# HKUST-Aerial-Robotics/MIND

Measured on AMD Instinct MI355X. Metric: sim steps/sec (whole node) + scenario-tree nodes expanded/sec, AV2 demo scenes, higher is better.
Workload: dtype f32-class (bf16 hi+mid+lo split operands = 24 significand bits, six products, fp32 accumulate) pair kernel + ActorNet, f32 elsewhere in the predictor, f64 iLQR

## Files before the change

include/mind_hip.h:

```cpp
#ifndef MIND_HIP_H
#define MIND_HIP_H

#include <stddef.h>
#include <stdint.h>

#ifdef __cplusplus
extern "C" {
#endif

#define MIND_OK 0
#define MIND_EINVAL (-1)
#define MIND_ENOMEM (-2)
#define MIND_EHIP (-3)
#define MIND_ESTATE (-4)
#define MIND_ENOTFOUND (-5)

typedef struct mind_ctx mind_ctx;

int mind_ctx_create(int device, void *stream, mind_ctx **out);
int mind_ctx_destroy(mind_ctx *ctx);
const char *mind_last_error_string(mind_ctx *ctx);
int mind_ctx_synchronize(mind_ctx *ctx);

typedef struct {
// ... 12 lines not shown
  const float *lanes;
  const float *lane_feat;
  const float *actor_ctrs;
  const float *actor_vecs;
  const float *lane_ctrs;
  const float *lane_vecs;
  const float *const *rpe;
  const float *tgt_nodes;
  const float *tgt_rpe;
} mind_scene_batch;

typedef struct {
  float *cls;
  float *reg;
  float *vel;
  float *lane_feat;
  float *actor_emb;
  float *cls_emb;
} mind_pred_out;

int mind_predict_batch(mind_ctx *ctx, const mind_scene_batch *in, mind_pred_out *out);

int mind_last_fusion_stats(mind_ctx *ctx, int *n_launches, float *total_ms, double *pairs_processed);
int mind_last_actor_stats(mind_ctx *ctx, int *layerwise, int *n_launches, int *n_chunks, float *total_ms);
int mind_last_token_stats(mind_ctx *ctx, int *layerwise, int *n_launches, int *n_chunks, float *total_ms);
int mind_last_token_stage_ms(mind_ctx *ctx, float *out_ms, int cap);
int mind_last_ilqr_stats(mind_ctx *ctx, float *kernel_ms, int *n_trees, int *workgroups_per_tree);
int mind_last_ilqr_profile(mind_ctx *ctx, double *out9);
int mind_last_ilqr_trace(mind_ctx *ctx, int tree, int phase, double *out, int cap_rows, int *n_rows);
int mind_set_profiling(mind_ctx *ctx, int enable);

#define MIND_PAIR_F32 0
#define MIND_PAIR_BF16X3 1
#define MIND_PAIR_BF16 2
#define MIND_PAIR_BF16X6 3
int mind_set_pair_precision(mind_ctx *ctx, int mode);

int mind_set_tuning(mind_ctx *ctx, const char *name, int value);
int mind_get_pair_precision(mind_ctx *ctx);
int mind_debug_pack_bfrag(const float *w, int row_stride, uint32_t *out);

int mind_debug_pair_schedule(const int *scene_tokens, const int *scene_actors, int n_scenes, int n_cu, int last_layer, int *out_jobs, int cap,
                             int *out_info);

int mind_debug_predict_choice(const char *const *knob_names, const int *knob_values, int n_knobs, int pair_prec, int n_cu, int have_side,
                              const int *scene_actors, const int *scene_lanes, int n_scenes, long long *out, int cap);

int mind_debug_ilqr_plan(const char *const *knob_names, const int *knob_values, int n_knobs, int n_cu, int mode, int n_trees, const int *n_nodes,
                         const int32_t *parents, long long *out, int cap, int *bad);

int mind_debug_aime_book(int pred_len, int max_depth, int max_rounds, int n_agents, int world, int rank, int force, int n_rounds, const int *dec_len,
                         const float *dec, int n_tokens, int bytes_per_pair, int plan_chunk_mb, int per_scene, long long *out, int cap, char *msg,
                         int msg_cap);

int mind_debug_actor_lw_plan(int n_actors, int np, int chunk, long long *out_launches, int cap, long long *out_info);

int mind_debug_token_lw_plan(int n_tokens, int mode, int chunk, long long *out_launches, int cap, long long *out_info);

int mind_debug_pack_conv_frag(const float *w, int co, int ci, int ksz, uint32_t *out, size_t cap);

int mind_debug_pack(const char *what, const float *w, int a, int b, int c, float *out, size_t cap);
int mind_debug_weight_image(const mind_tensor_desc *tensors, int n_tensors, float *blob, size_t blob_cap, char *names, size_t names_cap,
                            long long *entries, int entries_cap, long long *out_info, char *msg, int msg_cap);
int mind_debug_weight_bind(const mind_tensor_desc *tensors, int n_tensors, const char *drop, char *msg, int msg_cap);

int mind_debug_trig(mind_ctx *ctx, const double *x, int n, double *out);

int mind_debug_set_layers(mind_ctx *ctx, int n);
int64_t mind_debug_read(mind_ctx *ctx, const char *name, float *host, int64_t max_floats);

typedef struct {
  int n_nodes;
  const int32_t *parent;
  const float *prob;
  int n_agents;
  const float *agent_mean;
  const float *agent_cov;
  const double *field;
  const double *node_w;
} mind_cost_tree;

typedef struct {
  double dt, wheelbase;
  double w_des_state[6];
  double w_state_con[6];
  double state_lower[6], state_upper[6];
  double w_ctrl[2];
  double w_tgt, w_ego, w_ego_cov_offset, w_exo, w_exo_cov_offset, w_exo_cost_offset;
  double grid_res; int grid_w, grid_h;
  int max_iter;
} mind_ilqr_cfg;

typedef struct { int iterations; int converged; double J; double mu; } mind_ilqr_stats;

int mind_ilqr_solve_trees(mind_ctx *ctx, const mind_ilqr_cfg *cfg, const mind_cost_tree *trees,
                          int n_trees, const double *x0, const double *target_lane, int n_lane_pts,
                          double target_vel, int use_exo, const double *us_init, double *xs,
                          double *us, mind_ilqr_stats *stats);

int mind_ilqr_contingency(mind_ctx *ctx, const mind_ilqr_cfg *cfg_warm, const mind_ilqr_cfg *cfg_full,
                          const mind_cost_tree *trees, int n_trees, const double *x0,
                          const double *target_lane, int n_lane_pts, double target_vel, double *xs,
                          double *us, mind_ilqr_stats *stats_warm, mind_ilqr_stats *stats_full);
int mind_ilqr_contingency_begin(mind_ctx *ctx, const mind_ilqr_cfg *cfg_warm, const mind_ilqr_cfg *cfg_full,
                                const mind_cost_tree *trees, int n_trees, const double *x0,
                                const double *target_lane, int n_lane_pts, double target_vel, double *xs,
// ... 282 lines not shown
```

mind_amd/_lib.py:

```python
import ctypes as C
import os

_HERE = os.path.dirname(os.path.abspath(__file__))
LIB_PATH = os.environ.get("MIND_HIP_LIB", os.path.join(_HERE, "libmind_hip.so"))

MIND_OK = 0
MIND_EINVAL, MIND_ENOMEM, MIND_EHIP, MIND_ESTATE, MIND_ENOTFOUND = -1, -2, -3, -4, -5


class TensorDesc(C.Structure):
    _fields_ = [("name", C.c_char_p), ("data", C.POINTER(C.c_float)), ("numel", C.c_int64)]


class SceneBatch(C.Structure):
    _fields_ = [("n_scenes", C.c_int), ("actor_off", C.POINTER(C.c_int32)), ("lane_off", C.POINTER(C.c_int32)),
                ("actors", C.c_void_p), ("lanes", C.c_void_p), ("lane_feat", C.c_void_p),
                ("actor_ctrs", C.c_void_p), ("actor_vecs", C.c_void_p), ("lane_ctrs", C.c_void_p),
                ("lane_vecs", C.c_void_p), ("rpe", C.POINTER(C.c_void_p)), ("tgt_nodes", C.c_void_p),
                ("tgt_rpe", C.c_void_p)]


class PredOut(C.Structure):
    _fields_ = [("cls", C.c_void_p), ("reg", C.c_void_p), ("vel", C.c_void_p), ("lane_feat", C.c_void_p),
                ("actor_emb", C.c_void_p), ("cls_emb", C.c_void_p)]


class CostTree(C.Structure):
    _fields_ = [("n_nodes", C.c_int), ("parent", C.POINTER(C.c_int32)), ("prob", C.POINTER(C.c_float)),
                ("n_agents", C.c_int), ("agent_mean", C.POINTER(C.c_float)), ("agent_cov", C.POINTER(C.c_float)),
                ("field", C.POINTER(C.c_double)), ("node_w", C.POINTER(C.c_double))]


class FieldGrid(C.Structure):
    _fields_ = [("W", C.c_int), ("H", C.c_int), ("res", C.c_double), ("off_x", C.c_double), ("off_y", C.c_double),
                ("gx", C.POINTER(C.c_double)), ("gy", C.POINTER(C.c_double))]


class IlqrGainsOut(C.Structure):
    _fields_ = [(n, C.POINTER(C.c_double)) for n in ("k", "K", "dV", "V_x", "V_xx", "xs", "L", "J")] + [("bad_node", C.POINTER(C.c_int32))]


class WorldIn(C.Structure):
    _fields_ = [("n_scenes", C.c_int), ("actor_off", C.POINTER(C.c_int32)), ("reg", C.c_void_p), ("vel", C.c_void_p),
                ("actor_ctrs", C.c_void_p), ("actor_vecs", C.c_void_p), ("rot", C.POINTER(C.c_float)),
                ("orig", C.POINTER(C.c_float)), ("cov_last", C.POINTER(C.c_float)), ("last", C.POINTER(C.c_int32)),
                ("target_lane", C.POINTER(C.c_float)), ("n_lane_pts", C.c_int), ("cls", C.c_void_p),
                ("scen_prob", C.POINTER(C.c_float)), ("lane_check", C.c_int), ("dist_thres", C.c_float)]


class WorldOut(C.Structure):
    _fields_ = [("world", C.c_void_p), ("topo", C.c_void_p), ("ego_end", C.c_void_p), ("sel", C.c_void_p), ("sel_prob", C.c_void_p)]


class RebaseIn(C.Structure):
    _fields_ = [("n_scenes", C.c_int), ("n_agents", C.c_int), ("n_lanes", C.c_int), ("pos", C.POINTER(C.c_float)),
                ("ang", C.POINTER(C.c_float)), ("vel", C.POINTER(C.c_float)), ("types", C.POINTER(C.c_float)),
                ("pad", C.POINTER(C.c_float)), ("lane_ctrs", C.POINTER(C.c_float)), ("lane_vecs", C.POINTER(C.c_float)),
                ("target_lane", C.POINTER(C.c_float)), ("target_lane_info", C.POINTER(C.c_float)), ("n_lane_pts", C.c_int),
# ... 52 lines not shown

class LoopDesc(C.Structure):
    _fields_ = [("n_tracks", C.c_int), ("n_steps", C.c_int), ("clamp_last", C.c_int), ("ego_state", C.c_void_p), ("ego_state_is_f32", C.c_int), ("ego_obs", C.c_void_p), ("ego_trig32", C.c_void_p),
                ("tan_fn", C.c_void_p), ("sincos_fn", C.c_void_p), ("exo_obs", C.c_void_p),
                ("exo_valid", C.c_void_p), ("timestep", C.c_void_p), ("type_slot", C.c_void_p),
                ("sim_step", C.c_double), ("plan_step", C.c_double), ("enable_time", C.c_double),
                ("wheelbase", C.c_double), ("max_speed", C.c_double), ("max_steer", C.c_double), ("max_acc", C.c_double), ("max_dec", C.c_double),
                ("n_lanes", C.c_int), ("lane_pts", C.c_void_p), ("lane_flags", C.c_void_p),
                ("n_lane_pts", C.c_int), ("target_lane", C.c_void_p), ("target_lane_info", C.c_void_p),
                ("time_ahead", C.c_double), ("min_vel", C.c_float), ("dist_thres", C.c_float), ("max_depth", C.c_int), ("max_rounds", C.c_int),
                ("pred_len", C.c_int), ("prob_floor", C.c_float),
                ("cfg_warm", C.c_void_p), ("cfg_full", C.c_void_p), ("solve_n_lane_pts", C.c_int), ("solve_lane", C.c_void_p), ("target_vel", C.c_double),
                ("eval_n_lane_pts", C.c_int), ("eval_lane_is_f32", C.c_int), ("eval_lane", C.c_void_p), ("speculative", C.c_int)]


class LoopTotals(C.Structure):
    _fields_ = [("plans", C.c_longlong), ("expansions", C.c_longlong), ("scen_trees", C.c_longlong), ("rounds", C.c_longlong),
                ("aime_s", C.c_double), ("ilqr_s", C.c_double), ("total_s", C.c_double),
                ("iterations", C.c_longlong), ("node_iterations", C.c_longlong), ("node_iterations_exo", C.c_longlong),
                ("warm_speculated", C.c_longlong), ("warm_hits", C.c_longlong),
                ("pair_ms", C.c_double), ("pair_launches", C.c_longlong), ("scene_n2", C.c_double), ("scene_n_a1", C.c_double),
                ("ilqr_ms", C.c_double), ("ilqr_launches", C.c_longlong), ("ilqr_trees", C.c_longlong), ("ilqr_workgroups_per_tree", C.c_int),
                ("ilqr_prof", C.c_double * 9), ("ilqr_node_steps", C.c_double)]


class LoopOut(C.Structure):
    _fields_ = [("planned", C.c_int), ("enabled", C.c_int), ("n_steps", C.c_longlong), ("n_plans", C.c_longlong), ("episode_steps", C.c_longlong),
                ("sim_time", C.c_double), ("last_trigger", C.c_double), ("state", C.c_double * 4), ("ctrl", C.c_double * 2),
                ("n_agents", C.c_int), ("n_trees", C.c_int), ("best", C.c_int), ("n_expanded", C.c_int), ("n_rounds", C.c_int), ("n_traj_nodes", C.c_int),
                ("costs", C.POINTER(C.c_double)), ("aime_s", C.c_double), ("ilqr_s", C.c_double), ("total_s", C.c_double),
                ("tot", LoopTotals)]


PLANNER_EGO_KEY = -(1 << 63)


class PlannerDesc(C.Structure):
    _fields_ = [("time_ahead", C.c_double), ("min_vel", C.c_float), ("dist_thres", C.c_float), ("max_depth", C.c_int), ("max_rounds", C.c_int),
                ("pred_len", C.c_int), ("prob_floor", C.c_float), ("cfg_warm", C.c_void_p), ("cfg_full", C.c_void_p), ("speculative", C.c_int),
                ("ego_type_slot", C.c_int)]


class PlannerOut(C.Structure):
    _fields_ = [("n_plans", C.c_longlong),
                ("n_agents", C.c_int), ("n_trees", C.c_int), ("best", C.c_int), ("n_expanded", C.c_int), ("n_rounds", C.c_int), ("n_traj_nodes", C.c_int),
                ("costs", C.POINTER(C.c_double)), ("ctrl", C.c_double * 2), ("aime_s", C.c_double), ("ilqr_s", C.c_double), ("total_s", C.c_double),
                ("tot", LoopTotals)]


EXPORTS = ["mind_ctx_create", "mind_ctx_destroy", "mind_last_error_string", "mind_ctx_synchronize",
           "mind_weights_load", "mind_predict_batch", "mind_last_fusion_stats", "mind_last_actor_stats", "mind_debug_actor_lw_plan", "mind_last_token_stats", "mind_last_token_stage_ms", "mind_debug_token_lw_plan", "mind_set_profiling",
           "mind_ilqr_solve_trees", "mind_ilqr_contingency", "mind_ilqr_solve_fields", "mind_cost_eval", "mind_ilqr_score_trees", "mind_ilqr_gains", "mind_ilqr_policy_rollouts", "mind_lane_dist_field", "mind_aime_world", "mind_aime_rebase", "mind_debug_aime_decide", "mind_debug_set_layers",
           "mind_debug_read", "mind_set_pair_precision", "mind_get_pair_precision", "mind_debug_pack_bfrag", "mind_debug_pack_conv_frag", "mind_debug_pack", "mind_debug_weight_image", "mind_debug_weight_bind", "mind_debug_pair_schedule", "mind_debug_predict_choice", "mind_debug_ilqr_plan", "mind_debug_aime_book", "mind_set_tuning", "mind_last_ilqr_stats", "mind_aime_plan", "mind_last_ilqr_profile", "mind_eval_traj_trees", "mind_last_ilqr_trace", "mind_ilqr_contingency_begin", "mind_ilqr_finish", "mind_fill_tracks", "mind_ilqr_contingency_begin_plan", "mind_debug_trig", "mind_aime_plan_begin", "mind_aime_plan_poll", "mind_aime_plan_finish", "mind_ctx_busy", "mind_ilqr_finish_plan",
           "mind_set_exchange", "mind_last_exchange_stats",
           "mind_loop_create", "mind_loop_destroy", "mind_loop_reset", "mind_loop_advance", "mind_loop_state", "mind_loop_last_plan", "mind_loop_export",
           "mind_planner_create", "mind_planner_destroy", "mind_planner_reset", "mind_planner_observe", "mind_planner_set_lanes", "mind_planner_set_target_lane",
           "mind_planner_set_solve_lane", "mind_planner_set_eval_lane", "mind_planner_plan", "mind_planner_last_plan", "mind_planner_export"]

EXCHANGE_FN = C.CFUNCTYPE(C.c_int, C.c_void_p, C.c_int, C.c_void_p, C.c_void_p, C.c_int64)
XCHG_ALLGATHER, XCHG_ALLREDUCE, XCHG_ALLTOALLV = 0, 1, 2

_lib = None


def load():
    global _lib
    if _lib is not None:
        return _lib
    if not os.path.exists(LIB_PATH):
        raise ImportError(f"{LIB_PATH} is missing: the HIP extension must be built (hipcc --offload-arch=gfx950); "
                          "there is no CPU fallback for the product path")
    lib = C.CDLL(LIB_PATH)
    lib.mind_ctx_create.argtypes = [C.c_int, C.c_void_p, C.POINTER(C.c_void_p)]
    lib.mind_ctx_destroy.argtypes = [C.c_void_p]
    lib.mind_last_error_string.argtypes = [C.c_void_p]
    lib.mind_last_error_string.restype = C.c_char_p
    lib.mind_ctx_synchronize.argtypes = [C.c_void_p]
    lib.mind_weights_load.argtypes = [C.c_void_p, C.POINTER(TensorDesc), C.c_int]
    lib.mind_predict_batch.argtypes = [C.c_void_p, C.POINTER(SceneBatch), C.POINTER(PredOut)]
    lib.mind_last_fusion_stats.argtypes = [C.c_void_p, C.POINTER(C.c_int), C.POINTER(C.c_float), C.POINTER(C.c_double)]
    lib.mind_last_actor_stats.argtypes = [C.c_void_p, C.POINTER(C.c_int), C.POINTER(C.c_int), C.POINTER(C.c_int), C.POINTER(C.c_float)]
    lib.mind_debug_actor_lw_plan.argtypes = [C.c_int, C.c_int, C.c_int, C.POINTER(C.c_longlong), C.c_int, C.POINTER(C.c_longlong)]
    lib.mind_last_token_stats.argtypes = [C.c_void_p, C.POINTER(C.c_int), C.POINTER(C.c_int), C.POINTER(C.c_int), C.POINTER(C.c_float)]
    lib.mind_last_token_stage_ms.argtypes = [C.c_void_p, C.POINTER(C.c_float), C.c_int]
    lib.mind_debug_token_lw_plan.argtypes = [C.c_int, C.c_int, C.c_int, C.POINTER(C.c_longlong), C.c_int, C.POINTER(C.c_longlong)]
    lib.mind_set_profiling.argtypes = [C.c_void_p, C.c_int]
    lib.mind_ilqr_solve_trees.argtypes = [C.c_void_p, C.POINTER(IlqrCfg), C.POINTER(CostTree), C.c_int,
                                          C.POINTER(C.c_double), C.POINTER(C.c_double), C.c_int, C.c_double, C.c_int,
                                          C.POINTER(C.c_double), C.POINTER(C.c_double), C.POINTER(C.c_double),
                                          C.POINTER(IlqrStats)]
    lib.mind_ilqr_contingency.argtypes = [C.c_void_p, C.POINTER(IlqrCfg), C.POINTER(IlqrCfg), C.POINTER(CostTree), C.c_int,
                                          C.POINTER(C.c_double), C.POINTER(C.c_double), C.c_int, C.c_double,
                                          C.POINTER(C.c_double), C.POINTER(C.c_double), C.POINTER(IlqrStats), C.POINTER(IlqrStats)]
    lib.mind_ilqr_contingency_begin.argtypes = [C.c_void_p, C.POINTER(IlqrCfg), C.POINTER(IlqrCfg), C.POINTER(CostTree), C.c_int,
                                          C.POINTER(C.c_double), C.POINTER(C.c_double), C.c_int, C.c_double,
                                          C.POINTER(C.c_double), C.POINTER(C.c_double), C.POINTER(IlqrStats), C.POINTER(IlqrStats)]
    lib.mind_ilqr_finish.argtypes = [C.c_void_p]
    lib.mind_ilqr_contingency_begin_plan.argtypes = [C.c_void_p, C.POINTER(IlqrCfg), C.POINTER(IlqrCfg), C.c_void_p, C.c_void_p, C.c_int, C.c_double,
                                                     C.c_void_p, C.c_void_p, C.c_void_p, C.c_void_p]
    lib.mind_fill_tracks.argtypes = [C.c_void_p, C.c_int, C.c_int, C.c_void_p, C.c_void_p, C.c_void_p, C.c_void_p, C.c_void_p, C.c_void_p]
    lib.mind_ilqr_solve_fields.argtypes = [C.c_void_p, C.POINTER(IlqrCfg), C.POINTER(FieldGrid), C.POINTER(CostTree), C.c_int,
                                           C.POINTER(C.c_double), C.POINTER(C.c_double), C.POINTER(C.c_double),
                                           C.POINTER(C.c_double), C.POINTER(IlqrStats)]
    lib.mind_cost_eval.argtypes = [C.c_void_p, C.POINTER(IlqrCfg), C.POINTER(FieldGrid), C.POINTER(CostTree),
                                   C.POINTER(C.c_double), C.POINTER(C.c_double), C.c_int, C.c_double, C.c_int, C.c_int,
                                   C.POINTER(C.c_int32), C.POINTER(C.c_double), C.POINTER(C.c_double), C.POINTER(C.c_double)]
    lib.mind_ilqr_score_trees.argtypes = [C.c_void_p, C.POINTER(IlqrCfg), C.POINTER(FieldGrid), C.POINTER(CostTree), C.c_int,
                                          C.POINTER(C.c_double), C.POINTER(C.c_double), C.c_int, C.c_double, C.c_int, C.c_int,
                                          C.POINTER(C.c_double), C.POINTER(C.c_double), C.POINTER(C.c_double), C.POINTER(C.c_double)]
    lib.mind_ilqr_gains.argtypes = [C.c_void_p, C.POINTER(IlqrCfg), C.POINTER(FieldGrid), C.POINTER(CostTree), C.c_int,
                                    C.POINTER(C.c_double), C.POINTER(C.c_double), C.c_int, C.c_double, C.c_int,
                                    C.POINTER(C.c_double), C.POINTER(C.c_double), C.POINTER(IlqrGainsOut)]
    lib.mind_ilqr_policy_rollouts.argtypes = [C.c_void_p, C.POINTER(IlqrCfg), C.POINTER(FieldGrid), C.POINTER(CostTree), C.c_int,
                                              C.POINTER(C.c_double), C.POINTER(C.c_double), C.c_int, C.c_double, C.c_int,
                                              C.POINTER(C.c_double), C.POINTER(C.c_double), C.POINTER(C.c_double), C.c_int,
                                              C.POINTER(C.c_double), C.POINTER(C.c_double), C.POINTER(C.c_double), C.POINTER(C.c_double),
                                              C.POINTER(C.c_double), C.POINTER(C.c_double)]
    lib.mind_lane_dist_field.argtypes = [C.c_void_p, C.POINTER(C.c_double), C.POINTER(C.c_double), C.c_int, C.c_int, C.c_int,
                                         C.c_double] + [C.POINTER(C.c_double)] * 4
    lib.mind_aime_world.argtypes = [C.c_void_p, C.POINTER(WorldIn), C.POINTER(WorldOut)]
    lib.mind_aime_rebase.argtypes = [C.c_void_p, C.POINTER(RebaseIn), C.POINTER(RebaseOut)]
    lib.mind_debug_aime_decide.argtypes = [C.c_void_p, C.c_int, C.POINTER(C.c_int32), C.POINTER(C.c_int32), C.c_void_p, C.POINTER(C.c_float), C.c_void_p,
                                           C.c_void_p, C.c_void_p, C.c_int, C.c_float, C.c_float, C.c_int, C.c_int, C.c_void_p, C.c_void_p, C.c_void_p]
    lib.mind_aime_plan.argtypes = [C.c_void_p, C.POINTER(AimePlanIn), C.POINTER(AimePlanOut)]
    lib.mind_aime_plan_begin.argtypes = [C.c_void_p, C.POINTER(AimePlanIn)]
    lib.mind_aime_plan_poll.argtypes = [C.c_void_p]
    lib.mind_aime_plan_finish.argtypes = [C.c_void_p, C.POINTER(AimePlanOut)]
    lib.mind_ctx_busy.argtypes = [C.c_void_p]
    lib.mind_ilqr_finish_plan.argtypes = [C.c_void_p, C.c_int, C.c_int, C.c_void_p, C.c_void_p, C.c_void_p, C.c_void_p]
    lib.mind_set_pair_precision.argtypes = [C.c_void_p, C.c_int]
    lib.mind_set_tuning.argtypes = [C.c_void_p, C.c_char_p, C.c_int]
    lib.mind_last_ilqr_stats.argtypes = [C.c_void_p, C.POINTER(C.c_float), C.POINTER(C.c_int), C.POINTER(C.c_int)]
    lib.mind_last_ilqr_profile.argtypes = [C.c_void_p, C.POINTER(C.c_double)]
    lib.mind_last_ilqr_trace.argtypes = [C.c_void_p, C.c_int, C.c_int, C.POINTER(C.c_double), C.c_int, C.POINTER(C.c_int)]
    lib.mind_eval_traj_trees.argtypes = [C.POINTER(C.c_double), C.POINTER(C.c_double), C.POINTER(C.c_int32), C.c_int, C.c_void_p, C.c_int, C.c_int,
                                         C.c_double, C.POINTER(C.c_double)]
    lib.mind_get_pair_precision.argtypes = [C.c_void_p]
    lib.mind_debug_pack_bfrag.argtypes = [C.POINTER(C.c_float), C.c_int, C.POINTER(C.c_uint32)]
    lib.mind_debug_pair_schedule.argtypes = [C.POINTER(C.c_int), C.POINTER(C.c_int), C.c_int, C.c_int, C.c_int, C.POINTER(C.c_int), C.c_int, C.POINTER(C.c_int)]
    lib.mind_debug_predict_choice.argtypes = [C.POINTER(C.c_char_p), C.POINTER(C.c_int), C.c_int, C.c_int, C.c_int, C.c_int, C.POINTER(C.c_int), C.POINTER(C.c_int),
                                              C.c_int, C.POINTER(C.c_longlong), C.c_int]
    lib.mind_debug_ilqr_plan.argtypes = [C.POINTER(C.c_char_p), C.POINTER(C.c_int), C.c_int, C.c_int, C.c_int, C.c_int, C.POINTER(C.c_int), C.POINTER(C.c_int32),
                                         C.POINTER(C.c_longlong), C.c_int, C.POINTER(C.c_int)]
    lib.mind_debug_aime_book.argtypes = [C.c_int] * 8 + [C.POINTER(C.c_int), C.POINTER(C.c_float)] + [C.c_int] * 4 + [C.POINTER(C.c_longlong), C.c_int, C.c_char_p, C.c_int]
    lib.mind_debug_trig.argtypes = [C.c_void_p, C.POINTER(C.c_double), C.c_int, C.POINTER(C.c_double)]
    lib.mind_debug_pack_conv_frag.argtypes = [C.POINTER(C.c_float), C.c_int, C.c_int, C.c_int, C.POINTER(C.c_uint32), C.c_size_t]
    lib.mind_debug_pack.argtypes = [C.c_char_p, C.POINTER(C.c_float), C.c_int, C.c_int, C.c_int, C.POINTER(C.c_float), C.c_size_t]
    lib.mind_debug_weight_image.argtypes = [C.POINTER(TensorDesc), C.c_int, C.POINTER(C.c_float), C.c_size_t, C.c_char_p, C.c_size_t,
                                            C.POINTER(C.c_longlong), C.c_int, C.POINTER(C.c_longlong), C.c_char_p, C.c_int]
    lib.mind_debug_weight_bind.argtypes = [C.POINTER(TensorDesc), C.c_int, C.c_char_p, C.c_char_p, C.c_int]
    lib.mind_debug_set_layers.argtypes = [C.c_void_p, C.c_int]
    lib.mind_debug_read.argtypes = [C.c_void_p, C.c_char_p, C.POINTER(C.c_float), C.c_int64]
    lib.mind_set_exchange.argtypes = [C.c_void_p, C.c_int, C.c_int, EXCHANGE_FN, C.c_void_p, C.c_int]
    lib.mind_last_exchange_stats.argtypes = [C.c_void_p, C.POINTER(C.c_longlong), C.POINTER(C.c_longlong)]
    lib.mind_loop_create.argtypes = [C.c_void_p, C.POINTER(LoopDesc), C.POINTER(C.c_void_p)]
    lib.mind_loop_destroy.argtypes = [C.c_void_p]
    lib.mind_loop_reset.argtypes = [C.c_void_p]
    lib.mind_loop_advance.argtypes = [C.c_void_p, C.c_int, C.c_double, C.c_longlong, C.POINTER(LoopOut)]
    lib.mind_loop_state.argtypes = [C.c_void_p, C.POINTER(LoopOut)]
    lib.mind_loop_last_plan.argtypes = [C.c_void_p, C.POINTER(AimePlanOut)] + [C.POINTER(C.c_void_p)] * 6 + [C.c_void_p]
    lib.mind_loop_export.argtypes = [C.c_void_p, C.c_int, C.POINTER(C.c_int), C.c_void_p, C.c_void_p, C.c_void_p]
    lib.mind_planner_create.argtypes = [C.c_void_p, C.POINTER(PlannerDesc), C.POINTER(C.c_void_p)]
    lib.mind_planner_destroy.argtypes = [C.c_void_p]
    lib.mind_planner_reset.argtypes = [C.c_void_p]
    lib.mind_planner_observe.argtypes = [C.c_void_p, C.c_int, C.c_void_p, C.c_int, C.c_void_p, C.c_void_p, C.c_void_p]
    lib.mind_planner_set_lanes.argtypes = [C.c_void_p, C.c_int, C.c_void_p, C.c_void_p]
    lib.mind_planner_set_target_lane.argtypes = [C.c_void_p, C.c_int, C.c_void_p, C.c_void_p]
    lib.mind_planner_set_solve_lane.argtypes = [C.c_void_p, C.c_int, C.c_void_p, C.c_double]
    lib.mind_planner_set_eval_lane.argtypes = [C.c_void_p, C.c_int, C.c_void_p, C.c_int]
    lib.mind_planner_plan.argtypes = [C.c_void_p, C.c_void_p, C.c_void_p, C.POINTER(PlannerOut)]
    lib.mind_planner_last_plan.argtypes = [C.c_void_p, C.POINTER(AimePlanOut)] + [C.POINTER(C.c_void_p)] * 6 + [C.c_void_p]
    lib.mind_planner_export.argtypes = [C.c_void_p, C.c_int, C.POINTER(C.c_int), C.c_void_p, C.c_void_p, C.c_void_p]
    for n in EXPORTS:
        getattr(lib, n)
        if n not in ("mind_last_error_string", "mind_debug_read"):
            getattr(lib, n).restype = C.c_int
    lib.mind_debug_read.restype = C.c_int64
    _lib = lib
    return lib


PRED_CHOICE_FIELDS = ("header", "n_runs", "np", "actor_form", "actor_arg", "actor_grid", "actor_chunk", "actor_chunks", "actor_launches", "qsplit", "qk_stride",
                      "tiled", "edge_bf16", "edge_pair_bytes", "tok_chunk", "tok_lw", "tok_chunks", "pair_family", "pair_np", "l5_jobs5", "xcd_lanes",
                      "xcd_lanes5", "dec_actor", "dec_np", "fp32_dec", "split_dec", "want_mw", "mw_blocks", "cls_on_side", "tgt_wait_first")
PAIR_PREC = ("f32", "bf16x3", "bf16", "bf16x6")


def predict_choice(knobs, prec, scenes, n_cu=256, have_side=True):
    lib = load()
    names = (C.c_char_p * max(1, len(knobs)))(*[k.encode() for k in knobs])
    vals = (C.c_int * max(1, len(knobs)))(*[int(v) for v in knobs.values()])
    sa = (C.c_int * len(scenes))(*[a for a, _ in scenes])
    sl = (C.c_int * len(scenes))(*[l for _, l in scenes])
    cap = 32 + 6 * len(scenes)
    out = (C.c_longlong * cap)()
    n = lib.mind_debug_predict_choice(names, vals, len(knobs), PAIR_PREC.index(prec) if isinstance(prec, str) else prec, n_cu, int(have_side),
                                      sa, sl, len(scenes), out, cap)
    if n == MIND_EINVAL:
        return None
    assert 0 < n <= cap and out[0] == 32 and n == 32 + 6 * out[1], n
    d = dict(zip(PRED_CHOICE_FIELDS, out[:30]))
    d["runs"] = [tuple(out[32 + 6 * i:38 + 6 * i]) for i in range(out[1])]
    return d


ILQR_PLAN_FIELDS = ("header", "n_trees", "form", "G", "GS", "spec", "nslot", "grid", "workgroups_per_tree", "host_out", "early", "starve_followers")
ILQR_TREE_FIELDS = ("M", "nl", "nseg", "nsl", "maxls", "nfs")
ILQR_TREE_TABLES = ("level_start", "level_nodes", "child_start", "child_list", "seg_start", "seg_nodes", "slevel_start", "slevel_segs", "seg_rec",
                    "fstep_start", "fstep_items", "fstep_q1", "fstep_nstart", "fstep_nodes")


def ilqr_plan(knobs, parents, n_cu=256, generic=False, evaluate=False, two_fits=False):
    lib = load()
    names = (C.c_char_p * max(1, len(knobs)))(*[k.encode() for k in knobs])
    vals = (C.c_int * max(1, len(knobs)))(*[int(v) for v in knobs.values()])
    nn = (C.c_int * len(parents))(*[len(p) for p in parents])
    flat = [int(v) for p in parents for v in p]
    par = (C.c_int32 * max(1, len(flat)))(*flat)
    bad = (C.c_int * 2)()
    mode = int(generic) | int(evaluate) << 1 | int(two_fits) << 2
    n = lib.mind_debug_ilqr_plan(names, vals, len(knobs), n_cu, mode, len(parents), nn, par, None, 0, bad)
    if n == MIND_EINVAL:
        return {"bad": (bad[0], bad[1])} if bad[0] >= 0 else None
    out = (C.c_longlong * n)()
    assert lib.mind_debug_ilqr_plan(names, vals, len(knobs), n_cu, mode, len(parents), nn, par, out, n, bad) == n and out[0] == 16
    d = dict(zip(ILQR_PLAN_FIELDS, out[:12]))
    d["trees"], o = [], 16
    for _ in parents:
        tr = dict(zip(ILQR_TREE_FIELDS, out[o:o + 6]))
        lens, o = out[o + 6:o + 20], o + 20
        for name, ln in zip(ILQR_TREE_TABLES, lens):
            tr[name], o = list(out[o:o + ln]), o + ln
        d["trees"].append(tr)
    assert o == n
    return d


AIME_ROUND_FIELDS = ("B", "lo", "hi", "Bmax", "chunk", "S", "s0", "Sm", "any")
AIME_NODE_FIELDS = ("round", "scene", "mode", "parent", "prob", "cur_t", "end_t", "flags", "dur", "row_off", "owner", "lscene")


def aime_book(pred_len, max_depth, n_agents, rounds, world=1, rank=0, force=False, max_rounds=32, n_tokens=0, bytes_per_pair=512, plan_chunk_mb=96 * 1024,
              per_scene=1):
    import numpy as np
    lib = load()
    arrs = [np.ascontiguousarray(r, np.float32).ravel() for r in rounds]
    lens = (C.c_int * max(1, len(arrs)))(*[a.size for a in arrs])
    dec = np.concatenate(arrs + [np.zeros(1, np.float32)])
    msg = C.create_string_buffer(256)
    args = [pred_len, max_depth, max_rounds, n_agents, world, rank, int(force), len(arrs), lens, dec.ctypes.data_as(C.POINTER(C.c_float)), n_tokens,
            bytes_per_pair, plan_chunk_mb, per_scene]
    n = lib.mind_debug_aime_book(*args, None, 0, msg, 256)
    if n == MIND_EINVAL:
        return None
# ... 78 lines not shown
```

mind_amd/csrc/aime_book.h:

```cpp
#pragma once
#include <algorithm>
#include <cstddef>
#include <cstdint>
#include <cstring>
#include <vector>

#include "../../include/mind_hip.h"

constexpr int PL_K = 6;
constexpr int PL_OBS = 50;

struct PlScene {
  int node;
  float prob;
  int cur_t, end_t;
  float rot[4], orig[2], tgt[22];
};

struct PlNode {
  int round, scene, mode, parent, depth;
  int owner, lscene;
  float prob;
  int cur_t, end_t;
  bool branch, end, term, rebased;
  unsigned long long hit;
  float tgt[22];
};

inline void pl_block(int n, int r, int w, int &lo, int &hi) {
  const int base = n / w, rem = n % w;
  lo = r * base + (r < rem ? r : rem);
  hi = lo + base + (r < rem ? 1 : 0);
}
inline int pl_owner(int n, int w, int b) {
  for (int r = 0; r < w; ++r) { int lo, hi; pl_block(n, r, w, lo, hi); if (b >= lo && b < hi) return r; }
  return w - 1;
}

inline bool pl_exchanges(bool have_transport, int world, bool force) { return have_transport && (world > 1 || force); }

inline int pl_chunk(int n_tokens, int bytes_per_pair, int plan_chunk_mb, int Bk) {
  const double edge_mb = (double)n_tokens * (((n_tokens + 15) / 16) * 16) * bytes_per_pair / (1024.0 * 1024.0);
  return std::max(1, (int)std::min<double>((double)(Bk > 0 ? Bk : 1), (double)plan_chunk_mb / edge_mb));
}

enum { PL_OK = 0, PL_E_ROUNDS, PL_E_ROOT, PL_E_TRIMMED, PL_E_AGAIN, PL_E_ORDER, PL_E_NO_END };
struct PlErr { int code = PL_OK, a0 = 0, a1 = 0; explicit operator bool() const { return code != PL_OK; } };
inline const char *pl_err_format(int code) {
  switch (code) {
    case PL_E_ROUNDS: return "unsupported: more than %d AIME rounds";
    case PL_E_ROOT: return "unsupported: the root is a branching candidate";
    case PL_E_TRIMMED: return "unsupported: branch time of a trimmed node with CUR_T > 0";
    case PL_E_AGAIN: return "unsupported: a node of round %d is expanded again in round %d";
    case PL_E_ORDER: return "unsupported: branch set out of scene order";
    case PL_E_NO_END: return "unsupported: no end node found in the scenario tree";
  }
  return "";
}

struct PlTake { size_t o = 0; size_t operator()(size_t n) { const size_t r = o; o += (n + 3) & ~(size_t)3; return r; } };
struct RootLayout {
  size_t actors, ctrs, vecs, lanes, lc, lv, tn, tr, cov, types, tl, ti, wpos, wang, wvel, fr, rpos, rang, rvel, rpad, lpts, lfl, total;
  RootLayout(size_t a, size_t l, size_t P, bool raw) {
    PlTake take;
    actors = take(a * 14 * 48); ctrs = take(a * 2); vecs = take(a * 2); lanes = take(l * 160);
    lc = take(l * 2); lv = take(l * 2); tn = take(160); tr = take(20); cov = take(a);
    types = take(a * PL_OBS * 7); tl = take(P * 2); ti = take(P * 12);
    wpos = take(a * PL_OBS * 2); wang = take(a * PL_OBS); wvel = take(a * PL_OBS * 2);
    fr = take(28); rpos = take(raw ? a * PL_OBS * 2 : 0); rang = take(raw ? a * PL_OBS : 0);
    rvel = take(raw ? a * PL_OBS * 2 : 0); rpad = take(raw ? a * PL_OBS : 0);
    lpts = take(raw ? l * 11 * 2 * 2 : 0); lfl = take(raw ? l * 6 : 0);
    total = take.o;
  }
};
struct InLayout {
  size_t actors, ctrs, vecs, lc, lv, tn, tr, fr, cov, total;
  InLayout(size_t S, size_t a, size_t l) {
    PlTake take;
    actors = take(S * a * 14 * 48); ctrs = take(S * a * 2); vecs = take(S * a * 2); lc = take(S * l * 2); lv = take(S * l * 2);
    tn = take(S * 160); tr = take(S * 20); fr = take(S * 28); cov = take(S * a); total = take.o;
  }
};

struct PlRoute {
  std::vector<int64_t> tab;
  std::vector<int> snd, rcv;
  long long any = 0;
};
inline void pl_route(int S, int world, int rank, const std::vector<int> &cnt_r, const std::vector<int> &s0_r, size_t per_scene, bool self_too, PlRoute &q) {
  q.tab.assign(2 * (size_t)world, 0); q.snd.assign(2 * (size_t)world, 0); q.rcv.assign(2 * (size_t)world, 0);
  q.any = 0;
  for (int j = 0; j < world; ++j)
    for (int k = 0; k < world; ++k) {
      if (j == k && !self_too) continue;
      int klo, khi;
      pl_block(S, k, world, klo, khi);
// ... 240 lines not shown
```

mind_amd/csrc/aime_kernels.hip:

```cpp
#include <hip/hip_runtime.h>
#include <stdint.h>

struct AimeScene {
  int a0, a1;
  int last, cmp;
  float r00, r01, r10, r11;
  float ox, oy, theta_g, pad2;
};

#define AIME_SMALL 8
struct AimeSmall {
  AimeScene s[AIME_SMALL];
  float prob[AIME_SMALL];
  int n, a, pad0, pad1;
};

#define AIME_T 60
#define AIME_K 6
#define AIME_PK 6

__device__ __forceinline__ void aime_to_world(float lx, float ly, float c, float s, float cx, float cy, const AimeScene &S,
                                              bool translate, float &wx, float &wy) {
  float ax = lx * c + ly * (-s), ay = lx * s + ly * c;
  if (translate) { ax += cx; ay += cy; }
// ... 151 lines not shown
  float so[AIME_K], po[AIME_K];
  aime_select_scene(S, sp, b, t, cls, topo, ego_end, lane_check, dist_thres, prob_floor, so, po);
  if (t != 0) return;
#pragma unroll
  for (int k = 0; k < AIME_K; ++k) { sel[(size_t)b * AIME_K + k] = so[k]; sel_prob[(size_t)b * AIME_K + k] = po[k]; }
}

#define RB_THREADS 256
#define RB_FEAT_BLOCKS(a) ((int)(((size_t)(a) * 48 + RB_THREADS - 1) / RB_THREADS))
#define RB_T 50
#define RB_LANE_LDS 1024

struct RebaseArgs {
  int a, l, n_lane, pad_ones;
  const float *pos, *ang, *vel;
  const float *types;
  const float *pad;
  const float *lane_ctrs0, *lane_vecs0;
  const float *tlane, *tinfo;
  float time_ahead, min_vel;
  float *actors, *actor_ctrs, *actor_vecs, *lane_ctrs, *lane_vecs, *tgt_nodes, *tgt_rpe, *frames;
  float travel0;
};

__device__ __forceinline__ void rb_cs(float ax, float ay, float bx, float by, float &c, float &s) {
  const float den = sqrtf(ax * ax + ay * ay) * sqrtf(bx * bx + by * by) + 1e-10f;
  c = (ax * bx + ay * by) / den;
  s = (ax * by - ay * bx) / den;
}

__global__ __launch_bounds__(64) void k_aime_windows(const float *__restrict__ prev_pos, const float *__restrict__ prev_ang,
                                                     const float *__restrict__ prev_vel, const float *__restrict__ rows,
                                                     const int *__restrict__ parent_slot, const int *__restrict__ row0,
                                                     const int *__restrict__ dur, int a, float *__restrict__ pos,
                                                     float *__restrict__ ang, float *__restrict__ vel, int row_stride,
                                                     float *__restrict__ cov_last) {
  const int s = blockIdx.x / a, i = blockIdx.x - s * a, t = threadIdx.x;
  if (t >= RB_T) return;
  const int d = dur[s];
  const int src = t + d;
  float x, y, vx, vy, h;
  if (src < RB_T) {
    const size_t p = ((size_t)parent_slot[s] * a + i) * RB_T + src;
    x = prev_pos[2 * p]; y = prev_pos[2 * p + 1]; vx = prev_vel[2 * p]; vy = prev_vel[2 * p + 1]; h = prev_ang[p];
  } else {
    const float *r = rows + (((size_t)row0[s] + (size_t)i * row_stride) * AIME_T + (src - RB_T)) * AIME_PK;
    x = r[0]; y = r[1]; vx = r[2]; vy = r[3]; h = r[4];
    if (cov_last && t == RB_T - 1) cov_last[(size_t)s * a + i] = r[5];
  }
  const size_t o = ((size_t)s * a + i) * RB_T + t;
  pos[2 * o] = x; pos[2 * o + 1] = y; vel[2 * o] = vx; vel[2 * o + 1] = vy; ang[o] = h;
}

__global__ __launch_bounds__(64) void k_aime_branch(const AimeScene *__restrict__ scenes, const float *__restrict__ sel,
                                                    const float *__restrict__ world, unsigned *__restrict__ hit,
                                                    const float *__restrict__ sel_prob, float *__restrict__ h_sel, float *__restrict__ h_selp,
                                                    unsigned *__restrict__ h_hit, const AimeSmall sm) {
  const int b = blockIdx.x / AIME_K, j = blockIdx.x % AIME_K, t = threadIdx.x;
  const AimeScene S = sm.n ? sm.s[b] : scenes[b];
  const int k = (int)sel[(size_t)b * AIME_K + j];
  bool h = false;
  if (k >= 0 && t < AIME_T) {
    for (int i = S.a0; i < S.a1; ++i) {
      const float *r = world + ((size_t)i * AIME_K + k) * AIME_T * AIME_PK;
      h |= (r[t * AIME_PK + 5] / r[S.cmp * AIME_PK + 5]) > 9.0f;
    }
  }
  const unsigned long long m = __ballot(h);
  if (t == 0) { hit[2 * (size_t)blockIdx.x] = (unsigned)m; hit[2 * (size_t)blockIdx.x + 1] = (unsigned)(m >> 32); }
  if (h_sel && t == 0) {
    h_hit[2 * (size_t)blockIdx.x] = (unsigned)m; h_hit[2 * (size_t)blockIdx.x + 1] = (unsigned)(m >> 32);
    h_sel[blockIdx.x] = sel[blockIdx.x]; h_selp[blockIdx.x] = sel_prob[blockIdx.x];
  }
}

__global__ __launch_bounds__(64) void k_aime_select_branch(const AimeScene *__restrict__ scenes, const float *__restrict__ cls,
                                                           const float *__restrict__ scen_prob, const float *__restrict__ topo,
                                                           const float *__restrict__ ego_end, int lane_check, float dist_thres, float prob_floor,
                                                           const float *__restrict__ world, float *__restrict__ sel, float *__restrict__ sel_prob,
                                                           unsigned *__restrict__ hit, float *__restrict__ h_sel, float *__restrict__ h_selp,
                                                           unsigned *__restrict__ h_hit, const AimeSmall sm) {
  const int b = blockIdx.x / AIME_K, j = blockIdx.x % AIME_K, t = threadIdx.x;
  const AimeScene S = sm.n ? sm.s[b] : scenes[b];
  const float sp = sm.n ? sm.prob[b] : scen_prob[b];
  float so[AIME_K], po[AIME_K];
  aime_select_scene(S, sp, b, t, cls, topo, ego_end, lane_check, dist_thres, prob_floor, so, po);
  float kf = -1.f, pj = 0.f;
#pragma unroll
  for (int q = 0; q < AIME_K; ++q) if (q == j) { kf = so[q]; pj = po[q]; }
  const int k = (int)kf;
  bool h = false;
  if (k >= 0 && t < AIME_T) {
    for (int i0 = S.a0; i0 < S.a1; i0 += 8) {
      float num[8], den[8];
#pragma unroll
      for (int q = 0; q < 8; ++q) {
        const int i = i0 + q < S.a1 ? i0 + q : S.a1 - 1;
        const float *r = world + ((size_t)i * AIME_K + k) * AIME_T * AIME_PK;
        num[q] = r[t * AIME_PK + 5]; den[q] = r[S.cmp * AIME_PK + 5];
      }
#pragma unroll
      for (int q = 0; q < 8; ++q) if (i0 + q < S.a1) h |= (num[q] / den[q]) > 9.0f;
    }
  }
  const unsigned long long m = __ballot(h);
  if (t == 0) {
    hit[2 * (size_t)blockIdx.x] = (unsigned)m; hit[2 * (size_t)blockIdx.x + 1] = (unsigned)(m >> 32);
    sel[blockIdx.x] = kf; sel_prob[blockIdx.x] = pj;
    if (h_sel) {
      h_hit[2 * (size_t)blockIdx.x] = (unsigned)m; h_hit[2 * (size_t)blockIdx.x + 1] = (unsigned)(m >> 32);
      h_sel[blockIdx.x] = kf; h_selp[blockIdx.x] = pj;
    }
  }
}

struct AimeGather { int row0, dur, dst, a; };
__global__ __launch_bounds__(64) void k_aime_gather(const AimeGather *__restrict__ jobs, const int *__restrict__ job_of_block,
                                                    const int *__restrict__ agent_of_block, const float *const *__restrict__ world_of_job,
                                                    float *__restrict__ out) {
  const AimeGather J = jobs[job_of_block[blockIdx.x]];
  const int i = agent_of_block[blockIdx.x], t = threadIdx.x;
  if (t >= J.dur) return;
  const float *r = world_of_job[job_of_block[blockIdx.x]] + (((size_t)J.row0 + (size_t)i * AIME_K) * AIME_T + t) * AIME_PK;
  float *o = out + (size_t)J.dst + ((size_t)i * J.dur + t) * 3;
  o[0] = r[0]; o[1] = r[1]; o[2] = r[5];
}

struct AimeFlat { int row0, n, dst, a; };
__global__ __launch_bounds__(64) void k_aime_flat(const AimeFlat *__restrict__ jobs, const int *__restrict__ job_of_block,
                                                  const int *__restrict__ agent_of_block, const float *const *__restrict__ world_of_job,
                                                  float *__restrict__ mean, float *__restrict__ cov) {
  const AimeFlat J = jobs[job_of_block[blockIdx.x]];
  const int i = agent_of_block[blockIdx.x], m = threadIdx.x;
  if (m >= J.n) return;
  const float *r = world_of_job[job_of_block[blockIdx.x]] + (((size_t)J.row0 + (size_t)i * AIME_K) * AIME_T + 2 * m) * AIME_PK;
  const size_t o = (size_t)(J.dst + m) * J.a + i;
  mean[2 * o] = r[0]; mean[2 * o + 1] = r[1];
  cov[o] = r[5];
}

__global__ void k_repeat_rows(const float *__restrict__ src, size_t n, int times, float *__restrict__ dst) {
  const size_t i = (size_t)blockIdx.x * blockDim.x + threadIdx.x;
  if (i >= n * (size_t)times) return;
  dst[i] = src[i % n];
}

__global__ __launch_bounds__(RB_THREADS) void k_aime_rebase(RebaseArgs A) {
  const int sc = blockIdx.x, tid = threadIdx.x;
  const int a = A.a;
  extern __shared__ float rb_sm[];
  __shared__ float fr[8];
  __shared__ float rdv[RB_THREADS];
  __shared__ int rdi[RB_THREADS];
  __shared__ int s_idx;
  __shared__ float ctr[11][2];
  const float *pos = A.pos + (size_t)sc * a * RB_T * 2;
  const float *ang = A.ang + (size_t)sc * a * RB_T;
  const float *vel = A.vel + (size_t)sc * a * RB_T * 2;
  if (tid == 0) {
    const float th = ang[RB_T - 1];
    fr[0] = pos[(RB_T - 1) * 2]; fr[1] = pos[(RB_T - 1) * 2 + 1]; fr[2] = th; fr[3] = cosf(th); fr[4] = sinf(th);
  }
  __syncthreads();
  const float ox = fr[0], oy = fr[1], th0 = fr[2], c0 = fr[3], s0 = fr[4];
// ... 222 lines not shown
```

mind_amd/csrc/aime_plan.hip:

```cpp
#include <chrono>
namespace {

int pl_pin(mind_ctx *c, int which, size_t bytes) {
  if (bytes <= c->pl_pin_cap[which]) return MIND_OK;
  if (c->pl_pin[which]) (void)hipHostFree(c->pl_pin[which]);
  c->pl_pin[which] = nullptr; c->pl_pin_cap[which] = 0;
  const size_t want = bytes < ((size_t)64 << 20) ? std::max<size_t>(2 * bytes, (size_t)1 << 20) : bytes + bytes / 2 + 4096;
  if (hipHostMalloc(&c->pl_pin[which], want, hipHostMallocDefault) != hipSuccess)
    return fail(c, MIND_ENOMEM, "hipHostMalloc(%zu) failed", want);
  c->pl_pin_cap[which] = want;
  return MIND_OK;
}

struct CopySeg { const float *src; float *dst; long long n; };
__global__ __launch_bounds__(256) void k_copy_segs(const CopySeg *__restrict__ segs) {
  const CopySeg S = segs[blockIdx.y];
  const long long i0 = (long long)blockIdx.x * 2048 + threadIdx.x;
#pragma unroll
  for (int k = 0; k < 8; ++k) {
    const long long i = i0 + k * 256;
    if (i < S.n) S.dst[i] = S.src[i];
  }
}

int pl_exchange(mind_ctx *c, int op, void *send, void *recv, size_t bytes) {
  HIPCHK(c, hipStreamSynchronize(c->stream));
  const int rc = c->xfn(c->xuser, op, send, recv, (int64_t)bytes);
  if (rc) return fail(c, MIND_EHIP, "mind_aime_plan: the exchange callback failed (%d)", rc);
  c->x_collectives += 1;
  c->x_bytes += op == MIND_XCHG_ALLGATHER ? (long long)bytes * c->xw : (long long)bytes;
  return MIND_OK;
}

int pl_exchange_v(mind_ctx *c, void *send, void *recv, const int64_t *table) {
  HIPCHK(c, hipStreamSynchronize(c->stream));
  const int rc = c->xfn(c->xuser, MIND_XCHG_ALLTOALLV, send, recv, (int64_t)(intptr_t)table);
  if (rc) return fail(c, MIND_EHIP, "mind_aime_plan: the exchange callback failed (%d)", rc);
  c->x_collectives += 1;
  for (int r = 0; r < c->xw; ++r) c->x_bytes += (long long)table[(size_t)c->xw + r];
  return MIND_OK;
}

int pl_copy_segs(mind_ctx *c, const std::vector<CopySeg> &segs) {
  if (segs.empty()) return MIND_OK;
  long long mx = 0;
  for (const CopySeg &s : segs) mx = std::max(mx, s.n);
  if (mx == 0) return MIND_OK;
  int rc;
  if ((rc = ensure(c, c->x_seg, segs.size() * sizeof(CopySeg)))) return rc;
  if ((rc = pl_pin(c, 6, segs.size() * sizeof(CopySeg)))) return rc;
  memcpy(c->pl_pin[6], segs.data(), segs.size() * sizeof(CopySeg));
  HIPCHK(c, hipMemcpyAsync(c->x_seg.p, c->pl_pin[6], segs.size() * sizeof(CopySeg), hipMemcpyHostToDevice, c->stream));
  hipLaunchKernelGGL(k_copy_segs, dim3((unsigned)((mx + 2047) / 2048), (unsigned)segs.size()), dim3(256), 0, c->stream, (const CopySeg *)c->x_seg.p);
  HIPCHK(c, hipGetLastError());
  return MIND_OK;
}

static_assert(PL_K == AIME_K && PL_OBS == RB_T, "aime_book.h restates the kernels' constants");
static_assert(sizeof(PlJob) == sizeof(AimeGather) && sizeof(PlJob) == sizeof(AimeFlat) && offsetof(PlJob, row0) == offsetof(AimeGather, row0) &&
                  offsetof(PlJob, row0) == offsetof(AimeFlat, row0) && offsetof(PlJob, n) == offsetof(AimeGather, dur) && offsetof(PlJob, n) == offsetof(AimeFlat, n) &&
                  offsetof(PlJob, dst) == offsetof(AimeGather, dst) && offsetof(PlJob, dst) == offsetof(AimeFlat, dst) && offsetof(PlJob, a) == offsetof(AimeGather, a) &&
                  offsetof(PlJob, a) == offsetof(AimeFlat, a), "JobTable holds the packing kernels' job records");

struct PlTrace {
  std::chrono::steady_clock::time_point t0 = std::chrono::steady_clock::now();
  void operator()(const char *what) const {
    static const bool on = getenv("MIND_PLAN_TRACE") != nullptr;
    if (on) fprintf(stderr, "[plan] %8.1f us  %s\n", std::chrono::duration<double, std::micro>(std::chrono::steady_clock::now() - t0).count(), what);
  }
};

struct PlanRun {
  mind_ctx *c;
  const mind_aime_plan_in *in;
  mind_aime_plan_out *out;
  hipStream_t st;
  AimeBook &book;
  const int a, l, P, HZ;
  const bool raw;
  const int XW, XR;
  const bool dist;
  const RootLayout ro;
  const float *droot = nullptr;
  int cur_in = -1;
  const float *prev_pos = nullptr, *prev_ang = nullptr, *prev_vel = nullptr, *cov_last_dev = nullptr;
  bool frames_pending = false;
  int n_expanded = 0, pair_launches = 0;
  PlGeom g = {0, 0, 0, 0, 0};
  int chunk = 1;
  bool all_small = false, tables_done = false;
  size_t bS = 0, bI = 0, bP = 0, tab_bytes = 0, n_back = 0;
  DevBuf *tabb = nullptr;
  float *d_topo = nullptr, *d_ego = nullptr, *d_sel = nullptr, *d_selp = nullptr, *h_mirror = nullptr, *d_world = nullptr;
  unsigned *d_hit = nullptr;
  int nxt = 0;
  InLayout q{0, 0, 0};
  float *d_in = nullptr, *w_pos = nullptr, *w_ang = nullptr, *w_vel = nullptr;
  bool want_solves = false, solves_tried = false;
  int solves_rc = MIND_OK;
  PlTrace TR;

  PlanRun(mind_ctx *c_, const mind_aime_plan_in *in_, mind_aime_plan_out *out_)
      : c(c_), in(in_), out(out_), st(c_->stream), book(c_->plan.book), a(in_->n_agents), l(in_->n_lanes), P(in_->n_lane_pts), HZ(in_->pred_len),
        raw(in_->raw_pos != nullptr), XW(c_->xfn ? c_->xw : 1), XR(c_->xfn ? c_->xr : 0), dist(pl_exchanges(c_->xfn != nullptr, c_->xw, c_->xforce)),
        ro(in_->n_agents, in_->n_lanes, in_->n_lane_pts, in_->raw_pos != nullptr) {}
  bool solves_asked() const { return in->solve_cfg_full && in->solve_x0 && in->solve_lane && in->solve_n_lane_pts >= 2 && !dist; }
  int fail_book(const PlErr &e) const { return fail(c, MIND_ESTATE, pl_err_format(e.code), e.a0, e.a1); }
  int pl_root(), pl_root_raw(), pl_root_host();
  int pl_round_buffers(int round), pl_round_launch(), pl_round_tables(), pl_round_decisions(const float *&h_dec);
  int pl_predict_chunk(int g0, int cb, float *d_cls, float *d_reg, float *d_vel, const float *&d_ctrs, const float *&d_vecs);
  int pl_rebase_next(), pl_exchange_next(int round), pl_next_inputs(), pl_pack_results(), pl_hand_out();
  void pl_begin_solves();
  int pl_side_hop(hipStream_t &rs), pl_frames_back(const float *d_fr, size_t S, hipStream_t rs);
  template <class Layout> RebaseArgs pl_rebase_args(float *base, const Layout &q, size_t s0, int l) const;
};

int PlanRun::pl_side_hop(hipStream_t &rs) {
  rs = st;
  if (c->side && !dist) {
    if (!c->ev_root) HIPCHK(c, hipEventCreateWithFlags(&c->ev_root, hipEventDisableTiming));
    HIPCHK(c, hipEventRecord(c->ev_root, st));
    HIPCHK(c, hipStreamWaitEvent(c->side, c->ev_root, 0));
    rs = c->side;
  }
  return MIND_OK;
}

int PlanRun::pl_frames_back(const float *d_fr, size_t S, hipStream_t rs) {
  int rc;
  if ((rc = pl_pin(c, 3, S * 28 * sizeof(float)))) return rc;
  HIPCHK(c, hipMemcpyAsync(c->pl_pin[3], d_fr, S * 28 * sizeof(float), hipMemcpyDeviceToHost, rs));
  HIPCHK(c, hipEventRecord(c->ev_pl, rs));
  frames_pending = true;
  return MIND_OK;
}

template <class Layout>
RebaseArgs PlanRun::pl_rebase_args(float *base, const Layout &q, size_t s0, int l) const {
  RebaseArgs R;
  R.a = a; R.l = l; R.n_lane = P;
  R.types = droot + ro.types; R.tlane = droot + ro.tl; R.tinfo = droot + ro.ti;
  R.time_ahead = in->time_ahead; R.min_vel = in->min_vel;
  R.actors = base + q.actors + s0 * a * 14 * 48; R.actor_ctrs = base + q.ctrs + s0 * a * 2; R.actor_vecs = base + q.vecs + s0 * a * 2;
  R.lane_ctrs = l ? base + q.lc + s0 * l * 2 : nullptr; R.lane_vecs = l ? base + q.lv + s0 * l * 2 : nullptr;
  R.tgt_nodes = base + q.tn + s0 * 160; R.tgt_rpe = base + q.tr + s0 * 20; R.frames = base + q.fr + s0 * 28;
  return R;
}

int pl_check(mind_ctx *c, const mind_aime_plan_in *in) {
  if (!c->have_weights) return fail(c, MIND_ESTATE, "weights not loaded");
  if (c->il_finish) {
    if (!c->il_finish_owned)
      return fail(c, MIND_ESTATE, "mind_aime_plan: a tree-iLQR call begun with mind_ilqr_contingency_begin is pending on this context (mind_ilqr_finish first)");
    (void)mind_ilqr_finish(c);
    c->pl_sol_xs.clear(); c->pl_sol_us.clear(); c->pl_sol_stw.clear(); c->pl_sol_stf.clear();
  }
  const bool raw = in->raw_pos != nullptr;
  if (in->n_agents <= 0 || in->n_lanes <= 0 || in->n_lane_pts < 12 || !in->types || !in->target_lane || !in->target_lane_info ||
      (raw ? (!in->raw_ang || !in->raw_vel || !in->raw_pad || !in->lane_pts || !in->lane_flags || !(in->travel0 >= 0.f))
           : (!in->actors || !in->actor_ctrs || !in->actor_vecs || !in->lanes || !in->lane_ctrs || !in->lane_vecs || !in->tgt_nodes ||
              !in->tgt_rpe || !in->rot || !in->orig || !in->tgt_pts || !in->hist)) || in->max_depth < 0 || in->max_rounds <= 0 || in->max_rounds > 32 || in->pred_len < 2 || in->pred_len > AIME_T)
    return fail(c, MIND_EINVAL, "mind_aime_plan: bad argument");
  if (in->script_cls && (!in->script_reg || !in->script_vel)) return fail(c, MIND_EINVAL, "mind_aime_plan: scripted modes need cls, reg and vel");
  return MIND_OK;
}

int PlanRun::pl_root_raw() {
  const RootLayout &o = ro;
  const size_t OBS = RB_T;
  int rc;
  float *h = (float *)c->pl_pin[0];
  memcpy(h + o.types, in->types, a * OBS * 7 * sizeof(float));
  memcpy(h + o.tl, in->target_lane, P * 2 * sizeof(float));
  memcpy(h + o.ti, in->target_lane_info, P * 12 * sizeof(float));
  memcpy(h + o.rpos, in->raw_pos, a * OBS * 2 * sizeof(float));
  memcpy(h + o.rang, in->raw_ang, a * OBS * sizeof(float));
  memcpy(h + o.rvel, in->raw_vel, a * OBS * 2 * sizeof(float));
  memcpy(h + o.rpad, in->raw_pad, a * OBS * sizeof(float));
  memcpy(h + o.lpts, in->lane_pts, l * 22 * sizeof(double));
  memcpy(h + o.lfl, in->lane_flags, l * 6 * sizeof(int));
  if ((rc = pl_upload(c, (float *)c->pl_root.p + o.types, h + o.types, (o.total - o.types) * sizeof(float), st))) return rc;
  float *d = (float *)c->pl_root.p;
  RebaseArgs R = pl_rebase_args(d, o, 0, 0);
  R.pad_ones = 0;
  R.pos = d + o.rpos; R.ang = d + o.rang; R.vel = d + o.rvel; R.pad = d + o.rpad;
  R.lane_ctrs0 = nullptr; R.lane_vecs0 = nullptr; R.travel0 = in->travel0;
  hipLaunchKernelGGL(k_aime_rebase, dim3(1, 1 + RB_FEAT_BLOCKS(a)), dim3(RB_THREADS), 5 * a * sizeof(float), st, R);
  hipStream_t rs;
  if ((rc = pl_side_hop(rs))) return rc;
  hipLaunchKernelGGL(k_aime_root_lanes, dim3(l), dim3(64), 0, rs, (const double *)(d + o.lpts), (const int *)(d + o.lfl), (const float *)(d + o.fr),
                     d + o.lc, d + o.lv, d + o.lanes);
  hipLaunchKernelGGL(k_aime_root_hist, dim3(a), dim3(64), 0, rs, (const float *)(d + o.rpos), (const float *)(d + o.rang), (const float *)(d + o.rvel),
                     (const float *)(d + o.fr), (const float *)(d + o.ctrs), (const float *)(d + o.vecs), d + o.wpos, d + o.wang, d + o.wvel, d + o.cov);
  HIPCHK(c, hipGetLastError());
  return pl_frames_back(d + o.fr, 1, rs);
}

int PlanRun::pl_root_host() {
  const RootLayout &o = ro;
  const size_t OBS = RB_T;
  float *h = (float *)c->pl_pin[0];
  memcpy(h + o.actors, in->actors, a * 14 * 48 * sizeof(float));
  memcpy(h + o.ctrs, in->actor_ctrs, a * 2 * sizeof(float));
  memcpy(h + o.vecs, in->actor_vecs, a * 2 * sizeof(float));
  memcpy(h + o.lanes, in->lanes, l * 160 * sizeof(float));
  memcpy(h + o.lc, in->lane_ctrs, l * 2 * sizeof(float));
  memcpy(h + o.lv, in->lane_vecs, l * 2 * sizeof(float));
  memcpy(h + o.tn, in->tgt_nodes, 160 * sizeof(float));
  memcpy(h + o.tr, in->tgt_rpe, 20 * sizeof(float));
  memcpy(h + o.types, in->types, a * OBS * 7 * sizeof(float));
  memcpy(h + o.tl, in->target_lane, P * 2 * sizeof(float));
  memcpy(h + o.ti, in->target_lane_info, P * 12 * sizeof(float));
  for (size_t i = 0; i < a; ++i) {
    h[o.cov + i] = in->hist[(i * OBS + OBS - 1) * 6 + 5];
    for (size_t t = 0; t < OBS; ++t) {
      const float *r = in->hist + (i * OBS + t) * 6;
      h[o.wpos + (i * OBS + t) * 2] = r[0]; h[o.wpos + (i * OBS + t) * 2 + 1] = r[1];
      h[o.wvel + (i * OBS + t) * 2] = r[2]; h[o.wvel + (i * OBS + t) * 2 + 1] = r[3];
      h[o.wang + i * OBS + t] = r[4];
    }
  }
  HIPCHK(c, hipMemcpyAsync(c->pl_root.p, h, o.total * sizeof(float), hipMemcpyHostToDevice, st));
  PlScene &s = book.batch[0];
  memcpy(s.rot, in->rot, 4 * sizeof(float)); memcpy(s.orig, in->orig, 2 * sizeof(float)); memcpy(s.tgt, in->tgt_pts, 22 * sizeof(float));
  return MIND_OK;
}

int PlanRun::pl_root() {
  int rc;
  if ((rc = ensure(c, c->pl_root, ro.total * sizeof(float)))) return rc;
  if ((rc = pl_pin(c, 0, ro.total * sizeof(float)))) return rc;
  droot = (const float *)c->pl_root.p;
  if ((rc = raw ? pl_root_raw() : pl_root_host())) return rc;
  if ((rc = ensure(c, c->pl_lf, (size_t)l * 128 * sizeof(float)))) return rc;
  if (solves_asked() && (rc = il_field_prepare(c, in->solve_cfg_full, in->solve_x0, in->solve_lane, in->solve_n_lane_pts, c->pl_copy))) return rc;
  prev_pos = droot + ro.wpos; prev_ang = droot + ro.wang; prev_vel = droot + ro.wvel;
  cov_last_dev = droot + ro.cov;
  return MIND_OK;
}

int PlanRun::pl_round_buffers(int round) {
  const int Bk = g.Bk, Bmax = g.Bmax, A = Bk * a;
  int rc;
  const size_t n_topo = ((size_t)A * 6 + 3) & ~(size_t)3, n_ego = (size_t)Bk * 24;
  n_back = (size_t)Bmax * 6 * 4;
  if ((rc = ensure(c, c->pl_small, (n_topo + n_ego + n_back) * sizeof(float)))) return rc;
  d_topo = (float *)c->pl_small.p; d_ego = d_topo + n_topo; d_sel = d_ego + n_ego; d_selp = d_sel + (size_t)Bmax * 6;
  d_hit = (unsigned *)(d_selp + (size_t)Bmax * 6);
  h_mirror = nullptr;
  if (!dist && c->dec_mirror) {
    if ((rc = pl_pin(c, 2, n_back * sizeof(float)))) return rc;
    h_mirror = (float *)c->pl_pin[2];
  }
  tabb = &c->pl_tab[round & 1];
  bS = ((size_t)Bk * sizeof(AimeScene) + 15) & ~(size_t)15; bI = ((size_t)A * sizeof(int) + 15) & ~(size_t)15;
  bP = ((size_t)Bk * sizeof(float) + 15) & ~(size_t)15;
  tab_bytes = bS + bI + bP;
  if ((rc = ensure(c, *tabb, tab_bytes + 3 * (size_t)6 * Bmax * sizeof(int) + 64))) return rc;
  if ((rc = pl_pin(c, 1, tab_bytes + 3 * (size_t)6 * Bmax * sizeof(int) + 64))) return rc;
  if ((int)c->pl_world.size() <= round) c->pl_world.resize(round + 1);
  d_world = nullptr;
  chunk = pl_chunk(a + l + 1, pred_edge_pair_bytes(c->pt, c->pair_prec), c->plan_chunk_mb, Bk);
  if (Bk > 0) {
    if ((rc = ensure(c, c->pl_world[round], (size_t)A * 6 * AIME_T * 6 * sizeof(float)))) return rc;
    d_world = (float *)c->pl_world[round].p;
    const int cbm = std::min(chunk, Bk);
    const size_t n_cls = ((size_t)cbm * 6 + 3) & ~(size_t)3;
    if ((rc = ensure(c, c->pl_pred, (n_cls + (size_t)cbm * a * 6 * AIME_T * 7) * sizeof(float)))) return rc;
  }
  tables_done = false;
  all_small = c->tab_small && std::min(chunk, std::max(Bk, 1)) <= AIME_SMALL;
  return MIND_OK;
}

int PlanRun::pl_round_tables() {
  std::vector<PlScene> &batch = book.batch;
  const int Bk = g.Bk;
  tables_done = true;
  if (frames_pending) {
    HIPCHK(c, hipEventSynchronize(c->ev_pl));
    const float *fr = (const float *)c->pl_pin[3];
    for (int b = 0; b < g.B; ++b) {
      memcpy(batch[b].rot, fr + (size_t)b * 28, 4 * sizeof(float));
      memcpy(batch[b].orig, fr + (size_t)b * 28 + 4, 2 * sizeof(float));
      memcpy(batch[b].tgt, fr + (size_t)b * 28 + 6, 22 * sizeof(float));
    }
    frames_pending = false;
  }
  if (Bk <= 0) return MIND_OK;
  char *h = (char *)c->pl_pin[1];
  AimeScene *hs = (AimeScene *)h;
  int *as = (int *)(h + bS);
  float *sp = (float *)(h + bS + bI);
  for (int b = 0; b < Bk; ++b) {
    AimeScene &S = hs[b];
    const PlScene &q = batch[g.lo + b];
    const int bc = b % chunk;
    S.a0 = a * bc; S.a1 = a * (bc + 1); S.last = HZ - 1;      S.cmp = q.cur_t == 0 ? 1 : q.cur_t; S.pad2 = 0.f;
    S.r00 = q.rot[0]; S.r01 = q.rot[1]; S.r10 = q.rot[2]; S.r11 = q.rot[3];
    S.ox = q.orig[0]; S.oy = q.orig[1];
    S.theta_g = atan2f(S.r10, S.r00);
    for (int i = 0; i < a; ++i) as[(size_t)b * a + i] = bc;
    sp[b] = q.prob;
  }
  if (all_small) {
  } else if (c->pl_tab_side) {
    HIPCHK(c, hipMemcpyAsync(tabb->p, h, tab_bytes, hipMemcpyHostToDevice, c->pl_copy));
    HIPCHK(c, hipEventRecord(c->ev_tab, c->pl_copy));
    HIPCHK(c, hipStreamWaitEvent(st, c->ev_tab, 0));
  } else {
    HIPCHK(c, hipMemcpyAsync(tabb->p, h, tab_bytes, hipMemcpyHostToDevice, st));
  }
  return MIND_OK;
}

int PlanRun::pl_predict_chunk(int g0, int cb, float *d_cls, float *d_reg, float *d_vel, const float *&d_ctrs, const float *&d_vecs) {
  std::vector<int32_t> ao(cb + 1), lof(cb + 1);
  for (int b = 0; b <= cb; ++b) { ao[b] = a * b; lof[b] = l * b; }
  mind_scene_batch sb;
  memset(&sb, 0, sizeof(sb));
  mind_pred_out po;
  memset(&po, 0, sizeof(po));
  sb.n_scenes = cb; sb.actor_off = ao.data(); sb.lane_off = lof.data();
  if (cur_in < 0) {
// ... 4 lines not shown
  } else {
    const InLayout q(g.B, a, l);
    const float *d = (const float *)c->pl_in[cur_in].p;
    sb.actors = d + q.actors + (size_t)g0 * a * 14 * 48; sb.actor_ctrs = d_ctrs = d + q.ctrs + (size_t)g0 * a * 2; sb.actor_vecs = d_vecs = d + q.vecs + (size_t)g0 * a * 2;
    sb.lane_ctrs = d + q.lc + (size_t)g0 * l * 2; sb.lane_vecs = d + q.lv + (size_t)g0 * l * 2;
    sb.tgt_nodes = d + q.tn + (size_t)g0 * 160; sb.tgt_rpe = d + q.tr + (size_t)g0 * 20;
    sb.lane_feat = cb == 1 ? (const float *)c->pl_lf.p : (const float *)c->pl_lrep.p;
  }
  po.cls = d_cls; po.reg = d_reg; po.vel = d_vel;
  TR("round: predictor launch begins");
  const int rc = mind_predict_batch(c, &sb, &po);
  if (!rc) TR("round: predictor launched");
  return rc;
}

int PlanRun::pl_round_launch() {
  const int T = AIME_T, Bk = g.Bk, Bmax = g.Bmax;
  const char *dtab = (const char *)tabb->p;
  int rc;
  for (int c0 = 0; c0 < Bk; c0 += chunk) {
    const int cb = std::min(chunk, Bk - c0), g0 = g.lo + c0, Ac = cb * a;
    const size_t n_cls = ((size_t)cb * 6 + 3) & ~(size_t)3;
    float *d_cls = (float *)c->pl_pred.p, *d_reg = d_cls + n_cls, *d_vel = d_reg + (size_t)Ac * 6 * T * 5;
    const float *d_ctrs, *d_vecs;
    if ((rc = pl_predict_chunk(g0, cb, d_cls, d_reg, d_vel, d_ctrs, d_vecs))) return rc;
    if (!tables_done && (rc = pl_round_tables())) return rc;
    TR("round: tables prepared");
    n_expanded += cb;
    if (c->profiling) pair_launches += c->n_pair_launch;
    if (in->script_cls) {
      const size_t nr = (size_t)a * 6 * T * 5, nv = (size_t)a * 6 * T * 2;
      hipLaunchKernelGGL(k_repeat_rows, dim3((unsigned)((6 * (size_t)cb + 255) / 256)), dim3(256), 0, st, in->script_cls, (size_t)6, cb, d_cls);
      hipLaunchKernelGGL(k_repeat_rows, dim3((unsigned)((nr * cb + 255) / 256)), dim3(256), 0, st, in->script_reg, nr, cb, d_reg);
      hipLaunchKernelGGL(k_repeat_rows, dim3((unsigned)((nv * cb + 255) / 256)), dim3(256), 0, st, in->script_vel, nv, cb, d_vel);
    }
    const AimeScene *t_sc = (const AimeScene *)dtab + c0;
    const float *t_prob = (const float *)(dtab + bS + bI) + c0;
    float *w_c = d_world + (size_t)c0 * a * 6 * T * 6, *topo_c = d_topo + (size_t)c0 * a * 6, *ego_c = d_ego + (size_t)c0 * 24;
    float *sel_c = d_sel + (size_t)c0 * 6, *selp_c = d_selp + (size_t)c0 * 6;
    unsigned *hit_c = d_hit + (size_t)c0 * 12;
    AimeSmall sm;
    memset(&sm, 0, sizeof(sm));
    if (all_small) {
      const char *h = (const char *)c->pl_pin[1];
      memcpy(sm.s, (const AimeScene *)h + c0, (size_t)cb * sizeof(AimeScene));
      memcpy(sm.prob, (const float *)(h + bS + bI) + c0, (size_t)cb * sizeof(float));
      sm.n = cb; sm.a = a;
    }
    hipLaunchKernelGGL(k_aime_world, dim3(Ac * AIME_K), dim3(64), 0, st, t_sc, (const int *)(dtab + bS) + (size_t)c0 * a, d_reg, d_vel, d_ctrs, d_vecs,
                       cov_last_dev + (size_t)g0 * a, w_c, topo_c, ego_c, droot + ro.tl, P, sm);
    float *hs_ = h_mirror ? h_mirror + (size_t)c0 * 6 : nullptr, *hp_ = h_mirror ? h_mirror + (size_t)Bmax * 6 + (size_t)c0 * 6 : nullptr;
    unsigned *hh_ = h_mirror ? (unsigned *)(h_mirror + (size_t)Bmax * 12) + (size_t)c0 * 12 : nullptr;
    const float pf_ = in->prob_floor > 0.f ? in->prob_floor : 0.001f;
    if (c->glue_fused) {
      hipLaunchKernelGGL(k_aime_select_branch, dim3(cb * AIME_K), dim3(64), 0, st, t_sc, d_cls, t_prob, topo_c, ego_c, 1, in->dist_thres, pf_, w_c, sel_c, selp_c,
                         hit_c, hs_, hp_, hh_, sm);
    } else {
      hipLaunchKernelGGL(k_aime_select, dim3(cb), dim3(64), 0, st, t_sc, d_cls, t_prob, topo_c, ego_c, 1, in->dist_thres, sel_c, selp_c, pf_, sm);
      hipLaunchKernelGGL(k_aime_branch, dim3(cb * AIME_K), dim3(64), 0, st, t_sc, sel_c, w_c, hit_c, (const float *)selp_c, hs_, hp_, hh_, sm);
    }
    HIPCHK(c, hipGetLastError());
  }
  if (!tables_done && (rc = pl_round_tables())) return rc;
  return MIND_OK;
}

int PlanRun::pl_round_decisions(const float *&h_dec) {
  int rc;
  if (dist) {
    if ((rc = ensure(c, c->x_recv, (size_t)XW * n_back * sizeof(float)))) return rc;
    if ((rc = pl_exchange(c, MIND_XCHG_ALLGATHER, d_sel, c->x_recv.p, n_back * sizeof(float)))) return rc;
    if ((rc = pl_pin(c, 2, (size_t)XW * n_back * sizeof(float)))) return rc;
    HIPCHK(c, hipMemcpyAsync(c->pl_pin[2], c->x_recv.p, (size_t)XW * n_back * sizeof(float), hipMemcpyDeviceToHost, st));
  } else if (!h_mirror) {
    if ((rc = pl_pin(c, 2, n_back * sizeof(float)))) return rc;
    HIPCHK(c, hipMemcpyAsync(c->pl_pin[2], d_sel, n_back * sizeof(float), hipMemcpyDeviceToHost, st));
  }
  TR("round: glue launched, waiting for the decisions");
  HIPCHK(c, hipStreamSynchronize(st));
  TR("round: decisions on the host");
  h_dec = (const float *)c->pl_pin[2];
  return MIND_OK;
}

int PlanRun::pl_rebase_next() {
  const PlRound &r = book.rec;
  const size_t OBS = RB_T, S = r.S, s0 = r.s0;
  const int Sm = r.Sm;
  int rc;
  nxt = cur_in < 0 ? 0 : cur_in ^ 1;
  q = InLayout(S, a, l);
  if ((rc = ensure(c, c->pl_in[nxt], q.total * sizeof(float)))) return rc;
  const size_t n_wpos = S * a * OBS * 2, n_wang = S * a * OBS;
  if ((rc = ensure(c, c->pl_win[nxt], (2 * n_wpos + n_wang) * sizeof(float)))) return rc;
  w_pos = (float *)c->pl_win[nxt].p; w_ang = w_pos + n_wpos; w_vel = w_ang + n_wang;
  d_in = (float *)c->pl_in[nxt].p;
  if (Sm <= 0) return MIND_OK;
  int *hi_ = (int *)((char *)c->pl_pin[1] + tab_bytes);
  memcpy(hi_, r.win.data(), 3 * (size_t)Sm * sizeof(int));
  const bool tab_host = c->tab_host_max > 0 && (size_t)Sm * a <= (size_t)c->tab_host_max;
  if (!tab_host) HIPCHK(c, hipMemcpyAsync((char *)tabb->p + tab_bytes, hi_, 3 * (size_t)Sm * sizeof(int), hipMemcpyHostToDevice, st));
  const int *d_idx = tab_host ? (const int *)hi_ : (const int *)((const char *)tabb->p + tab_bytes);
  float *pos0 = w_pos + s0 * a * OBS * 2, *ang0 = w_ang + s0 * a * OBS, *vel0 = w_vel + s0 * a * OBS * 2;
  hipLaunchKernelGGL(k_aime_windows, dim3((unsigned)(Sm * a)), dim3(64), 0, st, prev_pos, prev_ang, prev_vel, (const float *)d_world, d_idx, d_idx + Sm,
                     d_idx + 2 * Sm, a, pos0, ang0, vel0, AIME_K, d_in + q.cov + s0 * a);
  RebaseArgs R = pl_rebase_args(d_in, q, s0, l);
  R.pad_ones = 1;
  R.pos = pos0; R.ang = ang0; R.vel = vel0; R.pad = nullptr;
  R.lane_ctrs0 = droot + ro.lc; R.lane_vecs0 = droot + ro.lv; R.travel0 = -1.f;
  hipLaunchKernelGGL(k_aime_rebase, dim3((unsigned)Sm, 1 + RB_FEAT_BLOCKS(a)), dim3(RB_THREADS), 5 * a * sizeof(float), st, R);
  HIPCHK(c, hipGetLastError());
  return MIND_OK;
}

int PlanRun::pl_exchange_next(int round) {
  const PlRound &r = book.rec;
  const size_t OBS = RB_T;
  float *fr_base = d_in + q.fr;
  int rc;
  struct Arr { float *base; size_t per; };
  const size_t na = a, nl = l;
  const Arr arrs[11] = {{d_in + q.actors, na * 14 * 48}, {d_in + q.ctrs, na * 2}, {d_in + q.vecs, na * 2}, {d_in + q.lc, nl * 2}, {d_in + q.lv, nl * 2}, {d_in + q.tn, 160},
                        {d_in + q.tr, 20}, {d_in + q.cov, na}, {w_pos, na * OBS * 2}, {w_ang, na * OBS}, {w_vel, na * OBS * 2}};
  std::vector<CopySeg> segs;
  {
    int cmax = 0;
    for (int k = 0; k < XW; ++k) cmax = std::max(cmax, r.cnt_r[k]);
    const size_t n_hdr = round == 0 ? nl * 128 : 0;
    const size_t n_pay = (n_hdr + (size_t)cmax * 28 + 3) & ~(size_t)3;
    if ((rc = ensure(c, c->x_send, n_pay * sizeof(float)))) return rc;
    if ((rc = ensure(c, c->x_recv, (size_t)XW * n_pay * sizeof(float)))) return rc;
    float *snd = (float *)c->x_send.p, *rcv = (float *)c->x_recv.p;
    if (n_hdr && XR == 0) segs.push_back({(const float *)c->pl_lf.p, snd, (long long)n_hdr});
    if (r.Sm > 0) segs.push_back({fr_base + (size_t)r.s0 * 28, snd + n_hdr, (long long)r.Sm * 28});
    if ((rc = pl_copy_segs(c, segs))) return rc;
    if ((rc = pl_exchange(c, MIND_XCHG_ALLGATHER, snd, rcv, n_pay * sizeof(float)))) return rc;
    segs.clear();
    if (n_hdr && XR != 0) segs.push_back({rcv, (float *)c->pl_lf.p, (long long)n_hdr});
    for (int k = 0; k < XW; ++k) {
      if (k == XR || r.cnt_r[k] == 0) continue;
      segs.push_back({rcv + (size_t)k * n_pay + n_hdr, fr_base + (size_t)r.s0_r[k] * 28, (long long)r.cnt_r[k] * 28});
    }
    if ((rc = pl_copy_segs(c, segs))) return rc;
  }
  size_t per_scene = 0;
  for (int k = 0; k < 11; ++k) per_scene += arrs[k].per;
  PlRoute rt;
  pl_route(r.S, XW, XR, r.cnt_r, r.s0_r, per_scene, c->xforce != 0, rt);
  if (rt.any <= 0) return MIND_OK;
  size_t n_snd = 0, n_rcv = 0;
  for (int k = 0; k < XW; ++k) { n_snd += (size_t)rt.tab[k] / sizeof(float); n_rcv += (size_t)rt.tab[(size_t)XW + k] / sizeof(float); }
  if ((rc = ensure(c, c->x_send, (n_snd + 4) * sizeof(float)))) return rc;
  if ((rc = ensure(c, c->x_recv, (n_rcv + 4) * sizeof(float)))) return rc;
  float *snd = (float *)c->x_send.p, *rcv = (float *)c->x_recv.p;
  const auto pair_segs = [&](const std::vector<int> &range, float *packed, bool unpack) {
    segs.clear();
    size_t o = 0;
    for (int k = 0; k < XW; ++k) {
      const size_t i0 = range[2 * k], n = range[2 * k + 1] - range[2 * k];
      for (int e = 0; e < 11 && n > 0; ++e) {
        float *arr = arrs[e].base + arrs[e].per * i0;
        segs.push_back(unpack ? CopySeg{packed + o, arr, (long long)(arrs[e].per * n)} : CopySeg{arr, packed + o, (long long)(arrs[e].per * n)});
        o += arrs[e].per * n;
      }
    }
  };
  pair_segs(rt.snd, snd, false);
  if ((rc = pl_copy_segs(c, segs))) return rc;
  if ((rc = pl_exchange_v(c, snd, rcv, rt.tab.data()))) return rc;
  pair_segs(rt.rcv, rcv, true);
  return pl_copy_segs(c, segs);
}

int PlanRun::pl_next_inputs() {
  const int S = book.rec.S;
  int nlo, nhi, rc;
  pl_block(S, XR, XW, nlo, nhi);
  hipStream_t rs;
  if ((rc = pl_side_hop(rs))) return rc;
  if (nhi - nlo > 1) {
    if ((rc = ensure(c, c->pl_lrep, (size_t)(nhi - nlo) * l * 128 * sizeof(float)))) return rc;
    const size_t n = (size_t)l * 128;
    hipLaunchKernelGGL(k_repeat_rows, dim3((unsigned)((n * (nhi - nlo) + 255) / 256)), dim3(256), 0, rs, (const float *)c->pl_lf.p, n, nhi - nlo, (float *)c->pl_lrep.p);
    HIPCHK(c, hipGetLastError());
  }
  if ((rc = pl_frames_back(d_in + q.fr, (size_t)S, rs))) return rc;
  prev_pos = w_pos; prev_ang = w_ang; prev_vel = w_vel;
  cov_last_dev = d_in + q.cov;
  cur_in = nxt;
  return MIND_OK;
}

void PlanRun::pl_begin_solves() {
  const size_t Mtot = (size_t)book.tree_off.back(), nt = book.tree_top.size();
  c->pl_sol_xs.resize(Mtot * 6); c->pl_sol_us.resize(Mtot * 2);
  c->pl_sol_stw.resize(nt); c->pl_sol_stf.resize(nt);
  solves_tried = true;
  solves_rc = mind_ilqr_contingency_begin_plan(c, in->solve_cfg_warm, in->solve_cfg_full, in->solve_x0, in->solve_lane, in->solve_n_lane_pts,
                                               in->solve_target_vel, c->pl_sol_xs.data(), c->pl_sol_us.data(), c->pl_sol_stw.data(), c->pl_sol_stf.data());
  c->il_finish_owned = solves_rc == MIND_OK;
}

int PlanRun::pl_pack_results() {
  const size_t Mtot = (size_t)book.tree_off.back(), n_rows = (size_t)book.n_rows, n_flat = Mtot * a * 3, n_res = n_rows + n_flat;
  want_solves = solves_asked() && !book.tree_top.empty();
  int rc;
  c->plan.agents = a;
  c->plan.rows_p = c->plan.fmean_p = c->plan.fcov_p = nullptr;
  c->plan.dev_fmean = c->plan.dev_fcov = nullptr;
  if (n_res > 0) {
    const JobTable &F = book.flat, &G = book.gather;
    const size_t o_g = F.bytes(), n_tab = o_g + G.bytes();
    const size_t o_rows = (n_tab + 255) & ~(size_t)255;
    if ((rc = ensure(c, c->pl_flat, o_rows + n_res * sizeof(float)))) return rc;
    if ((rc = pl_pin(c, 0, n_tab))) return rc;
    char *h = (char *)c->pl_pin[0];
    const float *world_of_round[32];
    for (size_t i = 0; i < c->pl_world.size() && i < 32; ++i) world_of_round[i] = (const float *)c->pl_world[i].p;
    F.pack(h, world_of_round);
    G.pack(h + o_g, world_of_round);
    TR("end: trees flattened on the host");
    const bool tab_host = !dist && c->tab_host_max > 0 && F.job_of_block.size() + G.job_of_block.size() <= (size_t)c->tab_host_max;
    if (n_tab && !tab_host) HIPCHK(c, hipMemcpyAsync(c->pl_flat.p, h, n_tab, hipMemcpyHostToDevice, st));
    char *d = tab_host ? h : (char *)c->pl_flat.p;
    float *d_rows = (float *)((char *)c->pl_flat.p + o_rows), *d_fmean = d_rows + n_rows, *d_fcov = d_fmean + Mtot * a * 2;
    if (dist) HIPCHK(c, hipMemsetAsync(d_rows, 0, n_res * sizeof(float), st));
    if (!F.jobs.empty())
      hipLaunchKernelGGL(k_aime_flat, dim3((unsigned)F.job_of_block.size()), dim3(64), 0, st, (const AimeFlat *)d, (const int *)(d + F.off_job()),
                         (const int *)(d + F.off_agent()), (const float *const *)(d + F.off_world()), d_fmean, d_fcov);
    const auto gather = [&](hipStream_t gs) {
      if (!G.jobs.empty())
        hipLaunchKernelGGL(k_aime_gather, dim3((unsigned)G.job_of_block.size()), dim3(64), 0, gs, (const AimeGather *)(d + o_g), (const int *)(d + o_g + G.off_job()),
                           (const int *)(d + o_g + G.off_agent()), (const float *const *)(d + o_g + G.off_world()), d_rows);
    };
    if (!want_solves) gather(st);
    HIPCHK(c, hipGetLastError());
    if (dist && (rc = pl_exchange(c, MIND_XCHG_ALLREDUCE, d_rows, d_rows, n_res * sizeof(float)))) return rc;
    c->plan.dev_fmean = d_fmean; c->plan.dev_fcov = d_fcov;
    if ((rc = pl_pin(c, 2, n_res * sizeof(float)))) return rc;
// ... 6 lines not shown
      TR("end: solves begun");
      HIPCHK(c, hipStreamWaitEvent(c->pl_copy, c->ev_tab, 0));
      gather(c->pl_copy);
      HIPCHK(c, hipGetLastError());
      HIPCHK(c, hipMemcpyAsync(hp, d_rows, n_res * sizeof(float), hipMemcpyDeviceToHost, c->pl_copy));
      HIPCHK(c, hipEventRecord(c->ev_rows, c->pl_copy));
      HIPCHK(c, hipEventSynchronize(c->ev_rows));
      TR("end: read-back on the host");
    } else {
      HIPCHK(c, hipMemcpyAsync(hp, d_rows, n_res * sizeof(float), hipMemcpyDeviceToHost, st));
      HIPCHK(c, hipStreamSynchronize(st));
    }
    c->plan.rows_p = hp; c->plan.fmean_p = hp + n_rows; c->plan.fcov_p = hp + n_rows + Mtot * a * 2;
  } else {
    HIPCHK(c, hipStreamSynchronize(st));
  }
  return MIND_OK;
}

int PlanRun::pl_hand_out() {
  float pair_ms = 0.f;
  int rc;
  out->nodes = book.table.data(); out->n_nodes = (int)book.table.size();
  out->rows = c->plan.rows_p; out->n_row_floats = book.n_rows;
  out->n_expanded = n_expanded; out->n_rounds = book.n_rounds;
  out->root_flags = book.root_flags();
  if (c->profiling && (rc = mind_pair_events_resolve(c, &pair_ms))) return rc;
  out->pair_ms = pair_ms; out->pair_launches = pair_launches;
  out->n_trees = (int)book.tree_top.size(); out->tree_top = book.tree_top.data(); out->tree_off = book.tree_off.data();
  out->flat_parent = book.flat_parent.data(); out->flat_prob = book.flat_prob.data();
  out->flat_mean = c->plan.fmean_p; out->flat_cov = c->plan.fcov_p;
  if (want_solves) {
    if (!solves_tried) pl_begin_solves();
    out->solves_begun = solves_rc == MIND_OK ? 1 : 0;
  }
  TR("end: result handed out");
  return MIND_OK;
}

}

extern "C" int mind_aime_plan(mind_ctx *c, const mind_aime_plan_in *in, mind_aime_plan_out *out) {
  if (!c || !in || !out) return MIND_EINVAL;
  int rc;
  if ((rc = pl_check(c, in))) return rc;
  HIPCHK(c, hipSetDevice(c->device));
  PlanRun p(c, in, out);
  c->plan.agents = 0;
  c->plan.gen += 1;
  p.book.reset(in->pred_len, in->max_depth, p.a, p.XW, p.XR, p.dist);
  if (!c->ev_pl) HIPCHK(c, hipEventCreateWithFlags(&c->ev_pl, hipEventDisableTiming));
  if (!c->ev_tab) HIPCHK(c, hipEventCreateWithFlags(&c->ev_tab, hipEventDisableTiming));
  if (!c->pl_copy) HIPCHK(c, hipStreamCreateWithFlags(&c->pl_copy, hipStreamNonBlocking));
  if ((rc = p.pl_root())) return rc;
  memset(out, 0, sizeof(*out));
  p.TR.t0 = std::chrono::steady_clock::now();
  struct DeferGuard { mind_ctx *c; ~DeferGuard() { c->ev_defer = false; c->ev_pending.clear(); c->ev_pool_used = 0; } } defer_guard{c};
  c->ev_defer = c->profiling;
  c->ev_pending.clear(); c->ev_pool_used = 0;
  for (int round = 0;; ++round) {
    PlErr e = p.book.begin_round(in->max_rounds, p.g);
    if (e) return p.fail_book(e);
    out->round_scenes[round] = p.g.Bk;
    const float *h_dec;
    if ((rc = p.pl_round_buffers(round)) || (rc = p.pl_round_launch()) || (rc = p.pl_round_decisions(h_dec))) return rc;
    if ((e = p.book.round(h_dec, p.g.Bmax))) return p.fail_book(e);
    if (p.book.rec.todo.empty()) break;
    if ((rc = p.pl_rebase_next())) return rc;
    if (p.dist && (rc = p.pl_exchange_next(round))) return rc;
    if ((rc = p.pl_next_inputs())) return rc;
  }
  p.TR("rounds done");
  const PlErr e = p.book.finish();
  if (e) return p.fail_book(e);
  if ((rc = p.pl_pack_results())) return rc;
  return p.pl_hand_out();
}

extern "C" int mind_ilqr_finish_plan(mind_ctx *c, int n_nodes, int n_trees, double *xs, double *us, mind_ilqr_stats *stats_warm, mind_ilqr_stats *stats_full) {
  if (!c || !xs || !us || !stats_full) return MIND_EINVAL;
  if (!c->il_finish || !c->il_finish_owned) return fail(c, MIND_ESTATE, "mind_ilqr_finish_plan: no plan-begun tree-iLQR call is pending on this context");
  const int rc = mind_ilqr_finish(c);
  if (rc) return rc;
  if ((size_t)n_nodes * 6 != c->pl_sol_xs.size() || (size_t)n_trees != c->pl_sol_stf.size() || (size_t)n_trees + 1 != c->plan.book.tree_off.size() ||
      c->plan.book.tree_off[(size_t)n_trees] != n_nodes)
    return fail(c, MIND_EINVAL, "mind_ilqr_finish_plan: the caller expects %d nodes in %d trees, the pending solves hold %zu in %zu", n_nodes, n_trees,
                c->pl_sol_xs.size() / 6, c->pl_sol_stf.size());
  memcpy(xs, c->pl_sol_xs.data(), c->pl_sol_xs.size() * sizeof(double));
  memcpy(us, c->pl_sol_us.data(), c->pl_sol_us.size() * sizeof(double));
  if (stats_warm) memcpy(stats_warm, c->pl_sol_stw.data(), c->pl_sol_stw.size() * sizeof(mind_ilqr_stats));
  memcpy(stats_full, c->pl_sol_stf.data(), c->pl_sol_stf.size() * sizeof(mind_ilqr_stats));
  return MIND_OK;
}


extern "C" int mind_aime_plan_begin(mind_ctx *c, const mind_aime_plan_in *in) {
  if (!c || !in) return MIND_EINVAL;
  if (c->pa_state.load(std::memory_order_acquire) == 1) return fail(c, MIND_ESTATE, "mind_aime_plan_begin: a plan is running on this context");
  if (c->pa_thread.joinable()) c->pa_thread.join();
  c->pa_in = *in;
  memset(&c->pa_out, 0, sizeof(c->pa_out));
  c->pa_state.store(1, std::memory_order_release);
  try {
    c->pa_thread = std::thread([c] {
      c->pa_rc = mind_aime_plan(c, &c->pa_in, &c->pa_out);
      c->pa_state.store(2, std::memory_order_release);
    });
  } catch (...) {
    c->pa_state.store(0, std::memory_order_release);
    return fail(c, MIND_ESTATE, "mind_aime_plan_begin: no thread");
  }
  return MIND_OK;
}

extern "C" int mind_aime_plan_poll(mind_ctx *c) {
  if (!c) return MIND_EINVAL;
  return c->pa_state.load(std::memory_order_acquire) == 1 ? 1 : 0;
}

extern "C" int mind_aime_plan_finish(mind_ctx *c, mind_aime_plan_out *out) {
  if (!c || !out) return MIND_EINVAL;
  if (c->pa_state.load(std::memory_order_acquire) == 0) return fail(c, MIND_ESTATE, "mind_aime_plan_finish: no plan was begun");
  if (c->pa_thread.joinable()) c->pa_thread.join();
  *out = c->pa_out;
  c->pa_state.store(0, std::memory_order_release);
  return c->pa_rc;
}

extern "C" int mind_ctx_busy(mind_ctx *c) {
  if (!c) return MIND_EINVAL;
  if (c->pa_state.load(std::memory_order_acquire) == 1) return 1;
  (void)hipSetDevice(c->device);
  const hipError_t e = hipStreamQuery(c->stream);
  if (e == hipErrorNotReady) return 1;
  if (e != hipSuccess) return fail(c, MIND_EHIP, "mind_ctx_busy: %s", hipGetErrorString(e));
  return 0;
}

constexpr int PL_BOOK_HEADER = 16;
extern "C" int mind_debug_aime_book(int pred_len, int max_depth, int max_rounds, int n_agents, int world, int rank, int force, int n_rounds, const int *dec_len,
                                    const float *dec, int n_tokens, int bytes_per_pair, int plan_chunk_mb, int per_scene, long long *out, int cap, char *msg,
                                    int msg_cap) {
  if (pred_len < 2 || pred_len > AIME_T || max_depth < 0 || max_rounds <= 0 || max_rounds > 32 || n_agents <= 0 || world < 1 || rank < 0 || rank >= world ||
      n_rounds < 0 || (n_rounds > 0 && (!dec_len || !dec)) || n_tokens < 0 || (n_tokens > 0 && (bytes_per_pair <= 0 || plan_chunk_mb <= 0)) || per_scene < 0 ||
      cap < 0 || (cap > 0 && !out) || msg_cap < 0 || (msg_cap > 0 && !msg))
    return MIND_EINVAL;
  const bool dist = pl_exchanges(true, world, force != 0);
  const auto bits = [](float f) { uint32_t u; memcpy(&u, &f, 4); return (long long)u; };
  AimeBook book(pred_len, max_depth, n_agents, world, rank, dist);
  std::vector<long long> rec(PL_BOOK_HEADER, 0);
  const auto put = [&rec](const auto &v) { rec.insert(rec.end(), v.begin(), v.end()); };
  PlErr e;
  PlGeom g;
  PlRoute rt;
  int rounds = 0;
  for (const float *d = dec; rounds < n_rounds; d += dec_len[rounds++]) {
    if ((e = book.begin_round(max_rounds, g))) break;
    if (dec_len[rounds] != (dist ? world : 1) * g.Bmax * 24) return MIND_EINVAL;
    if ((e = book.round(d, g.Bmax))) break;
    const PlRound &q = book.rec;
    pl_route(q.S, world, rank, q.cnt_r, q.s0_r, (size_t)per_scene, force != 0, rt);
    rec.insert(rec.end(), {g.B, g.lo, g.hi, g.Bmax, n_tokens ? pl_chunk(n_tokens, bytes_per_pair, plan_chunk_mb, g.Bk) : 0, q.S, q.s0, q.Sm, rt.any});
    put(q.todo); put(q.cnt_r); put(q.s0_r); put(q.win); put(rt.tab); put(rt.snd); put(rt.rcv);
  }
  if (!e) e = book.finish();
  if (msg_cap > 0) snprintf(msg, (size_t)msg_cap, pl_err_format(e.code), e.a0, e.a1);
  if (!e) {
    for (size_t i = 0; i < book.table.size(); ++i) {
      const mind_aime_node &n = book.table[i];
      const PlNode &m = book.nodes[i + 1];
      rec.insert(rec.end(), {n.round, n.scene, n.mode, n.parent, bits(n.prob), n.cur_t, n.end_t, n.flags, n.dur, n.row_off, m.owner, m.lscene});
    }
    for (const JobTable *t : {&book.gather, &book.flat}) {
      rec.insert(rec.end(), {(long long)t->jobs.size(), (long long)t->job_of_block.size(), (long long)t->bytes()});
      for (size_t i = 0; i < t->jobs.size(); ++i) rec.insert(rec.end(), {t->jobs[i].row0, t->jobs[i].n, t->jobs[i].dst, t->jobs[i].a, t->world[i]});
      put(t->job_of_block); put(t->agent_of_block);
    }
    put(book.tree_top); put(book.tree_off); put(book.flat_parent);
    for (float f : book.flat_prob) rec.push_back(bits(f));
  }
  const long long hdr[12] = {PL_BOOK_HEADER, e.code, e.a0, e.a1, rounds, e ? 0 : (long long)book.table.size(), e ? 0 : (long long)book.tree_top.size(),
                             e ? 0 : (long long)book.flat_parent.size(), e ? 0 : book.n_rows, book.root_flags(), dist, world};
  std::copy(hdr, hdr + 12, rec.begin());
  for (size_t i = 0; i < rec.size() && (int)i < cap; ++i) out[i] = rec[i];
  return (int)rec.size();
}
```

mind_amd/csrc/encdec_kernels.hip:

```cpp
#include <hip/hip_runtime.h>
#include <stdint.h>

#include "weight_tables.h"

typedef float f32x4 __attribute__((ext_vector_type(4)));

#define NT 256

__device__ __forceinline__ float wave_sum(float v) {
  v += __shfl_xor(v, 32, 64);
  v += __shfl_xor(v, 16, 64);
  v += __shfl_xor(v, 8, 64);
  v += __shfl_xor(v, 4, 64);
  v += __shfl_xor(v, 2, 64);
  v += __shfl_xor(v, 1, 64);
  return v;
}

__device__ __forceinline__ float block_sum(float v, float *red) {
  v = wave_sum(v);
  __syncthreads();
  if ((threadIdx.x & 63) == 0) red[threadIdx.x >> 6] = v;
  __syncthreads();
  return red[0] + red[1] + red[2] + red[3];
// ... 226 lines not shown
            acc[r] = fmaf(w[4 * q4 + 3], x[3], acc[r]);
          }
        DENSE_ROW_FENCE();
        }
      }
      for (; k < K; k += 4) {
#pragma unroll
        for (int r = 0; r < R; ++r) {
          const f32x4 x = *(const f32x4 *)(in + r * ldi + k);
#pragma unroll
          for (int q = 0; q < 4; ++q) acc[r] = fmaf(WT[(size_t)(k + q) * NOUT + o], x[q], acc[r]);
        }
      }
#pragma unroll
      for (int r = 0; r < R; ++r) out[r * ldo + o] = acc[r];
    }
    return;
  }
  const int kp = threadIdx.x / NOUT, o = threadIdx.x % NOUT;
  const int Kc = ((K / 4 + KP - 1) / KP) * 4;
  if (kp < KP) {
    float acc[R];
#pragma unroll
    for (int r = 0; r < R; ++r) acc[r] = 0.f;
    const int k0 = kp * Kc, k1 = min(K, k0 + Kc);
    int k = k0;
    for (; k + DB <= k1; k += DB) {
      float w[DB];
#pragma unroll
      for (int q = 0; q < DB; ++q) w[q] = WT[(size_t)(k + q) * NOUT + o];
#pragma unroll
      for (int r = 0; r < R; ++r) {
#pragma unroll
        for (int q4 = 0; q4 < DB / 4; ++q4) {
          const f32x4 x = *(const f32x4 *)(in + r * ldi + k + 4 * q4);
          acc[r] = fmaf(w[4 * q4 + 0], x[0], acc[r]);
          acc[r] = fmaf(w[4 * q4 + 1], x[1], acc[r]);
          acc[r] = fmaf(w[4 * q4 + 2], x[2], acc[r]);
          acc[r] = fmaf(w[4 * q4 + 3], x[3], acc[r]);
        }
        DENSE_ROW_FENCE();
      }
    }
    for (; k < k1; k += 4) {
#pragma unroll
      for (int r = 0; r < R; ++r) {
        const f32x4 x = *(const f32x4 *)(in + r * ldi + k);
#pragma unroll
        for (int q = 0; q < 4; ++q) acc[r] = fmaf(WT[(size_t)(k + q) * NOUT + o], x[q], acc[r]);
      }
    }
#pragma unroll
    for (int r = 0; r < R; ++r) part[(kp * R + r) * NOUT + o] = acc[r];
  }
  __syncthreads();
  for (int i = threadIdx.x; i < R * NOUT; i += nthr) {
    const int r = i / NOUT, oo = i % NOUT;
    float v = b ? b[oo] : 0.f;
    for (int q = 0; q < KP; ++q) v += part[(q * R + r) * NOUT + oo];
    out[r * ldo + oo] = v;
  }
}

#define LN_REGS 12
__device__ __forceinline__ void ln_rows(float *buf, int ld, int R, int n, const float *__restrict__ g,
                                        const float *__restrict__ be, bool relu) {
  const int lane = threadIdx.x & 63, wave = threadIdx.x >> 6, nw = blockDim.x >> 6;
  for (int r = wave; r < R; r += nw) {
    if (n <= 64 * LN_REGS) {
      float xv[LN_REGS], gv[LN_REGS], bv[LN_REGS];
#pragma unroll
      for (int i = 0; i < LN_REGS; ++i) {
        const int k = lane + 64 * i;
        const bool in = k < n;
        xv[i] = in ? buf[r * ld + k] : 0.f;
        gv[i] = in ? g[k] : 0.f;
        bv[i] = in ? be[k] : 0.f;
      }
      float s = 0.f;
#pragma unroll
      for (int i = 0; i < LN_REGS; ++i) if (lane + 64 * i < n) s += xv[i];
      const float mean = wave_sum(s) / (float)n;
      float v = 0.f;
#pragma unroll
      for (int i = 0; i < LN_REGS; ++i) if (lane + 64 * i < n) { const float d = xv[i] - mean; v = fmaf(d, d, v); }
      const float rstd = 1.0f / sqrtf(wave_sum(v) / (float)n + 1e-5f);
#pragma unroll
      for (int i = 0; i < LN_REGS; ++i) {
        const int k = lane + 64 * i;
        if (k < n) {
          float y = (xv[i] - mean) * rstd * gv[i] + bv[i];
          if (relu) y = fmaxf(y, 0.f);
          buf[r * ld + k] = y;
        }
      }
      continue;
    }
    float s = 0.f;
    for (int k = lane; k < n; k += 64) s += buf[r * ld + k];
    const float mean = wave_sum(s) / (float)n;
    float v = 0.f;
    for (int k = lane; k < n; k += 64) { const float d = buf[r * ld + k] - mean; v = fmaf(d, d, v); }
    const float rstd = 1.0f / sqrtf(wave_sum(v) / (float)n + 1e-5f);
    for (int k = lane; k < n; k += 64) {
      float y = (buf[r * ld + k] - mean) * rstd * g[k] + be[k];
      if (relu) y = fmaxf(y, 0.f);
// ... 444 lines not shown
  __syncthreads();
  dense<6>(&att[0][0], 128, 128, W.k3W, W.k3b, 128, &t2[0][0], 128, part, PF);
  DEC_MARK();
  __syncthreads();
  ln_rows(&t2[0][0], 128, 6, 128, W.k3g, W.k3be, true);
  DEC_MARK();
  __syncthreads();
  for (int k = tid >> 6; k < 6; k += (int)(blockDim.x >> 6)) {
    const int lane = tid & 63;
    float s = t2[k][lane] * W.k6W[lane] + t2[k][lane + 64] * W.k6W[lane + 64];
    s = wave_sum(s);
    if (lane == 0) sc[0][0][k] = s + W.k6b[0];
  }
  __syncthreads();
  if (tid == 0 && (!MW || wg == 0)) {
    float m = -INFINITY;
    for (int k = 0; k < 6; ++k) m = fmaxf(m, sc[0][0][k]);
    float e[6], sum = 0.f;
    for (int k = 0; k < 6; ++k) { e[k] = expf(sc[0][0][k] - m); sum += e[k]; }
    for (int k = 0; k < 6; ++k) cls_out[(size_t)b * 6 + k] = e[k] / sum;
  }
  DEC_MARK();
#ifdef MIND_DEC_TRACE
  if (blockIdx.x == 0 && tid == 0) {
    printf("[k_dec_scene] cycles between marks (dense / LayerNorm stages in program order):");
    for (int q = 1; q < dec_trn_ && q < 64; ++q) printf(" %lld", dec_tr_[q] - dec_tr_[q - 1]);
    printf("\n");
  }
#endif
}

__global__ __launch_bounds__(DT) void k_dec_scene(const float *__restrict__ x, const int *__restrict__ cls_row, float *__restrict__ Cout,
                                                  float *__restrict__ cls_out, DecW W) {
  k_dec_scene_body<false>(x, cls_row, Cout, cls_out, W, (int)blockIdx.x, 0, 1, nullptr, nullptr, nullptr);
}
__global__ __launch_bounds__(DT) void k_dec_scene_c(const float *__restrict__ x, const int *__restrict__ cls_row, float *__restrict__ Cout, DecW W) {
  k_dec_scene_body<false, 1>(x, cls_row, Cout, nullptr, W, (int)blockIdx.x, 0, 1, nullptr, nullptr, nullptr);
}
__global__ __launch_bounds__(DT) void k_dec_cls(float *__restrict__ Cout, float *__restrict__ cls_out, DecW W) {
  k_dec_scene_body<false, 2>(nullptr, nullptr, Cout, cls_out, W, (int)blockIdx.x, 0, 1, nullptr, nullptr, nullptr);
}
#define DEC_MW_G 8
__global__ __launch_bounds__(DT) void k_dec_scene_mw(const float *__restrict__ x, const int *__restrict__ cls_row, float *__restrict__ Cout,
                                                     float *__restrict__ cls_out, DecW W, int n_scenes, float *__restrict__ xbuf,
                                                     unsigned *__restrict__ bars, unsigned *abort_word) {
  const int r = (int)blockIdx.x % (8 * DEC_MW_G);
  const int b = 8 * ((int)blockIdx.x / (8 * DEC_MW_G)) + (r & 7), wg = r >> 3;
  if (b >= n_scenes) return;
  k_dec_scene_body<true>(x, cls_row, Cout, cls_out, W, b, wg, DEC_MW_G, xbuf + (size_t)b * 2 * 6 * 1536, bars + 4 * (size_t)b, abort_word);
}

#define RA 4
#define DEC_ACTOR_LDS_FLOATS (512 + 1536 + 3072 + 3072 + 3072 + 960 + 6144)
template <int PART>
__global__ __launch_bounds__(DT) void k_dec_actor(const float *__restrict__ x ,
                                                  const int *__restrict__ actor_row ,
                                                  const int *__restrict__ actor_scene , int n_actors,
                                                  const float *__restrict__ Cmode ,
                                                  const float *__restrict__ tgt ,
                                                  float *__restrict__ reg, float *__restrict__ vel, DecW W, float *__restrict__ h2g) {
  extern __shared__ __attribute__((aligned(16))) float dsm[];
  float (*xin)[128] = (float (*)[128])(dsm);
  float (*h1)[384] = (float (*)[384])(dsm + 512);
  float (*h2)[768] = (float (*)[768])(dsm + 2048);
  float (*E)[128] = (float (*)[128])(dsm + 5120);
  float (*t1)[128] = (float (*)[128])(dsm + 8192);
  float (*prm)[40] = (float (*)[40])(dsm + 11264);
  float *part = dsm + 12224;
  const int PF = 6144;
  const int tid = threadIdx.x;
  const int a0 = blockIdx.x * RA;
  if (PART != 2) {
    for (int i = tid; i < RA * 128; i += blockDim.x) {
      const int r = i / 128, a = a0 + r;
      xin[r][i % 128] = a < n_actors ? x[(size_t)actor_row[a] * 128 + i % 128] : 0.f;
    }
    __syncthreads();
    dense<RA>(&xin[0][0], 128, 128, W.a0W, W.a0b, 384, &h1[0][0], 384, part, PF);
    __syncthreads();
    ln_rows(&h1[0][0], 384, RA, 384, W.a0g, W.a0be, true);
    __syncthreads();
    dense<RA>(&h1[0][0], 384, 384, W.a3W, W.a3b, 768, &h2[0][0], 768, part, PF);
    __syncthreads();
    ln_rows(&h2[0][0], 768, RA, 768, W.a3g, W.a3be, true);
    __syncthreads();
    if (PART == 1) {
      for (int i = tid; i < RA * 768; i += blockDim.x) {
        const int r = i / 768, a = a0 + r;
        if (a < n_actors) h2g[(size_t)a * 768 + i % 768] = h2[r][i % 768];
      }
      return;
    }
  } else {
    for (int i = tid; i < RA * 768; i += blockDim.x) {
      const int r = i / 768, a = a0 + r;
      h2[r][i % 768] = a < n_actors ? h2g[(size_t)a * 768 + i % 768] : 0.f;
    }
    __syncthreads();
  }
  for (int i = tid; i < RA * 768; i += blockDim.x) {
    const int r = i / 768, k = (i % 768) / 128, c = i % 128;
    const int a = a0 + r;
    float v = 0.f;
    if (a < n_actors) {
      const int sc = actor_scene[a];
      v = h2[r][k * 128 + c] + Cmode[((size_t)sc * 6 + k) * 128 + c];
      if (k == 0) v += tgt[(size_t)sc * 128 + c];
    }
    E[r * 6 + k][c] = v;
  }
  __syncthreads();
  dense<RA * 6>(&E[0][0], 128, 128, W.r0W, W.r0b, 128, &t1[0][0], 128, part, PF);
  __syncthreads();
  ln_rows(&t1[0][0], 128, RA * 6, 128, W.r0g, W.r0be, true);
  __syncthreads();
  dense<RA * 6>(&t1[0][0], 128, 128, W.r3W, W.r3b, 128, &E[0][0], 128, part, PF);
  __syncthreads();
  ln_rows(&E[0][0], 128, RA * 6, 128, W.r3g, W.r3be, true);
  __syncthreads();
  for (int i = tid; i < RA * 6 * 40; i += blockDim.x) {
    const int r = i / 40, o = i % 40;
    float acc = W.r6b[o];
    for (int k = 0; k < 128; ++k) acc = fmaf(W.r6W[k * 40 + o], E[r][k], acc);
    prm[r][o] = acc;
  }
  __syncthreads();
  for (int i = tid; i < RA * 6 * 60; i += blockDim.x) {
    const int r = i / 60, t = i % 60;
    const int a = a0 + r / 6, k = r % 6;
    if (a >= n_actors) continue;
    float o5[5] = {0.f, 0.f, 0.f, 0.f, 0.f};
    for (int c = 0; c < 8; ++c) {
      const float tv = W.T[t * 8 + c];
#pragma unroll
      for (int d = 0; d < 5; ++d) o5[d] = fmaf(tv, prm[r][c * 5 + d], o5[d]);
    }
    float v2[2] = {0.f, 0.f};
    for (int c = 0; c < 7; ++c) {
      const float tv = W.Tp[t * 7 + c];
      v2[0] = fmaf(tv, prm[r][(c + 1) * 5 + 0] - prm[r][c * 5 + 0], v2[0]);
      v2[1] = fmaf(tv, prm[r][(c + 1) * 5 + 1] - prm[r][c * 5 + 1], v2[1]);
    }
    float *ro = reg + (((size_t)a * 6 + k) * 60 + t) * 5;
    ro[0] = o5[0]; ro[1] = o5[1]; ro[2] = expf(o5[2]); ro[3] = expf(o5[3]); ro[4] = expf(o5[4]);
    float *vo = vel + (((size_t)a * 6 + k) * 60 + t) * 2;
    vo[0] = v2[0] / 6.0f; vo[1] = v2[1] / 6.0f;
  }
}

extern "C" size_t mind_dec_scene_lds_bytes() { return (size_t)DEC_SCENE_LDS_FLOATS * sizeof(float); }
extern "C" size_t mind_dec_actor_lds_bytes() { return (size_t)DEC_ACTOR_LDS_FLOATS * sizeof(float); }
```

mind_amd/csrc/mind_hip.hip:

```cpp
#include <hip/hip_runtime.h>

#include <cmath>
#include <cstdarg>
#include <cstdio>
#include <cstdlib>
#include <algorithm>
#include <cstring>
#include <map>
#include <string>
#include <thread>
#include <atomic>
#include <functional>
#include <vector>

#include "../../include/mind_hip.h"
#include "encdec_kernels.hip"
#include "fusion_kernels.hip"
#include "pair_bf16_kernels.hip"
#include "pair_tile_kernels.hip"
#include "pair_tile6_kernels.hip"
#include "token_mfma_kernels.hip"
#include "actor_mfma_kernels.hip"
#include "actor_lw_kernels.hip"
#include "token_lw_kernels.hip"
// ... 4 lines not shown
#include "ilqr_policy_kernels.hip"
#include "pair_jobs.h"
#include "pred_choice.h"
#include "ilqr_choice.h"
#include "aime_book.h"
#include "weight_pack.h"
#include "aime_kernels.hip"

namespace {

struct DevBuf {
  void *p = nullptr;
  size_t cap = 0;
};

}

struct TableSet {
  std::vector<int> key;
  DevBuf meta, jobs, jobs5, rows;
  std::vector<int> actor_row, cls_row, scene_n;
  long long edge_pairs = 0, edge_pairs_t = 0, stamp = 0;
  int ntok = 0, slot = 0, njobs = 0, njobs5 = 0;
  double pairs_full = 0, pairs_l5 = 0;
};
#define MIND_TABLE_SETS 8

struct mind_ctx {
  int device = 0;
  hipStream_t stream = nullptr;
  bool own_stream = false;
  hipStream_t side = nullptr;
  hipEvent_t ev_side = nullptr, ev_main = nullptr, ev_stage = nullptr, ev_tgt = nullptr, ev_cls = nullptr;
  std::vector<char> aime_stage;
  bool aime_stage_busy = false;
  std::string err;
  float *wdev = nullptr;
  bool have_weights = false;
  WeightTables W = {};
  PredTuning pt;
  DevBuf tok_lw_arena;
  std::vector<TlLaunch> tok_lw_plan;
  int last_tok_lw = 0, last_tok_launches = 0, last_tok_chunks = 0;
  float tok_ms = 0.f, tok_stage_ms[TL_NSTAGE + 1] = {};
  std::vector<hipEvent_t> ev_tok;
  std::vector<int> ev_tok_tag;
  TableSet tabs[MIND_TABLE_SETS];
  long long tab_clock = 0;
  long long n_table_hits = 0;
  IlqrTuning it;
  int upload_kernel_max = 1 << 20;
  bool dec_mirror = true;
  bool glue_fused = true;
  bool early_eval = true;
  int tab_host_max = 4096;
  bool tab_small = true;
  std::vector<IlTables> il_tab;
  struct IlImage { std::vector<double> hD; std::vector<float> hF; std::vector<int> hI; } il_img;
  struct IlEarly { const double *xs = nullptr, *us = nullptr; volatile unsigned *done = nullptr; unsigned gen = 0; int n_trees = 0; long nodes = 0; } il_early;
  unsigned il_gen = 0;
  long long il_spec_req = 0, il_spec_hit = 0;
  DevBuf actor_lw_arena;
  std::vector<LwLaunch> actor_lw_plan;
  int last_actor_lw = 0, last_actor_launches = 0, last_actor_chunks = 0;
  float actor_ms = 0.f;
  hipEvent_t ev_act0 = nullptr, ev_act1 = nullptr;
  int pair_prec = 3;
  int plan_chunk_mb = 96 * 1024;
  std::vector<int> last_scene_n;
  bool last_edge_tiled = false, last_edge_bf16 = false;
  DevBuf edge, x, ST, QK, part, tokpos, meta, jobs, actor_feat, lane_feat, tgt_feat, cmode, tgt_emb,
      rows, rpe_ptrs;
  DevBuf ilqr_dev, aime_dev, rebase_dev2[2], dec_h2;
  DevBuf pl_root, pl_in[2], pl_lf, pl_lrep, pl_pred, pl_small, pl_tab[2], pl_win[2];
  std::vector<DevBuf> pl_world;
  void *pl_pin[8] = {nullptr, nullptr, nullptr, nullptr, nullptr, nullptr, nullptr, nullptr};
  size_t pl_pin_cap[8] = {0, 0, 0, 0, 0, 0, 0, 0};
  hipEvent_t ev_pl = nullptr, ev_tab = nullptr, ev_root = nullptr;
  DevBuf il_field;
  void *il_field_pin = nullptr;
  size_t il_field_pin_cap = 0;
  hipEvent_t ev_field = nullptr;
  bool il_field_valid = false;
  double il_field_key[5] = {0, 0, 0, 0, 0};
  std::vector<double> il_field_lane;
  int xr = 0, xw = 1;
  mind_exchange_fn xfn = nullptr;
  void *xuser = nullptr;
  bool xforce = false;
  DevBuf x_send, x_recv, x_seg;
  long long x_collectives = 0, x_bytes = 0;
  hipStream_t pl_copy = nullptr;
  bool pl_tab_side = false;
  std::vector<double> pl_sol_xs, pl_sol_us;
  std::vector<mind_ilqr_stats> pl_sol_stw, pl_sol_stf;
  std::thread pa_thread;
  std::atomic<int> pa_state{0};
  mind_aime_plan_in pa_in;
  mind_aime_plan_out pa_out;
  int pa_rc = 0;
  struct Plan {
    AimeBook book;
    int agents = 0;
    long long gen = 0;
    const float *rows_p = nullptr, *fmean_p = nullptr, *fcov_p = nullptr;
    const float *dev_fmean = nullptr, *dev_fcov = nullptr;
// ... 103 lines not shown
  (void)hipFuncSetAttribute((const void *)k_pair_t<0, 1>, hipFuncAttributeMaxDynamicSharedMemorySize, (int)mind_pair_bf_lds_bytes());
  (void)hipFuncSetAttribute((const void *)k_pair_t<1, 1>, hipFuncAttributeMaxDynamicSharedMemorySize, (int)mind_pair_bf_lds_bytes());
  (void)hipFuncSetAttribute((const void *)k_pair_t6<0>, hipFuncAttributeMaxDynamicSharedMemorySize, (int)mind_pair_bf_lds_bytes());
  (void)hipFuncSetAttribute((const void *)k_pair_t6<1>, hipFuncAttributeMaxDynamicSharedMemorySize, (int)mind_pair_bf_lds_bytes());
  if (const char *te = getenv("MIND_PAIR_TILE")) c->pt.pair_tile = !(te[0] == '0');
  if (const char *xe = getenv("MIND_XCD_ORDER")) c->pt.xcd_order = !(xe[0] == '0');

  if (const char *pe = getenv("MIND_PAIR_PREC")) {
    const std::string v = pe;
    if (v == "f32" || v == "0") c->pair_prec = 0;
    else if (v == "bf16x3" || v == "1") c->pair_prec = 1;
    else if (v == "bf16" || v == "2") c->pair_prec = 2;
    else if (v == "bf16x6" || v == "3") c->pair_prec = 3;
  }
  (void)hipFuncSetAttribute((const void *)k_actor_net, hipFuncAttributeMaxDynamicSharedMemorySize, (int)mind_actor_lds_bytes());
  (void)hipFuncSetAttribute((const void *)k_actor_mfma<3>, hipFuncAttributeMaxDynamicSharedMemorySize, (int)mind_actor_mfma_lds_bytes());
  (void)hipFuncSetAttribute((const void *)k_actor_mfma<6>, hipFuncAttributeMaxDynamicSharedMemorySize, (int)mind_actor_mfma_lds_bytes());
  (void)hipFuncSetAttribute((const void *)k_dec_actor_mfma<1>, hipFuncAttributeMaxDynamicSharedMemorySize, (int)mind_dec_actor_mfma_lds_bytes());
  (void)hipFuncSetAttribute((const void *)k_dec_actor_mfma<3>, hipFuncAttributeMaxDynamicSharedMemorySize, (int)mind_dec_actor_mfma_lds_bytes());
  (void)hipFuncSetAttribute((const void *)k_dec_actor_mfma<6>, hipFuncAttributeMaxDynamicSharedMemorySize, (int)mind_dec_actor_mfma_lds_bytes());
  if (const char *se = getenv("MIND_ACTOR_SPLIT")) c->pt.actor_np = atoi(se) == 3 ? 3 : 6;
  (void)hipFuncSetAttribute((const void *)k_actor_mfma<1>, hipFuncAttributeMaxDynamicSharedMemorySize, (int)mind_actor_mfma_lds_bytes());
  if (const char *me = getenv("MIND_ENC_MFMA")) c->pt.enc_mfma = !(me[0] == '0');
  if (const char *me = getenv("MIND_ACTOR_F32")) c->pt.actor_f32 = !(me[0] == '0');
  if (const char *me = getenv("MIND_ACTOR_F32_MIN")) c->pt.actor_f32_min = atoi(me);
  if (const char *me = getenv("MIND_ACTOR_LW_MIN")) c->pt.actor_lw_min = atoi(me);
  lw_set_attributes();
  (void)hipFuncSetAttribute((const void *)k_actor_f32<1>, hipFuncAttributeMaxDynamicSharedMemorySize, (int)mind_actor_f32_lds_bytes(1));
  (void)hipFuncSetAttribute((const void *)k_actor_f32<2>, hipFuncAttributeMaxDynamicSharedMemorySize, (int)mind_actor_f32_lds_bytes(2));
  if (const char *de = getenv("MIND_DEC_MFMA_MIN")) c->pt.dec_mfma_min = atoi(de);
  if (const char *oe = getenv("MIND_DEC_OVERLAP")) c->pt.dec_overlap = !(oe[0] == '0');
  (void)hipFuncSetAttribute((const void *)k_ilqr<true, 0>, hipFuncAttributeMaxDynamicSharedMemorySize, (int)il_lds_bytes(0));
  (void)hipFuncSetAttribute((const void *)k_ilqr<false, 1>, hipFuncAttributeMaxDynamicSharedMemorySize, (int)il_lds_bytes(0));
  (void)hipFuncSetAttribute((const void *)k_ilqr<false, 0>, hipFuncAttributeMaxDynamicSharedMemorySize, (int)il_lds_bytes(0));
  (void)hipFuncSetAttribute((const void *)k_ilqr<false, 2>, hipFuncAttributeMaxDynamicSharedMemorySize, (int)il_lds_bytes(0));
  if (const char *te = getenv("MIND_TOK_MFMA")) c->pt.tok_mfma = !(te[0] == '0');
  if (const char *te = getenv("MIND_TOK_SMALL_MAX")) c->pt.tok_small_max = atoi(te);
  if (const char *te = getenv("MIND_TOK_MERGE")) c->pt.tok_merge = !(te[0] == '0');
  if (const char *te = getenv("MIND_DEC_MW")) c->pt.dec_mw = !(te[0] == '0');
  if (const char *te = getenv("MIND_DEC_CLS_SIDE")) c->pt.dec_cls_side = !(te[0] == '0');
  if (const char *te = getenv("MIND_TOK_BF_MIN_N")) c->pt.tok_bf_min_n = atoi(te);
  if (const char *te = getenv("MIND_TOK_LW_MIN_N")) c->pt.tok_lw_min_n = atoi(te);
  if (const char *te = getenv("MIND_TOK_LW_MIN")) c->pt.tok_lw_min = atoi(te);
  if (const char *te = getenv("MIND_TGT_SIDE")) c->pt.tgt_side = !(te[0] == '0');
  if (const char *te = getenv("MIND_PL_TAB_SIDE")) c->pl_tab_side = !(te[0] == '0');
  (void)hipFuncSetAttribute((const void *)k_token_mfma<0>, hipFuncAttributeMaxDynamicSharedMemorySize, (int)mind_token_mfma_lds_bytes());
  (void)hipFuncSetAttribute((const void *)k_token_mfma<1>, hipFuncAttributeMaxDynamicSharedMemorySize, (int)mind_token_mfma_lds_bytes());
  if (const char *ce = getenv("MIND_PLAN_CHUNK_MB")) { const long v = atol(ce); if (v > 0) c->plan_chunk_mb = v; }
  if (const char *we = getenv("MIND_TAB_SMALL")) c->tab_small = atoi(we) != 0;
  if (const char *we = getenv("MIND_TAB_HOST_MAX")) c->tab_host_max = std::max(0, atoi(we));
  if (const char *we = getenv("MIND_EARLY_EVAL")) c->early_eval = atoi(we) != 0;
  if (const char *we = getenv("MIND_GLUE_FUSED")) c->glue_fused = atoi(we) != 0;
  if (const char *we = getenv("MIND_DEC_MIRROR")) c->dec_mirror = atoi(we) != 0;
  if (const char *we = getenv("MIND_UPLOAD_KERNEL_MAX")) c->upload_kernel_max = std::max(0, atoi(we));
  const char *const il_env[][2] = {{"MIND_ILQR_CHUNK", "ilqr_chunk"}, {"MIND_ILQR_WGS", "ilqr_wgs"}, {"MIND_ILQR_SPEC_DERIV", "ilqr_spec_deriv"},
                                   {"MIND_ILQR_HOST_OUT_MAX", "ilqr_host_out_max"}, {"MIND_ILQR_SLOTS", "ilqr_slots"}};
  for (const auto &e : il_env)
    if (const char *we = getenv(e[0])) (void)ilqr_tuning_set(c->it, e[1], atoi(we));
  (void)hipFuncSetAttribute((const void *)k_dec_scene, hipFuncAttributeMaxDynamicSharedMemorySize, (int)mind_dec_scene_lds_bytes());
  (void)hipFuncSetAttribute((const void *)k_dec_scene_mw, hipFuncAttributeMaxDynamicSharedMemorySize, (int)mind_dec_scene_lds_bytes());
  (void)hipFuncSetAttribute((const void *)k_dec_scene_c, hipFuncAttributeMaxDynamicSharedMemorySize, (int)mind_dec_scene_lds_bytes());
  (void)hipFuncSetAttribute((const void *)k_dec_cls, hipFuncAttributeMaxDynamicSharedMemorySize, (int)mind_dec_scene_lds_bytes());
  (void)hipFuncSetAttribute((const void *)k_dec_tgt, hipFuncAttributeMaxDynamicSharedMemorySize, (int)mind_dec_scene_lds_bytes());
  (void)hipFuncSetAttribute((const void *)k_dec_actor<0>, hipFuncAttributeMaxDynamicSharedMemorySize, (int)mind_dec_actor_lds_bytes());
  (void)hipFuncSetAttribute((const void *)k_dec_actor<1>, hipFuncAttributeMaxDynamicSharedMemorySize, (int)mind_dec_actor_lds_bytes());
  (void)hipFuncSetAttribute((const void *)k_dec_actor<2>, hipFuncAttributeMaxDynamicSharedMemorySize, (int)mind_dec_actor_lds_bytes());
  *out = c;
  return MIND_OK;
}

extern "C" int mind_ctx_destroy(mind_ctx *c) {
  if (!c) return MIND_EINVAL;
  if (c->pa_thread.joinable()) c->pa_thread.join();
  (void)hipSetDevice(c->device);
  (void)hipStreamSynchronize(c->stream);
  DevBuf *bufs[] = {&c->edge, &c->x, &c->ST, &c->QK, &c->part, &c->tokpos, &c->meta, &c->jobs, &c->actor_feat,
                    &c->lane_feat, &c->tgt_feat, &c->cmode, &c->tgt_emb, &c->rows, &c->rpe_ptrs, &c->ilqr_dev, &c->aime_dev, &c->rebase_dev2[0], &c->rebase_dev2[1], &c->dec_h2};
  for (DevBuf *b : bufs)
    if (b->p) (void)hipFree(b->p);
  for (TableSet &t : c->tabs)
    for (DevBuf *b : {&t.meta, &t.jobs, &t.jobs5, &t.rows})
      if (b->p) (void)hipFree(b->p);
  if (c->wdev) (void)hipFree(c->wdev);
  for (DevBuf *b : {&c->dec_xbuf, &c->dec_bars})
    if (b->p) (void)hipFree(b->p);
  if (c->dec_abort) (void)hipHostFree(c->dec_abort);
  for (DevBuf *b : {&c->pl_root, &c->pl_in[0], &c->pl_in[1], &c->pl_lf, &c->pl_lrep, &c->pl_pred, &c->pl_small, &c->pl_tab[0], &c->pl_tab[1], &c->pl_win[0],
                    &c->pl_win[1], &c->pl_flat, &c->x_send, &c->x_recv, &c->x_seg})
    if (b->p) (void)hipFree(b->p);
  for (DevBuf &b : c->pl_world)
    if (b.p) (void)hipFree(b.p);
  for (void *q : c->pl_pin)
    if (q) (void)hipHostFree(q);
  if (c->ev_pl) (void)hipEventDestroy(c->ev_pl);
  if (c->ev_root) (void)hipEventDestroy(c->ev_root);
  if (c->ev_field) (void)hipEventDestroy(c->ev_field);
  if (c->il_field.p) (void)hipFree(c->il_field.p);
  if (c->il_field_pin) (void)hipHostFree(c->il_field_pin);
  if (c->ev_tab) (void)hipEventDestroy(c->ev_tab);
  if (c->ev_rows) (void)hipEventDestroy(c->ev_rows);
  if (c->pl_copy) (void)hipStreamDestroy(c->pl_copy);
  for (hipEvent_t e : c->ev) (void)hipEventDestroy(e);
  for (hipEvent_t e : c->ev_pool) (void)hipEventDestroy(e);
  if (c->ev_side) (void)hipEventDestroy(c->ev_side);
  if (c->ev_main) (void)hipEventDestroy(c->ev_main);
  if (c->ev_tgt) (void)hipEventDestroy(c->ev_tgt);
  if (c->ev_stage) (void)hipEventDestroy(c->ev_stage);
  if (c->ev_cls) (void)hipEventDestroy(c->ev_cls);
  if (c->actor_lw_arena.p) (void)hipFree(c->actor_lw_arena.p);
  if (c->tok_lw_arena.p) (void)hipFree(c->tok_lw_arena.p);
  for (hipEvent_t e : c->ev_tok) (void)hipEventDestroy(e);
  if (c->ev_act0) (void)hipEventDestroy(c->ev_act0);
  if (c->ev_act1) (void)hipEventDestroy(c->ev_act1);
  if (c->ev_il0) (void)hipEventDestroy(c->ev_il0);
  if (c->ev_il1) (void)hipEventDestroy(c->ev_il1);
  if (c->side) { (void)hipStreamSynchronize(c->side); (void)hipStreamDestroy(c->side); }
  if (c->own_stream) (void)hipStreamDestroy(c->stream);
  delete c;
  return MIND_OK;
}

extern "C" const char *mind_last_error_string(mind_ctx *c) { return c ? c->err.c_str() : "null context"; }

extern "C" int mind_ctx_synchronize(mind_ctx *c) {
  if (!c) return MIND_EINVAL;
  HIPCHK(c, hipStreamSynchronize(c->stream));
  return MIND_OK;
}

extern "C" int mind_set_tuning(mind_ctx *c, const char *name, int value) {
  if (!c || !name) return MIND_EINVAL;
  const std::string n = name;
  if (pred_tuning_set(c->pt, name, value)) return MIND_OK;
  if (ilqr_tuning_set(c->it, name, value)) return MIND_OK;
  if (n == "plan_chunk_mb") c->plan_chunk_mb = value < 1 ? 1 : value;
  else if (n == "pl_tab_side") c->pl_tab_side = value != 0;
  else if (n == "tab_small") c->tab_small = value != 0;
  else if (n == "tab_host_max") c->tab_host_max = value < 0 ? 0 : value;
  else if (n == "early_eval") c->early_eval = value != 0;
  else if (n == "glue_fused") c->glue_fused = value != 0;
  else if (n == "dec_mirror") c->dec_mirror = value != 0;
  else if (n == "upload_kernel_max") c->upload_kernel_max = value < 0 ? 0 : value;
  else return fail(c, MIND_EINVAL, "mind_set_tuning: unknown knob '%s'", name);
  return MIND_OK;
}

extern "C" int mind_set_exchange(mind_ctx *c, int rank, int world, mind_exchange_fn fn, void *user, int force) {
  if (!c) return MIND_EINVAL;
  if (fn && (world < 1 || rank < 0 || rank >= world)) return fail(c, MIND_EINVAL, "mind_set_exchange: rank %d of %d", rank, world);
  c->xfn = fn; c->xuser = user;
  c->xr = fn ? rank : 0; c->xw = fn ? world : 1; c->xforce = fn && force != 0;
  return MIND_OK;
}

extern "C" int mind_last_exchange_stats(mind_ctx *c, long long *collectives, long long *bytes) {
  if (!c) return MIND_EINVAL;
  if (collectives) *collectives = c->x_collectives;
  if (bytes) *bytes = c->x_bytes;
  return MIND_OK;
}

extern "C" int mind_set_pair_precision(mind_ctx *c, int mode) {
  if (!c || mode < 0 || mode > 3) return MIND_EINVAL;
  c->pair_prec = mode;
  return MIND_OK;
}

extern "C" int mind_get_pair_precision(mind_ctx *c) { return c ? c->pair_prec : MIND_EINVAL; }

extern "C" int mind_debug_pack_bfrag(const float *w, int row_stride, uint32_t *out) {
  if (!w || !out || row_stride < 128) return MIND_EINVAL;
  std::vector<float> v(w, w + (size_t)127 * row_stride + 128);
  v.resize((size_t)128 * row_stride, 0.f);
  const std::vector<float> t = pack_bfrag(v, row_stride);
  memcpy(out, t.data(), 16384 * sizeof(uint32_t));
  return MIND_OK;
}

extern "C" int mind_set_profiling(mind_ctx *c, int enable) {
  if (!c) return MIND_EINVAL;
  c->profiling = enable != 0;
  return MIND_OK;
}

extern "C" int mind_last_ilqr_stats(mind_ctx *c, float *kernel_ms, int *n_trees, int *workgroups_per_tree) {
  if (!c) return MIND_EINVAL;
  if (kernel_ms) *kernel_ms = c->ilqr_ms;
  if (n_trees) *n_trees = c->ilqr_trees;
  if (workgroups_per_tree) *workgroups_per_tree = c->ilqr_multi;
  return MIND_OK;
}

extern "C" int mind_last_ilqr_trace(mind_ctx *c, int tree, int phase, double *out, int cap_rows, int *n_rows) {
  if (!c || !n_rows || (cap_rows > 0 && !out)) return MIND_EINVAL;
// ... 337 lines not shown
}

extern "C" int mind_debug_aime_decide(mind_ctx *c, int n_scenes, const int32_t *actor_off, const int32_t *cmp, const float *cls, const float *scen_prob,
                                      const float *topo, const float *ego_end, const float *world, int lane_check, float dist_thres,
                                      float prob_floor, int fused, int by_value, float *sel, float *sel_prob, uint32_t *hit) {
  if (!c || n_scenes <= 0 || !actor_off || !cmp || !cls || !scen_prob || !topo || !ego_end || !world || !sel || !sel_prob || !hit)
    return fail(c, MIND_EINVAL, "mind_debug_aime_decide: bad argument");
  const int B = n_scenes;
  std::vector<AimeScene> hs(B);
  for (int b = 0; b < B; ++b) {
    AimeScene &S = hs[b];
    memset(&S, 0, sizeof(S));
    S.a0 = actor_off[b]; S.a1 = actor_off[b + 1]; S.last = AIME_T - 1; S.cmp = cmp[b];
    S.r00 = S.r11 = 1.f;
    if (S.a0 < 0 || S.a1 <= S.a0) return fail(c, MIND_EINVAL, "mind_debug_aime_decide: scene %d has no agents", b);
    if (S.cmp < 0 || S.cmp >= AIME_T) return fail(c, MIND_EINVAL, "mind_debug_aime_decide: scene %d: compare step %d out of range", b, S.cmp);
  }
  AimeSmall sm;
  memset(&sm, 0, sizeof(sm));
  if (by_value) {
    const int a = hs[0].a1 - hs[0].a0;
    if (B > AIME_SMALL) return fail(c, MIND_EINVAL, "mind_debug_aime_decide: tables by value hold at most %d scenes (%d given)", AIME_SMALL, B);
    for (int b = 0; b < B; ++b)
      if (hs[b].a1 - hs[b].a0 != a || hs[b].a0 != b * a)
        return fail(c, MIND_EINVAL, "mind_debug_aime_decide: tables by value need the same agent count in every scene");
    memcpy(sm.s, hs.data(), (size_t)B * sizeof(AimeScene));
    memcpy(sm.prob, scen_prob, (size_t)B * sizeof(float));
    sm.n = B; sm.a = a;
  }
  HIPCHK(c, hipSetDevice(c->device));
  hipStream_t st = c->stream;
  const size_t bS = ((size_t)B * sizeof(AimeScene) + 15) & ~(size_t)15;
  std::vector<char> stage(bS + (size_t)B * sizeof(float), 0);
  memcpy(stage.data(), hs.data(), (size_t)B * sizeof(AimeScene));
  memcpy(stage.data() + bS, scen_prob, (size_t)B * sizeof(float));
  if (by_value) {
    for (int b = 0; b < B; ++b) {
      AimeScene S = hs[b];
      S.a1 = S.a0 + 1; S.cmp = (S.cmp + 29) % AIME_T;
      memcpy(stage.data() + (size_t)b * sizeof(AimeScene), &S, sizeof(S));
    }
    memset(stage.data() + bS, 0, (size_t)B * sizeof(float));
  }
  char *dtab = nullptr;
  HIPCHK(c, hipMalloc((void **)&dtab, stage.size()));
  hipError_t e = hipMemcpyAsync(dtab, stage.data(), stage.size(), hipMemcpyHostToDevice, st);
  if (e == hipSuccess) {
    const AimeScene *t_sc = (const AimeScene *)dtab;
    const float *t_prob = (const float *)(dtab + bS);
    const float pf_ = prob_floor > 0.f ? prob_floor : 0.001f;
    const int lc = lane_check ? 1 : 0;
    if (fused) {
      hipLaunchKernelGGL(k_aime_select_branch, dim3(B * AIME_K), dim3(64), 0, st, t_sc, cls, t_prob, topo, ego_end, lc, dist_thres, pf_, world, sel, sel_prob,
                         hit, (float *)nullptr, (float *)nullptr, (unsigned *)nullptr, sm);
    } else {
      hipLaunchKernelGGL(k_aime_select, dim3(B), dim3(64), 0, st, t_sc, cls, t_prob, topo, ego_end, lc, dist_thres, sel, sel_prob, pf_, sm);
      hipLaunchKernelGGL(k_aime_branch, dim3(B * AIME_K), dim3(64), 0, st, t_sc, (const float *)sel, world, hit, (const float *)sel_prob, (float *)nullptr,
                         (float *)nullptr, (unsigned *)nullptr, sm);
    }
    e = hipGetLastError();
    if (e == hipSuccess) e = hipStreamSynchronize(st);
  }
  (void)hipFree(dtab);
  HIPCHK(c, e);
  return MIND_OK;
}

#include "aime_plan.hip"

namespace {
double np_pairwise(const double *a, long n) {
  if (n < 8) {
    double r = 0.0;
    for (long i = 0; i < n; ++i) r += a[i];
    return r;
  }
  if (n <= 128) {
    double r[8];
    long i;
    for (i = 0; i < 8; ++i) r[i] = a[i];
    for (i = 8; i < n - (n % 8); i += 8)
      for (int j = 0; j < 8; ++j) r[j] += a[i + j];
    double res = ((r[0] + r[1]) + (r[2] + r[3])) + ((r[4] + r[5]) + (r[6] + r[7]));
    for (; i < n; ++i) res += a[i];
    return res;
  }
  long n2 = n / 2;
  n2 -= n2 % 8;
  return np_pairwise(a, n2) + np_pairwise(a + n2, n - n2);
}
template <class T>
void eval_nodes(const double *st, const double *ct, long N, const T *lane, int P, double tv, double *per_node) {
  const int S = P - 1;
  std::vector<T> dx(S), dy(S), l2(S);
  for (int q = 0; q < S; ++q) {
    dx[q] = lane[2 * q + 2] - lane[2 * q];
    dy[q] = lane[2 * q + 3] - lane[2 * q + 1];
    l2[q] = dx[q] * dx[q] + dy[q] * dy[q];
  }
  constexpr int BS = 8;
  const int NB = (S + BS - 1) / BS;
  std::vector<double> sx_(S), sy_(S), sr_(S), bx(NB), by(NB), br(NB);
  for (int q = 0; q < S; ++q) {
    const double ax = (double)lane[2 * q], ay = (double)lane[2 * q + 1], ex = (double)lane[2 * q + 2], ey = (double)lane[2 * q + 3];
    sx_[q] = 0.5 * (ax + ex); sy_[q] = 0.5 * (ay + ey);
    sr_[q] = 0.5 * sqrt((ex - ax) * (ex - ax) + (ey - ay) * (ey - ay)) * (1.0 + 1e-9) + 1e-9;
  }
  for (int b = 0; b < NB; ++b) {
    const int q0 = b * BS, q1 = std::min(S, q0 + BS);
    double cx = 0.0, cy = 0.0;
    for (int q = q0; q < q1; ++q) { cx += sx_[q]; cy += sy_[q]; }
// ... 195 lines not shown
```

mind_amd/csrc/pred_choice.h:

```cpp
#pragma once
#include <cstring>
#include <vector>

struct PredTuning {
  bool pair_tile = true;
  bool xcd_order = true;
  bool enc_mfma = true;
  int actor_np = 6;
  bool actor_f32 = true;
  int actor_f32_min = 1 << 30, actor_f32_pair_min = 1 << 30;
  int actor_lw_min = 1 << 30, actor_lw_chunk = 0;
  bool tok_mfma = false;
  int tok_bf_min_n = 0;
  int tok_lw_min_n = 1 << 30, tok_lw_min = 1 << 30, tok_lw_chunk = 0;
  bool tok_merge = true;
  int tok_small_max = 2048;
  int dec_mfma_min = 1 << 30;
  bool dec_overlap = true;
  bool dec_mw = false;
  bool dec_cls_side = false;
  bool tgt_side = true;
};

static bool pred_tuning_set(PredTuning &t, const char *name, int value) {
  const auto is = [name](const char *k) { return strcmp(name, k) == 0; };
  if (is("dec_mfma_min")) t.dec_mfma_min = value;
  else if (is("enc_mfma")) t.enc_mfma = value != 0;
  else if (is("actor_f32")) t.actor_f32 = value != 0;
  else if (is("actor_f32_min")) t.actor_f32_min = value;
  else if (is("actor_f32_pair_min")) t.actor_f32_pair_min = value;
  else if (is("actor_lw_min")) t.actor_lw_min = value;
  else if (is("actor_lw_chunk")) t.actor_lw_chunk = value < 0 ? 0 : value;
  else if (is("actor_split")) t.actor_np = value == 3 ? 3 : 6;
  else if (is("xcd_order")) t.xcd_order = value != 0;
  else if (is("pair_tile")) t.pair_tile = value != 0;
  else if (is("dec_overlap")) t.dec_overlap = value != 0;
  else if (is("tok_mfma")) t.tok_mfma = value != 0;
  else if (is("tok_small_max")) t.tok_small_max = value;
  else if (is("tok_merge")) t.tok_merge = value != 0;
  else if (is("dec_mw")) t.dec_mw = value != 0;
  else if (is("dec_cls_side")) t.dec_cls_side = value != 0;
  else if (is("tok_bf_min_n")) t.tok_bf_min_n = value;
  else if (is("tok_lw_min_n")) t.tok_lw_min_n = value;
  else if (is("tok_lw_min")) t.tok_lw_min = value;
  else if (is("tok_lw_chunk")) t.tok_lw_chunk = value < 0 ? 0 : value;
  else if (is("tgt_side")) t.tgt_side = value != 0;
  else return false;
  return true;
}

static inline int pred_mfma_parts(const PredTuning &t, int pair_prec) {
  return (pair_prec == 3 || (pair_prec == 1 && t.actor_np == 6)) ? 6 : (pair_prec == 1 ? 3 : 1);
}

static inline bool pred_edge_tiled(const PredTuning &t, int pair_prec) { return pair_prec == 3 || (pair_prec != 0 && t.pair_tile); }

static inline int pred_edge_pair_bytes(const PredTuning &t, int pair_prec) { return pred_edge_tiled(t, pair_prec) && pair_prec == 2 ? 256 : 512; }

enum PredActorForm { PRED_ACTOR_VALU = 0, PRED_ACTOR_F32 = 1, PRED_ACTOR_MFMA = 2, PRED_ACTOR_LW = 3 };
enum PredPairFamily { PRED_PAIR_F32 = 0, PRED_PAIR_BF = 1, PRED_PAIR_T = 2, PRED_PAIR_T6 = 3 };
enum PredDecActor { PRED_DEC_ONE = 0, PRED_DEC_SPLIT = 1, PRED_DEC_MFMA = 2 };

struct PredTokRun {
  int t0, n, kind;
  bool layerwise;
  bool small, merged;
};

struct PredChoice {
  int np = 1;
  int actor_form = PRED_ACTOR_VALU, actor_arg = 0, actor_grid = 0, actor_chunk = 0, actor_chunks = 1, actor_launches = 1;
  int qsplit = 0, qk_stride = 1024;
  bool tiled = false, edge_bf16 = false;
  std::vector<PredTokRun> tok_runs;
  int tok_chunk = 0;
  bool tok_lw = false;
  int last_tok_chunks = 0;
  int pair_family = PRED_PAIR_F32, pair_np = 0;
  bool l5_jobs5 = false;
  int xcd_lanes = 1, xcd_lanes5 = 1;
  int dec_actor = PRED_DEC_ONE;
  bool fp32_dec = true, split_dec = false, want_mw = false, cls_side = false;
  int mw_blocks = 0;
  bool tgt_wait_first = false;
};

static PredChoice pred_choose(const PredTuning &t, int pair_prec, int n_cu, bool have_side, int n_scenes, const int *scene_actors, const int *scene_lanes) {
  PredChoice ch;
  int A = 0;
  for (int b = 0; b < n_scenes; ++b) A += scene_actors[b];
  ch.np = pred_mfma_parts(t, pair_prec);

  ch.actor_grid = A;
  if (t.actor_f32 && A >= (pair_prec == 0 ? t.actor_f32_pair_min : t.actor_f32_min)) {
    ch.actor_form = PRED_ACTOR_F32; ch.actor_arg = 2; ch.actor_grid = (A + 1) / 2;
  } else if (pair_prec == 0 && t.actor_f32 && t.enc_mfma) {
    ch.actor_form = PRED_ACTOR_F32; ch.actor_arg = 1;
  } else if (pair_prec == 0 || !t.enc_mfma) {
    ch.actor_form = PRED_ACTOR_VALU;
  } else if (A >= t.actor_lw_min) {
    ch.actor_form = PRED_ACTOR_LW; ch.actor_arg = ch.np;
    ch.actor_chunk = t.actor_lw_chunk > 0 ? t.actor_lw_chunk : LW_CHUNK;
    ch.actor_chunks = (A + ch.actor_chunk - 1) / ch.actor_chunk;
    ch.actor_grid = ch.actor_chunks;
    ch.actor_launches = ch.actor_chunks * (1 + 2 * LW_NSTAGE);
  } else {
    ch.actor_form = PRED_ACTOR_MFMA; ch.actor_arg = ch.np;
  }

  ch.qsplit = pair_prec == 3 ? 48 : pair_prec != 0 ? 16 : 0;
  ch.qk_stride = pair_prec == 3 ? P6_QK_STRIDE : 1024;
  ch.tiled = pred_edge_tiled(t, pair_prec);
  ch.edge_bf16 = pred_edge_pair_bytes(t, pair_prec) == 256;

  ch.tok_chunk = t.tok_lw_chunk > 0 ? t.tok_lw_chunk : TL_CHUNK;
  long long njobs = 0, njobs5 = 0;
  int t0 = 0;
  for (int b = 0; b < n_scenes; ++b) {
    const int N = scene_actors[b] + scene_lanes[b] + 1;
    const int kind = t.tok_mfma ? 1 : (pair_prec != 0 && pair_prec != 3 && t.tok_bf_min_n > 0 && N >= t.tok_bf_min_n) ? 2 : N >= t.tok_lw_min_n ? 1 : 0;
    if (!ch.tok_runs.empty() && ch.tok_runs.back().kind == kind) ch.tok_runs.back().n += N;
    else ch.tok_runs.push_back({t0, N, kind, false, false, false});
    t0 += N;
    njobs += (long long)N * pair_column_splits(N);
    njobs5 += (long long)(scene_actors[b] + 1) * pair_column_splits(N);
  }
  for (PredTokRun &r : ch.tok_runs) {
    r.layerwise = r.kind == 1 && r.n >= t.tok_lw_min;
    r.small = r.kind == 0 && r.n <= t.tok_small_max;
    r.merged = r.small && t.tok_merge;
    if (r.layerwise) {
      ch.tok_lw = true;
      ch.last_tok_chunks += (r.n + ch.tok_chunk - 1) / ch.tok_chunk;
    }
  }

  ch.pair_family = pair_prec == 0 ? PRED_PAIR_F32 : pair_prec == 3 ? PRED_PAIR_T6 : ch.tiled ? PRED_PAIR_T : PRED_PAIR_BF;
  ch.pair_np = (ch.pair_family == PRED_PAIR_T || ch.pair_family == PRED_PAIR_BF) ? (pair_prec == 1 ? 3 : 1) : 0;
  ch.l5_jobs5 = ch.tiled;
  ch.xcd_lanes = pair_xcd_lanes(t.xcd_order, n_scenes, pair_grid(njobs, n_cu));
  ch.xcd_lanes5 = pair_xcd_lanes(t.xcd_order, n_scenes, pair_grid(njobs5, n_cu));

  ch.fp32_dec = pair_prec == 0 || !t.enc_mfma || A < t.dec_mfma_min;
  ch.split_dec = ch.fp32_dec && have_side && t.dec_overlap;
  ch.dec_actor = ch.split_dec ? PRED_DEC_SPLIT : ch.fp32_dec ? PRED_DEC_ONE : PRED_DEC_MFMA;
  ch.mw_blocks = ((n_scenes + 7) / 8) * 8 * DEC_MW_G;
  ch.want_mw = t.dec_mw && ch.mw_blocks <= n_cu;
  ch.cls_side = ch.split_dec && t.dec_cls_side;
  ch.tgt_wait_first = have_side && !t.tgt_side;
  return ch;
}
```

mind_amd/csrc/predict.hip:

```cpp
__global__ void k_tokpos(const TokMeta *__restrict__ meta, int n_tok, const float *__restrict__ actr,
                         const float *__restrict__ avec, const float *__restrict__ lctr,
                         const float *__restrict__ lvec, float *__restrict__ tokpos) {
  const int t = blockIdx.x * blockDim.x + threadIdx.x;
  if (t >= n_tok) return;
  const TokMeta m = meta[t];
  float4 o = make_float4(0.f, 0.f, 0.f, 0.f);
  if (m.type == 0 && actr) o = make_float4(actr[m.src * 2], actr[m.src * 2 + 1], avec[m.src * 2], avec[m.src * 2 + 1]);
  if (m.type == 1 && lctr) o = make_float4(lctr[m.src * 2], lctr[m.src * 2 + 1], lvec[m.src * 2], lvec[m.src * 2 + 1]);
  ((float4 *)tokpos)[t] = o;
}

struct PairTables {
  std::vector<TokMeta> meta;
  std::vector<PairJob> jobs, jobs5;
  std::vector<int> actor_row, actor_scene, cls_row, scene_n;
  long long edge_pairs = 0, edge_pairs_t = 0;
  int ntok = 0, slot = 0;
  double pairs_full = 0, pairs_l5 = 0;
};

static void pair_tables_build(int Bn, const int *scene_actors, const int *scene_lanes, bool xcd_order, int n_cu, PairTables &T) {
  int A = 0;
  for (int b = 0; b < Bn; ++b) A += scene_actors[b];
  T.actor_row.assign(A, 0); T.actor_scene.assign(A, 0); T.cls_row.assign(Bn, 0); T.scene_n.assign(Bn, 0);
// ... 40 lines not shown
  for (const PairJob &J : T.jobs)
    if (J.flags & 1) T.jobs5.push_back(J);
  for (std::vector<PairJob> *jl : {&T.jobs, &T.jobs5}) {
    const int grid = pair_grid((long long)jl->size(), n_cu);
    pair_jobs_deal(*jl, grid, PAIR_WAVES, pair_xcd_lanes(xcd_order, Bn, grid));
  }
}

extern "C" int mind_debug_pair_schedule(const int *scene_tokens, const int *scene_actors, int n_scenes, int n_cu, int last_layer, int *out_jobs, int cap,
                                        int *out_info) {
  if (!scene_tokens || !scene_actors || n_scenes <= 0 || n_cu <= 0 || !out_jobs || !out_info) return MIND_EINVAL;
  std::vector<int> lanes(n_scenes);
  for (int b = 0; b < n_scenes; ++b) {
    const int N = scene_tokens[b], a = scene_actors[b];
    if (N <= 0 || a < 0 || a >= N) return MIND_EINVAL;
    lanes[b] = N - a - 1;
  }
  PairTables T;
  pair_tables_build(n_scenes, scene_actors, lanes.data(), true, n_cu, T);
  const std::vector<PairJob> &jl = last_layer ? T.jobs5 : T.jobs;
  const int grid = pair_grid((long long)jl.size(), n_cu);
  const int stride = grid * PAIR_WAVES;
  int n = 0;
  for (size_t i = 0; i < jl.size(); ++i) {
    const PairJob &J = jl[i];
    if (J.t1 <= J.t0) continue;
    if (n < cap) {
      int *o = out_jobs + (size_t)6 * n;
      o[0] = J.scene; o[1] = J.j; o[2] = J.t0; o[3] = J.t1; o[4] = J.slot; o[5] = (int)(i % stride);
    }
    ++n;
  }
  out_info[0] = pair_column_splits(scene_tokens[0]); out_info[1] = grid; out_info[2] = (int)jl.size(); out_info[3] = n;
  return n;
}

#define PRED_CHOICE_HEADER 32
extern "C" int mind_debug_predict_choice(const char *const *knob_names, const int *knob_values, int n_knobs, int pair_prec, int n_cu, int have_side,
                                         const int *scene_actors, const int *scene_lanes, int n_scenes, long long *out, int cap) {
  if (n_knobs < 0 || (n_knobs > 0 && (!knob_names || !knob_values)) || pair_prec < 0 || pair_prec > 3 || n_cu <= 0 || !scene_actors || !scene_lanes ||
      n_scenes <= 0 || cap < 0 || (cap > 0 && !out))
    return MIND_EINVAL;
  PredTuning t;
  for (int k = 0; k < n_knobs; ++k)
    if (!knob_names[k] || !pred_tuning_set(t, knob_names[k], knob_values[k])) return MIND_EINVAL;
  for (int b = 0; b < n_scenes; ++b)
    if (scene_actors[b] <= 0 || scene_lanes[b] < 0) return MIND_EINVAL;
  const PredChoice ch = pred_choose(t, pair_prec, n_cu, have_side != 0, n_scenes, scene_actors, scene_lanes);
  const bool mfma_dec = ch.dec_actor == PRED_DEC_MFMA;
  const long long head[PRED_CHOICE_HEADER] = {
      PRED_CHOICE_HEADER, (long long)ch.tok_runs.size(), ch.np, ch.actor_form, ch.actor_arg, ch.actor_grid, ch.actor_chunk, ch.actor_chunks,
      ch.actor_launches, ch.qsplit, ch.qk_stride, ch.tiled, ch.edge_bf16, pred_edge_pair_bytes(t, pair_prec), ch.tok_chunk, ch.tok_lw,
      ch.last_tok_chunks, ch.pair_family, ch.pair_np, ch.l5_jobs5, ch.xcd_lanes, ch.xcd_lanes5, ch.dec_actor, mfma_dec ? ch.np : 0,
      ch.fp32_dec, ch.split_dec, ch.want_mw, ch.mw_blocks, ch.cls_side && !ch.want_mw, ch.tgt_wait_first, 0, 0};
  std::vector<long long> rec(head, head + PRED_CHOICE_HEADER);
  for (const PredTokRun &r : ch.tok_runs) rec.insert(rec.end(), {r.t0, r.n, r.kind, r.layerwise, r.small, r.merged});
  for (size_t i = 0; i < rec.size() && (int)i < cap; ++i) out[i] = rec[i];
  return (int)rec.size();
}

struct PredCall {
  mind_ctx *c;
  const mind_scene_batch *in;
  mind_pred_out *out;
  const PredChoice &ch;
  int Bn, A, Ltot;
  hipStream_t st, ss;
  TableSet *ts = nullptr;
  const float *lane_feat = nullptr;
  const float *const *rpe_dev = nullptr;
  hipEvent_t *evs = nullptr;
  bool tok_timed = false;
  size_t ev_tok_used = 0;
  float *x() const { return (float *)c->x.p; }
  const int *rows() const { return (const int *)ts->rows.p; }
};

static int pred_tables(PredCall &p, const int *scene_actors, const int *scene_lanes) {
  mind_ctx *c = p.c;
  const int Bn = p.Bn, A = p.A;
  std::vector<int> key;
  key.reserve(2 * Bn + 3);
  key.push_back(Bn);
  for (int b = 0; b <= Bn; ++b) key.push_back(p.in->actor_off[b]);
  for (int b = 0; b <= Bn; ++b) key.push_back(p.in->lane_off[b]);
  TableSet *ts = nullptr;
  for (TableSet &t : c->tabs)
    if (t.key == key) ts = &t;
  const bool tab_hit = ts != nullptr;
  if (!ts) {
    ts = &c->tabs[0];
    for (TableSet &t : c->tabs)
      if (t.stamp < ts->stamp) ts = &t;
  }
  ts->stamp = ++c->tab_clock;
  p.ts = ts;
  if (tab_hit) {
    c->n_table_hits++;
    return MIND_OK;
  }
  PairTables T;
  pair_tables_build(Bn, scene_actors, scene_lanes, c->pt.xcd_order, c->n_cu, T);
  int rc;
  ts->key.clear();
  if ((rc = ensure(c, ts->meta, T.meta.size() * sizeof(TokMeta)))) return rc;
  if ((rc = ensure(c, ts->jobs, T.jobs.size() * sizeof(PairJob)))) return rc;
  if ((rc = ensure(c, ts->jobs5, T.jobs5.size() * sizeof(PairJob)))) return rc;
// ... 46 lines not shown
  mind_ctx *c = p.c;
  const PredChoice &ch = p.ch;
  const float *actors = p.in->actors;
  float *actor_feat = (float *)c->actor_feat.p;
  const int A = p.A;
  const dim3 grid(ch.actor_grid);
  switch (ch.actor_form) {
  case PRED_ACTOR_F32:
    if (ch.actor_arg == 2) hipLaunchKernelGGL(k_actor_f32<2>, grid, dim3(AF_T), mind_actor_f32_lds_bytes(2), p.st, actors, A, actor_feat, c->W.actorF);
    else hipLaunchKernelGGL(k_actor_f32<1>, grid, dim3(AF_T), mind_actor_f32_lds_bytes(1), p.st, actors, A, actor_feat, c->W.actorF);
    break;
  case PRED_ACTOR_VALU:
    hipLaunchKernelGGL(k_actor_net, grid, dim3(AT), mind_actor_lds_bytes(), p.st, actors, A, actor_feat, c->W.actor);
    break;
  case PRED_ACTOR_LW: {
    int rc;
    if ((rc = ensure_exact(c, c->actor_lw_arena, lw_arena_bytes(ch.actor_chunk), "the layer-wise ActorNet's arena"))) return rc;
    lw_build_plan(A, ch.actor_chunk, c->actor_lw_plan);
    u32 *arena = (u32 *)c->actor_lw_arena.p;
    const int nl = ch.np == 6 ? lw_run<6>(c->actor_lw_plan, p.st, arena, actors, actor_feat, c->W.actorB)
                 : ch.np == 3 ? lw_run<3>(c->actor_lw_plan, p.st, arena, actors, actor_feat, c->W.actorB)
                              : lw_run<1>(c->actor_lw_plan, p.st, arena, actors, actor_feat, c->W.actorB);
    if (nl < 0) return fail(c, MIND_ESTATE, "layer-wise ActorNet: a stage has no kernel");
    c->last_actor_lw = 1; c->last_actor_launches = nl; c->last_actor_chunks = ch.actor_chunks;
    break;
  }
  default:
    if (ch.np == 6) hipLaunchKernelGGL(k_actor_mfma<6>, grid, dim3(AM_T), mind_actor_mfma_lds_bytes(), p.st, actors, A, actor_feat, c->W.actorB);
    else if (ch.np == 3) hipLaunchKernelGGL(k_actor_mfma<3>, grid, dim3(AM_T), mind_actor_mfma_lds_bytes(), p.st, actors, A, actor_feat, c->W.actorB);
    else hipLaunchKernelGGL(k_actor_mfma<1>, grid, dim3(AM_T), mind_actor_mfma_lds_bytes(), p.st, actors, A, actor_feat, c->W.actorB);
  }
  return MIND_OK;
}

static int pred_encoders(PredCall &p) {
  mind_ctx *c = p.c;
  const mind_scene_batch *in = p.in;
  hipStream_t st = p.st, ss = p.ss;
  const int Bn = p.Bn, Ltot = p.Ltot, ntok = p.ts->ntok;
  if (c->side) {
    HIPCHK(c, hipEventRecord(c->ev_main, st));
    HIPCHK(c, hipStreamWaitEvent(c->side, c->ev_main, 0));
  }
  const bool act_timed = c->profiling && !c->ev_defer;
  if (act_timed && !c->ev_act0) {
    HIPCHK(c, hipEventCreate(&c->ev_act0));
    HIPCHK(c, hipEventCreate(&c->ev_act1));
  }
  c->last_actor_lw = 0; c->last_actor_launches = 1; c->last_actor_chunks = 1; c->actor_ms = 0.f;
  if (act_timed) HIPCHK(c, hipEventRecord(c->ev_act0, st));
  int rc;
  if ((rc = pred_actor_net(p))) return rc;
  if (act_timed) HIPCHK(c, hipEventRecord(c->ev_act1, st));
  p.lane_feat = in->lane_feat;
  if (!p.lane_feat) {
    float *lf = p.out->lane_feat ? p.out->lane_feat : (float *)c->lane_feat.p;
    if (Ltot > 0)
      hipLaunchKernelGGL(k_lane_net, dim3((Ltot + PL - 1) / PL), dim3(DT), 0, ss, in->lanes, Ltot, lf, c->W.lane);
    p.lane_feat = lf;
  } else if (p.out->lane_feat && p.out->lane_feat != in->lane_feat && Ltot > 0) {
    HIPCHK(c, hipMemcpyAsync(p.out->lane_feat, in->lane_feat, (size_t)Ltot * 128 * sizeof(float), hipMemcpyDeviceToDevice, ss));
  }
  hipLaunchKernelGGL(k_tokpos, dim3((ntok + 255) / 256), dim3(256), 0, ss, (const TokMeta *)p.ts->meta.p, ntok, in->actor_ctrs, in->actor_vecs,
                     in->lane_ctrs, in->lane_vecs, (float *)c->tokpos.p);
  if (c->side) {
    HIPCHK(c, hipEventRecord(c->ev_side, c->side));
    HIPCHK(c, hipStreamWaitEvent(st, c->ev_side, 0));
  }
  hipLaunchKernelGGL(k_lane_net, dim3((Bn + PL - 1) / PL), dim3(DT), 0, ss, in->tgt_nodes, Bn, (float *)c->tgt_feat.p, c->W.lane);
  hipLaunchKernelGGL(k_dec_tgt, dim3(Bn), dim3(DT), mind_dec_scene_lds_bytes(), ss, (const float *)c->tgt_feat.p, in->tgt_rpe, (float *)c->tgt_emb.p,
                     c->W.dec);
  if (c->side) HIPCHK(c, hipEventRecord(c->ev_tgt, c->side));
  if (p.ch.tgt_wait_first) HIPCHK(c, hipStreamWaitEvent(st, c->ev_tgt, 0));
  return MIND_OK;
}

static hipError_t pred_tok_mark(PredCall &p, int tag) {
  mind_ctx *c = p.c;
  if (!p.tok_timed) return hipSuccess;
  if (p.ev_tok_used == c->ev_tok.size()) {
    hipEvent_t e;
    const hipError_t rc_ = hipEventCreate(&e);
    if (rc_ != hipSuccess) return rc_;
    c->ev_tok.push_back(e);
    c->ev_tok_tag.push_back(0);
  }
  c->ev_tok_tag[p.ev_tok_used] = tag;
  return hipEventRecord(c->ev_tok[p.ev_tok_used++], p.st);
}

static int pred_token_step(PredCall &p, int mode, int Lw) {
  mind_ctx *c = p.c;
  hipStream_t st = p.st;
  const size_t qk_stride = p.ch.qk_stride, tokm_lds = mind_token_mfma_lds_bytes();
  const float *actor_feat = (const float *)c->actor_feat.p, *lane_feat = p.lane_feat;
  float *part = (float *)c->part.p;
  HIPCHK(c, pred_tok_mark(p, -1));
  for (const PredTokRun &r : p.ch.tok_runs) {
    const TokMeta *m_ = (const TokMeta *)p.ts->meta.p + r.t0;
    float *x_ = p.x() + (size_t)r.t0 * 128, *ST_ = (float *)c->ST.p + (size_t)r.t0 * 256, *QK_ = (float *)c->QK.p + (size_t)r.t0 * qk_stride;
    if (r.layerwise) {
      tl_build_plan(r.n, mode, p.ch.tok_chunk, c->n_cu, c->tok_lw_plan);
      for (const TlLaunch &L : c->tok_lw_plan) {
        if (tl_launch(L, st, mode, m_, actor_feat, lane_feat, x_, part, ST_, QK_, qk_stride, c->W.tok[Lw], c->W.tokM[Lw], (float *)c->tok_lw_arena.p, p.ch.tok_chunk))
          return fail(c, MIND_ESTATE, "layer-wise token stage: a stage has no kernel");
        HIPCHK(c, pred_tok_mark(p, L.stage));
      }
      c->last_tok_launches += (int)c->tok_lw_plan.size();
      continue;
    }
    c->last_tok_launches++;
    if (r.kind == 0) {
      const int tpw = r.small ? TOK_TPW_SMALL : TOK_TPW_BIG;
      hipLaunchKernelGGL(r.small ? (r.merged ? k_token_m : k_token<TOK_TPW_SMALL>) : k_token<TOK_TPW_BIG>, dim3((r.n + tpw - 1) / tpw), dim3(TT_THREADS), 0,
                         st, m_, r.n, mode, actor_feat, lane_feat, x_, part, ST_, QK_, c->W.tok[Lw]);
    } else if (r.kind == 1) {
      hipLaunchKernelGGL(k_token_mfma<0>, dim3((r.n + TM_TOK - 1) / TM_TOK), dim3(TM_THREADS), tokm_lds, st, m_, r.n, mode, actor_feat, lane_feat, x_,
                         part, ST_, QK_, c->W.tok[Lw], c->W.tokM[Lw]);
    } else {
      hipLaunchKernelGGL(k_token_mfma<1>, dim3((r.n + TM_TOK - 1) / TM_TOK), dim3(TM_THREADS), tokm_lds, st, m_, r.n, mode, actor_feat, lane_feat, x_,
                         part, ST_, QK_, c->W.tok[Lw], c->W.tokB[Lw]);
    }
    HIPCHK(c, pred_tok_mark(p, TL_NSTAGE));
  }
// ... 78 lines not shown
static int pred_decoder(PredCall &p) {
  mind_ctx *c = p.c;
  const PredChoice &ch = p.ch;
  mind_pred_out *out = p.out;
  hipStream_t st = p.st;
  const int A = p.A, Bn = p.Bn;
  const float *x = p.x();
  const int *d_actor_row = p.rows(), *d_actor_scene = d_actor_row + A, *d_cls_row = d_actor_row + 2 * A;
  const float *cmode = (const float *)c->cmode.p, *tgt_emb = (const float *)c->tgt_emb.p;
  const dim3 agrid((A + RA - 1) / RA), mgrid((A + DM_RA - 1) / DM_RA);
  int rc;
  if (ch.split_dec) {
    if ((rc = ensure(c, c->dec_h2, (size_t)A * 768 * sizeof(float)))) return rc;
    HIPCHK(c, hipEventRecord(c->ev_main, st));
    HIPCHK(c, hipStreamWaitEvent(c->side, c->ev_main, 0));
    hipLaunchKernelGGL(k_dec_actor<1>, agrid, dim3(DT), mind_dec_actor_lds_bytes(), c->side, x, d_actor_row, d_actor_scene, A,
                       (const float *)nullptr, (const float *)nullptr, (float *)nullptr, (float *)nullptr, c->W.dec, (float *)c->dec_h2.p);
    HIPCHK(c, hipEventRecord(c->ev_side, c->side));
  }
  bool cls_on_side = false;
  bool mw = ch.want_mw;
  if (mw) {
    if (c->dec_abort && *(volatile unsigned *)c->dec_abort) return fail(c, MIND_EHIP, "k_dec_scene_mw: a barrier of an earlier launch timed out (launch not resident)");
    if (!c->dec_abort) {
      if (hipHostMalloc((void **)&c->dec_abort, 64, hipHostMallocMapped) != hipSuccess) { c->dec_abort = nullptr; mw = false; }
      else *c->dec_abort = 0u;
    }
    const size_t need_x = (size_t)(c->n_cu / DEC_MW_G) * 2 * 6 * 1536 * sizeof(float), need_b = (size_t)(c->n_cu / DEC_MW_G) * 4 * sizeof(unsigned);
    if (mw && c->dec_xbuf.cap < need_x) {
      if ((rc = ensure(c, c->dec_xbuf, need_x))) return rc;
    }
    if (mw && c->dec_bars.cap < need_b) {
      if ((rc = ensure(c, c->dec_bars, need_b))) return rc;
      HIPCHK(c, hipMemsetAsync(c->dec_bars.p, 0, c->dec_bars.cap, st));
    }
  }
  if (mw)
    hipLaunchKernelGGL(k_dec_scene_mw, dim3(ch.mw_blocks), dim3(DT), mind_dec_scene_lds_bytes(), st, x, d_cls_row, (float *)c->cmode.p, out->cls, c->W.dec, Bn,
                       (float *)c->dec_xbuf.p, (unsigned *)c->dec_bars.p, c->dec_abort);
  else if (ch.cls_side) {
    hipLaunchKernelGGL(k_dec_scene_c, dim3(Bn), dim3(DT), mind_dec_scene_lds_bytes(), st, x, d_cls_row, (float *)c->cmode.p, c->W.dec);
    HIPCHK(c, hipEventRecord(c->ev_main, st));
    HIPCHK(c, hipStreamWaitEvent(c->side, c->ev_main, 0));
    hipLaunchKernelGGL(k_dec_cls, dim3(Bn), dim3(DT), mind_dec_scene_lds_bytes(), c->side, (float *)c->cmode.p, out->cls, c->W.dec);
    if (!c->ev_cls) HIPCHK(c, hipEventCreateWithFlags(&c->ev_cls, hipEventDisableTiming));
    HIPCHK(c, hipEventRecord(c->ev_cls, c->side));
    cls_on_side = true;
  } else
    hipLaunchKernelGGL(k_dec_scene, dim3(Bn), dim3(DT), mind_dec_scene_lds_bytes(), st, x, d_cls_row, (float *)c->cmode.p, out->cls, c->W.dec);
  if (c->side) HIPCHK(c, hipStreamWaitEvent(st, c->ev_tgt, 0));
  switch (ch.dec_actor) {
  case PRED_DEC_SPLIT:
    HIPCHK(c, hipStreamWaitEvent(st, c->ev_side, 0));
    hipLaunchKernelGGL(k_dec_actor<2>, agrid, dim3(DT), mind_dec_actor_lds_bytes(), st, x, d_actor_row, d_actor_scene, A, cmode, tgt_emb, out->reg,
                       out->vel, c->W.dec, (float *)c->dec_h2.p);
    break;
  case PRED_DEC_ONE:
    hipLaunchKernelGGL(k_dec_actor<0>, agrid, dim3(DT), mind_dec_actor_lds_bytes(), st, x, d_actor_row, d_actor_scene, A, cmode, tgt_emb, out->reg,
                       out->vel, c->W.dec, (float *)nullptr);
    break;
  default: {
#define DEC_MFMA(NPV)                                                                                                                     \
  hipLaunchKernelGGL(k_dec_actor_mfma<NPV>, mgrid, dim3(DM_T), mind_dec_actor_mfma_lds_bytes(), st, x, d_actor_row, d_actor_scene, A, cmode, \
                     tgt_emb, out->reg, out->vel, c->W.decB)
    if (ch.np == 6) DEC_MFMA(6);
    else if (ch.np == 3) DEC_MFMA(3);
    else DEC_MFMA(1);
#undef DEC_MFMA
  }
  }
  if (cls_on_side) HIPCHK(c, hipStreamWaitEvent(st, c->ev_cls, 0));
  return MIND_OK;
}

static int pred_finish(PredCall &p) {
  mind_ctx *c = p.c;
  mind_pred_out *out = p.out;
  const float *x = p.x();
  for (int a = 0; a < p.A && out->actor_emb; ++a)
    HIPCHK(c, hipMemcpyAsync(out->actor_emb + (size_t)a * 128, x + (size_t)p.ts->actor_row[a] * 128, 128 * sizeof(float), hipMemcpyDeviceToDevice, p.st));
  for (int b = 0; b < p.Bn && out->cls_emb; ++b)
    HIPCHK(c, hipMemcpyAsync(out->cls_emb + (size_t)b * 128, x + (size_t)p.ts->cls_row[b] * 128, 128 * sizeof(float), hipMemcpyDeviceToDevice, p.st));
  HIPCHK(c, hipGetLastError());
  if (c->profiling && c->ev_defer) {
    c->pair_ms = 0.f;
  } else if (c->profiling) {
    HIPCHK(c, hipStreamSynchronize(p.st));
    c->pair_ms = 0.f;
    for (int L = 0; L < c->debug_layers; ++L) {
      float ms = 0.f;
      HIPCHK(c, hipEventElapsedTime(&ms, c->ev[2 * L], c->ev[2 * L + 1]));
      c->pair_ms += ms;
    }
    if (c->ev_act0) HIPCHK(c, hipEventElapsedTime(&c->actor_ms, c->ev_act0, c->ev_act1));
    for (size_t i = 1; i < p.ev_tok_used; ++i) {
      if (c->ev_tok_tag[i] < 0) continue;
      float ms = 0.f;
      HIPCHK(c, hipEventElapsedTime(&ms, c->ev_tok[i - 1], c->ev_tok[i]));
      c->tok_stage_ms[c->ev_tok_tag[i]] += ms;
      c->tok_ms += ms;
    }
  }
  return MIND_OK;
}

extern "C" int mind_predict_batch(mind_ctx *c, const mind_scene_batch *in, mind_pred_out *out) {
  if (!c || !in || !out) return MIND_EINVAL;
  if (!c->have_weights) return fail(c, MIND_ESTATE, "weights not loaded");
// ... 26 lines not shown
```

Baseline: 1790.

## Poll host flag for round decisions, fold root setup into predictor, tune decoder head grid

Replaces the host stream synchronize after the AIME select/branch glue with a spin on a pinned generation word. The last kernel block writes that word after a grid-wide counter. It also presizes next-round buffers while waiting, and moves root lane/history kernels and field prep onto the predictor's side stream via enc_pre/enc_post hooks. Separately, the split decoder head now picks actors-per-block (1, 2 or RA) from the actor count versus CU count to widen the grid. This costs a busy-waiting host thread plus new env knobs, and the device-to-host flag ordering depends on system-scope fences.

```diff
diff --git a/include/mind_hip.h b/include/mind_hip.h
--- a/include/mind_hip.h
+++ b/include/mind_hip.h
@@ -88,6 +88,8 @@
 int mind_debug_aime_book(int pred_len, int max_depth, int max_rounds, int n_agents, int world, int rank, int force, int n_rounds, const int *dec_len,
                          const float *dec, int n_tokens, int bytes_per_pair, int plan_chunk_mb, int per_scene, long long *out, int cap, char *msg,
                          int msg_cap);
+
+int mind_debug_wait_word(const unsigned *word, unsigned want, double timeout_s, double (*clock)(void *user), void *user, int spins_per_look);
 
 int mind_debug_actor_lw_plan(int n_actors, int np, int chunk, long long *out_launches, int cap, long long *out_info);
 
diff --git a/mind_amd/_lib.py b/mind_amd/_lib.py
--- a/mind_amd/_lib.py
+++ b/mind_amd/_lib.py
@@ -4,6 +4,7 @@
 _HERE = os.path.dirname(os.path.abspath(__file__))
 LIB_PATH = os.environ.get("MIND_HIP_LIB", os.path.join(_HERE, "libmind_hip.so"))
 
+WAIT_CLOCK = C.CFUNCTYPE(C.c_double, C.c_void_p)
 MIND_OK = 0
 MIND_EINVAL, MIND_ENOMEM, MIND_EHIP, MIND_ESTATE, MIND_ENOTFOUND = -1, -2, -3, -4, -5
 
@@ -162,7 +163,7 @@
            "mind_weights_load", "mind_predict_batch", "mind_last_fusion_stats", "mind_last_actor_stats", "mind_debug_actor_lw_plan", "mind_last_token_stats", "mind_last_token_stage_ms", "mind_debug_token_lw_plan", "mind_set_profiling",
            "mind_ilqr_solve_trees", "mind_ilqr_contingency", "mind_ilqr_solve_fields", "mind_cost_eval", "mind_ilqr_score_trees", "mind_ilqr_gains", "mind_ilqr_policy_rollouts", "mind_lane_dist_field", "mind_aime_world", "mind_aime_rebase", "mind_debug_aime_decide", "mind_debug_set_layers",
            "mind_debug_read", "mind_set_pair_precision", "mind_get_pair_precision", "mind_debug_pack_bfrag", "mind_debug_pack_conv_frag", "mind_debug_pack", "mind_debug_weight_image", "mind_debug_weight_bind", "mind_debug_pair_schedule", "mind_debug_predict_choice", "mind_debug_ilqr_plan", "mind_debug_aime_book", "mind_set_tuning", "mind_last_ilqr_stats", "mind_aime_plan", "mind_last_ilqr_profile", "mind_eval_traj_trees", "mind_last_ilqr_trace", "mind_ilqr_contingency_begin", "mind_ilqr_finish", "mind_fill_tracks", "mind_ilqr_contingency_begin_plan", "mind_debug_trig", "mind_aime_plan_begin", "mind_aime_plan_poll", "mind_aime_plan_finish", "mind_ctx_busy", "mind_ilqr_finish_plan",
-           "mind_set_exchange", "mind_last_exchange_stats",
+           "mind_set_exchange", "mind_last_exchange_stats", "mind_debug_wait_word",
            "mind_loop_create", "mind_loop_destroy", "mind_loop_reset", "mind_loop_advance", "mind_loop_state", "mind_loop_last_plan", "mind_loop_export",
            "mind_planner_create", "mind_planner_destroy", "mind_planner_reset", "mind_planner_observe", "mind_planner_set_lanes", "mind_planner_set_target_lane",
            "mind_planner_set_solve_lane", "mind_planner_set_eval_lane", "mind_planner_plan", "mind_planner_last_plan", "mind_planner_export"]
@@ -252,6 +253,7 @@
                                               C.c_int, C.POINTER(C.c_longlong), C.c_int]
     lib.mind_debug_ilqr_plan.argtypes = [C.POINTER(C.c_char_p), C.POINTER(C.c_int), C.c_int, C.c_int, C.c_int, C.c_int, C.POINTER(C.c_int), C.POINTER(C.c_int32),
                                          C.POINTER(C.c_longlong), C.c_int, C.POINTER(C.c_int)]
+    lib.mind_debug_wait_word.argtypes = [C.POINTER(C.c_uint), C.c_uint, C.c_double, WAIT_CLOCK, C.c_void_p, C.c_int]
     lib.mind_debug_aime_book.argtypes = [C.c_int] * 8 + [C.POINTER(C.c_int), C.POINTER(C.c_float)] + [C.c_int] * 4 + [C.POINTER(C.c_longlong), C.c_int, C.c_char_p, C.c_int]
     lib.mind_debug_trig.argtypes = [C.c_void_p, C.POINTER(C.c_double), C.c_int, C.POINTER(C.c_double)]
     lib.mind_debug_pack_conv_frag.argtypes = [C.POINTER(C.c_float), C.c_int, C.c_int, C.c_int, C.POINTER(C.c_uint32), C.c_size_t]
@@ -292,7 +294,8 @@
 
 PRED_CHOICE_FIELDS = ("header", "n_runs", "np", "actor_form", "actor_arg", "actor_grid", "actor_chunk", "actor_chunks", "actor_launches", "qsplit", "qk_stride",
                       "tiled", "edge_bf16", "edge_pair_bytes", "tok_chunk", "tok_lw", "tok_chunks", "pair_family", "pair_np", "l5_jobs5", "xcd_lanes",
-                      "xcd_lanes5", "dec_actor", "dec_np", "fp32_dec", "split_dec", "want_mw", "mw_blocks", "cls_on_side", "tgt_wait_first")
+                      "xcd_lanes5", "dec_actor", "dec_np", "fp32_dec", "split_dec", "want_mw", "mw_blocks", "cls_on_side", "tgt_wait_first",
+                      "dec_head_ra")
 PAIR_PREC = ("f32", "bf16x3", "bf16", "bf16x6")
 
 
@@ -309,7 +312,7 @@
     if n == MIND_EINVAL:
         return None
     assert 0 < n <= cap and out[0] == 32 and n == 32 + 6 * out[1], n
-    d = dict(zip(PRED_CHOICE_FIELDS, out[:30]))
+    d = dict(zip(PRED_CHOICE_FIELDS, out[:31]))
     d["runs"] = [tuple(out[32 + 6 * i:38 + 6 * i]) for i in range(out[1])]
     return d
 
diff --git a/mind_amd/csrc/aime_book.h b/mind_amd/csrc/aime_book.h
--- a/mind_amd/csrc/aime_book.h
+++ b/mind_amd/csrc/aime_book.h
@@ -42,6 +42,18 @@
 inline int pl_chunk(int n_tokens, int bytes_per_pair, int plan_chunk_mb, int Bk) {
   const double edge_mb = (double)n_tokens * (((n_tokens + 15) / 16) * 16) * bytes_per_pair / (1024.0 * 1024.0);
   return std::max(1, (int)std::min<double>((double)(Bk > 0 ? Bk : 1), (double)plan_chunk_mb / edge_mb));
+}
+
+typedef double (*pl_clock_fn)(void *user);
+inline bool pl_wait_word(const volatile unsigned *word, unsigned want, double timeout_s, pl_clock_fn now, void *user, unsigned spins_per_look) {
+  if (__atomic_load_n((const unsigned *)word, __ATOMIC_ACQUIRE) == want) return true;
+  const double t0 = now(user);
+  for (unsigned spins = 0;;) {
+    if (__atomic_load_n((const unsigned *)word, __ATOMIC_ACQUIRE) == want) return true;
+    if (++spins < spins_per_look) continue;
+    spins = 0;
+    if (now(user) - t0 > timeout_s) return false;
+  }
 }
 
 enum { PL_OK = 0, PL_E_ROUNDS, PL_E_ROOT, PL_E_TRIMMED, PL_E_AGAIN, PL_E_ORDER, PL_E_NO_END };
diff --git a/mind_amd/csrc/aime_kernels.hip b/mind_amd/csrc/aime_kernels.hip
--- a/mind_amd/csrc/aime_kernels.hip
+++ b/mind_amd/csrc/aime_kernels.hip
@@ -227,10 +227,21 @@
   pos[2 * o] = x; pos[2 * o + 1] = y; vel[2 * o] = vx; vel[2 * o + 1] = vy; ang[o] = h;
 }
 
+struct AimeDone { unsigned *cnt; unsigned *h_gen; unsigned gen; };
+__device__ __forceinline__ void aime_decisions_done(const AimeDone D) {
+  if (!D.h_gen) return;
+  __threadfence_system();
+  const unsigned prev = __hip_atomic_fetch_add(D.cnt, 1u, __ATOMIC_ACQ_REL, __HIP_MEMORY_SCOPE_AGENT);
+  if (prev + 1u != gridDim.x) return;
+  __hip_atomic_store(D.cnt, 0u, __ATOMIC_RELAXED, __HIP_MEMORY_SCOPE_AGENT);
+  __threadfence_system();
+  __hip_atomic_store(D.h_gen, D.gen, __ATOMIC_RELEASE, __HIP_MEMORY_SCOPE_SYSTEM);
+}
+
 __global__ __launch_bounds__(64) void k_aime_branch(const AimeScene *__restrict__ scenes, const float *__restrict__ sel,
                                                     const float *__restrict__ world, unsigned *__restrict__ hit,
                                                     const float *__restrict__ sel_prob, float *__restrict__ h_sel, float *__restrict__ h_selp,
-                                                    unsigned *__restrict__ h_hit, const AimeSmall sm) {
+                                                    unsigned *__restrict__ h_hit, const AimeSmall sm, const AimeDone done) {
   const int b = blockIdx.x / AIME_K, j = blockIdx.x % AIME_K, t = threadIdx.x;
   const AimeScene S = sm.n ? sm.s[b] : scenes[b];
   const int k = (int)sel[(size_t)b * AIME_K + j];
@@ -246,6 +257,7 @@
   if (h_sel && t == 0) {
     h_hit[2 * (size_t)blockIdx.x] = (unsigned)m; h_hit[2 * (size_t)blockIdx.x + 1] = (unsigned)(m >> 32);
     h_sel[blockIdx.x] = sel[blockIdx.x]; h_selp[blockIdx.x] = sel_prob[blockIdx.x];
+    aime_decisions_done(done);
   }
 }
 
@@ -254,7 +266,7 @@
                                                            const float *__restrict__ ego_end, int lane_check, float dist_thres, float prob_floor,
                                                            const float *__restrict__ world, float *__restrict__ sel, float *__restrict__ sel_prob,
                                                            unsigned *__restrict__ hit, float *__restrict__ h_sel, float *__restrict__ h_selp,
-                                                           unsigned *__restrict__ h_hit, const AimeSmall sm) {
+                                                           unsigned *__restrict__ h_hit, const AimeSmall sm, const AimeDone done) {
   const int b = blockIdx.x / AIME_K, j = blockIdx.x % AIME_K, t = threadIdx.x;
   const AimeScene S = sm.n ? sm.s[b] : scenes[b];
   const float sp = sm.n ? sm.prob[b] : scen_prob[b];
@@ -285,6 +297,7 @@
     if (h_sel) {
       h_hit[2 * (size_t)blockIdx.x] = (unsigned)m; h_hit[2 * (size_t)blockIdx.x + 1] = (unsigned)(m >> 32);
       h_sel[blockIdx.x] = kf; h_selp[blockIdx.x] = pj;
+      aime_decisions_done(done);
     }
   }
 }
diff --git a/mind_amd/csrc/aime_plan.hip b/mind_amd/csrc/aime_plan.hip
--- a/mind_amd/csrc/aime_plan.hip
+++ b/mind_amd/csrc/aime_plan.hip
@@ -69,6 +69,8 @@
     if (on) fprintf(stderr, "[plan] %8.1f us  %s\n", std::chrono::duration<double, std::micro>(std::chrono::steady_clock::now() - t0).count(), what);
   }
 };
+
+double pl_steady_now(void *) { return std::chrono::duration<double>(std::chrono::steady_clock::now().time_since_epoch()).count(); }
 
 struct PlanRun {
   mind_ctx *c;
@@ -93,6 +95,8 @@
   DevBuf *tabb = nullptr;
   float *d_topo = nullptr, *d_ego = nullptr, *d_sel = nullptr, *d_selp = nullptr, *h_mirror = nullptr, *d_world = nullptr;
   unsigned *d_hit = nullptr;
+  unsigned *h_gen = nullptr, want_gen = 0;
+  int round_no = 0;
   int nxt = 0;
   InLayout q{0, 0, 0};
   float *d_in = nullptr, *w_pos = nullptr, *w_ang = nullptr, *w_vel = nullptr;
@@ -106,7 +110,7 @@
         ro(in_->n_agents, in_->n_lanes, in_->n_lane_pts, in_->raw_pos != nullptr) {}
   bool solves_asked() const { return in->solve_cfg_full && in->solve_x0 && in->solve_lane && in->solve_n_lane_pts >= 2 && !dist; }
   int fail_book(const PlErr &e) const { return fail(c, MIND_ESTATE, pl_err_format(e.code), e.a0, e.a1); }
-  int pl_root(), pl_root_raw(), pl_root_host();
+  int pl_root(), pl_root_raw(), pl_root_host(), pl_presize_next();
   int pl_round_buffers(int round), pl_round_launch(), pl_round_tables(), pl_round_decisions(const float *&h_dec);
   int pl_predict_chunk(int g0, int cb, float *d_cls, float *d_reg, float *d_vel, const float *&d_ctrs, const float *&d_vecs);
   int pl_rebase_next(), pl_exchange_next(int round), pl_next_inputs(), pl_pack_results(), pl_hand_out();
@@ -186,14 +190,27 @@
   R.pos = d + o.rpos; R.ang = d + o.rang; R.vel = d + o.rvel; R.pad = d + o.rpad;
   R.lane_ctrs0 = nullptr; R.lane_vecs0 = nullptr; R.travel0 = in->travel0;
   hipLaunchKernelGGL(k_aime_rebase, dim3(1, 1 + RB_FEAT_BLOCKS(a)), dim3(RB_THREADS), 5 * a * sizeof(float), st, R);
+  const auto lanes = [this, d](hipStream_t rs) {
+    const RootLayout &o = ro;
+    hipLaunchKernelGGL(k_aime_root_lanes, dim3(l), dim3(64), 0, rs, (const double *)(d + o.lpts), (const int *)(d + o.lfl), (const float *)(d + o.fr),
+                       d + o.lc, d + o.lv, d + o.lanes);
+    HIPCHK(c, hipGetLastError());
+    return (int)MIND_OK;
+  };
+  const auto hist = [this, d](hipStream_t rs) {
+    const RootLayout &o = ro;
+    hipLaunchKernelGGL(k_aime_root_hist, dim3(a), dim3(64), 0, rs, (const float *)(d + o.rpos), (const float *)(d + o.rang), (const float *)(d + o.rvel),
+                       (const float *)(d + o.fr), (const float *)(d + o.ctrs), (const float *)(d + o.vecs), d + o.wpos, d + o.wang, d + o.wvel, d + o.cov);
+    HIPCHK(c, hipGetLastError());
+    return pl_frames_back(d + o.fr, 1, rs);
+  };
+  if (c->root_head && c->side && !dist) {
+    c->enc_pre = lanes; c->enc_post = hist;
+    return MIND_OK;
+  }
   hipStream_t rs;
-  if ((rc = pl_side_hop(rs))) return rc;
-  hipLaunchKernelGGL(k_aime_root_lanes, dim3(l), dim3(64), 0, rs, (const double *)(d + o.lpts), (const int *)(d + o.lfl), (const float *)(d + o.fr),
-                     d + o.lc, d + o.lv, d + o.lanes);
-  hipLaunchKernelGGL(k_aime_root_hist, dim3(a), dim3(64), 0, rs, (const float *)(d + o.rpos), (const float *)(d + o.rang), (const float *)(d + o.rvel),
-                     (const float *)(d + o.fr), (const float *)(d + o.ctrs), (const float *)(d + o.vecs), d + o.wpos, d + o.wang, d + o.wvel, d + o.cov);
-  HIPCHK(c, hipGetLastError());
-  return pl_frames_back(d + o.fr, 1, rs);
+  if ((rc = pl_side_hop(rs)) || (rc = lanes(rs))) return rc;
+  return hist(rs);
 }
 
 int PlanRun::pl_root_host() {
@@ -233,7 +250,13 @@
   droot = (const float *)c->pl_root.p;
   if ((rc = raw ? pl_root_raw() : pl_root_host())) return rc;
   if ((rc = ensure(c, c->pl_lf, (size_t)l * 128 * sizeof(float)))) return rc;
-  if (solves_asked() && (rc = il_field_prepare(c, in->solve_cfg_full, in->solve_x0, in->solve_lane, in->solve_n_lane_pts, c->pl_copy))) return rc;
+  if (solves_asked()) {
+    const auto field = [this]() { return il_field_prepare(c, in->solve_cfg_full, in->solve_x0, in->solve_lane, in->solve_n_lane_pts, c->pl_copy); };
+    if (c->enc_post) {
+      const std::function<int(hipStream_t)> hist = std::move(c->enc_post);
+      c->enc_post = [hist, field](hipStream_t rs) { const int rc_ = hist(rs); return rc_ ? rc_ : field(); };
+    } else if ((rc = field())) return rc;
+  }
   prev_pos = droot + ro.wpos; prev_ang = droot + ro.wang; prev_vel = droot + ro.wvel;
   cov_last_dev = droot + ro.cov;
   return MIND_OK;
@@ -247,9 +270,10 @@
   if ((rc = ensure(c, c->pl_small, (n_topo + n_ego + n_back) * sizeof(float)))) return rc;
   d_topo = (float *)c->pl_small.p; d_ego = d_topo + n_topo; d_sel = d_ego + n_ego; d_selp = d_sel + (size_t)Bmax * 6;
   d_hit = (unsigned *)(d_selp + (size_t)Bmax * 6);
-  h_mirror = nullptr;
+  h_mirror = nullptr; h_gen = nullptr;
+  round_no = round;
   if (!dist && c->dec_mirror) {
-    if ((rc = pl_pin(c, 2, n_back * sizeof(float)))) return rc;
+    if ((rc = pl_pin(c, 2, n_back * sizeof(float) + 64))) return rc;
     h_mirror = (float *)c->pl_pin[2];
   }
   tabb = &c->pl_tab[round & 1];
@@ -270,6 +294,16 @@
   }
   tables_done = false;
   all_small = c->tab_small && std::min(chunk, std::max(Bk, 1)) <= AIME_SMALL;
+  if (h_mirror && c->dec_poll && Bk > 0 && chunk >= Bk) {
+    if (!c->pl_cnt.p) {
+      if ((rc = ensure(c, c->pl_cnt, 64))) return rc;
+      HIPCHK(c, hipMemsetAsync(c->pl_cnt.p, 0, 64, st));
+    }
+    h_gen = (unsigned *)(h_mirror + n_back);
+    if (++c->dec_gen == 0u) c->dec_gen = 1u;
+    want_gen = c->dec_gen;
+    __atomic_store_n(h_gen, 0u, __ATOMIC_RELEASE);
+  }
   return MIND_OK;
 }
 
@@ -380,12 +414,13 @@
     float *hs_ = h_mirror ? h_mirror + (size_t)c0 * 6 : nullptr, *hp_ = h_mirror ? h_mirror + (size_t)Bmax * 6 + (size_t)c0 * 6 : nullptr;
     unsigned *hh_ = h_mirror ? (unsigned *)(h_mirror + (size_t)Bmax * 12) + (size_t)c0 * 12 : nullptr;
     const float pf_ = in->prob_floor > 0.f ? in->prob_floor : 0.001f;
+    const AimeDone dn{h_gen ? (unsigned *)c->pl_cnt.p : nullptr, h_gen, want_gen};
     if (c->glue_fused) {
       hipLaunchKernelGGL(k_aime_select_branch, dim3(cb * AIME_K), dim3(64), 0, st, t_sc, d_cls, t_prob, topo_c, ego_c, 1, in->dist_thres, pf_, w_c, sel_c, selp_c,
-                         hit_c, hs_, hp_, hh_, sm);
+                         hit_c, hs_, hp_, hh_, sm, dn);
     } else {
       hipLaunchKernelGGL(k_aime_select, dim3(cb), dim3(64), 0, st, t_sc, d_cls, t_prob, topo_c, ego_c, 1, in->dist_thres, sel_c, selp_c, pf_, sm);
-      hipLaunchKernelGGL(k_aime_branch, dim3(cb * AIME_K), dim3(64), 0, st, t_sc, sel_c, w_c, hit_c, (const float *)selp_c, hs_, hp_, hh_, sm);
+      hipLaunchKernelGGL(k_aime_branch, dim3(cb * AIME_K), dim3(64), 0, st, t_sc, sel_c, w_c, hit_c, (const float *)selp_c, hs_, hp_, hh_, sm, dn);
     }
     HIPCHK(c, hipGetLastError());
   }
@@ -405,10 +440,30 @@
     HIPCHK(c, hipMemcpyAsync(c->pl_pin[2], d_sel, n_back * sizeof(float), hipMemcpyDeviceToHost, st));
   }
   TR("round: glue launched, waiting for the decisions");
-  HIPCHK(c, hipStreamSynchronize(st));
+  if (h_gen) {
+    if ((rc = pl_presize_next())) return rc;
+    if (!pl_wait_word(h_gen, want_gen, 0.25, pl_steady_now, nullptr, 1024)) {
+      HIPCHK(c, hipStreamSynchronize(st));
+      HIPCHK(c, hipMemsetAsync(c->pl_cnt.p, 0, 64, st));
+    }
+  } else {
+    HIPCHK(c, hipStreamSynchronize(st));
+  }
   TR("round: decisions on the host");
   h_dec = (const float *)c->pl_pin[2];
   return MIND_OK;
+}
+
+int PlanRun::pl_presize_next() {
+  if (round_no + 1 >= in->max_rounds) return MIND_OK;
+  const size_t OBS = RB_T, S = (size_t)g.B * AIME_K;
+  const int n = cur_in < 0 ? 0 : cur_in ^ 1;
+  const size_t b_in = InLayout(S, a, l).total * sizeof(float), b_win = S * a * OBS * 5 * sizeof(float), b_rep = S * l * 128 * sizeof(float);
+  if (std::max(b_in, std::max(b_win, b_rep)) >= ((size_t)64 << 20)) return MIND_OK;
+  int rc;
+  if (b_in > c->pl_in[n].cap || b_win > c->pl_win[n].cap || b_rep > c->pl_lrep.cap) HIPCHK(c, hipStreamSynchronize(st));
+  if ((rc = ensure(c, c->pl_in[n], b_in)) || (rc = ensure(c, c->pl_win[n], b_win)) || (rc = ensure(c, c->pl_lrep, b_rep))) return rc;
+  return pl_pin(c, 3, S * 28 * sizeof(float));
 }
 
 int PlanRun::pl_rebase_next() {
@@ -504,15 +559,24 @@
   const int S = book.rec.S;
   int nlo, nhi, rc;
   pl_block(S, XR, XW, nlo, nhi);
-  hipStream_t rs;
-  if ((rc = pl_side_hop(rs))) return rc;
-  if (nhi - nlo > 1) {
-    if ((rc = ensure(c, c->pl_lrep, (size_t)(nhi - nlo) * l * 128 * sizeof(float)))) return rc;
-    const size_t n = (size_t)l * 128;
-    hipLaunchKernelGGL(k_repeat_rows, dim3((unsigned)((n * (nhi - nlo) + 255) / 256)), dim3(256), 0, rs, (const float *)c->pl_lf.p, n, nhi - nlo, (float *)c->pl_lrep.p);
-    HIPCHK(c, hipGetLastError());
-  }
-  if ((rc = pl_frames_back(d_in + q.fr, (size_t)S, rs))) return rc;
+  const int n_rep = nhi - nlo;
+  if (n_rep > 1 && (rc = ensure(c, c->pl_lrep, (size_t)n_rep * l * 128 * sizeof(float)))) return rc;
+  const auto rep = [this, n_rep](hipStream_t rs) {
+    if (n_rep > 1) {
+      const size_t n = (size_t)l * 128;
+      hipLaunchKernelGGL(k_repeat_rows, dim3((unsigned)((n * n_rep + 255) / 256)), dim3(256), 0, rs, (const float *)c->pl_lf.p, n, n_rep, (float *)c->pl_lrep.p);
+      HIPCHK(c, hipGetLastError());
+    }
+    return (int)MIND_OK;
+  };
+  const float *d_fr = d_in + q.fr;
+  const auto back = [this, d_fr, S](hipStream_t rs) { return pl_frames_back(d_fr, (size_t)S, rs); };
+  if (c->round_head && c->side && !dist) {
+    c->enc_pre = rep; c->enc_post = back;
+  } else {
+    hipStream_t rs;
+    if ((rc = pl_side_hop(rs)) || (rc = rep(rs)) || (rc = back(rs))) return rc;
+  }
   prev_pos = w_pos; prev_ang = w_ang; prev_vel = w_vel;
   cov_last_dev = d_in + q.cov;
   cur_in = nxt;
@@ -625,6 +689,7 @@
   if (!c->ev_pl) HIPCHK(c, hipEventCreateWithFlags(&c->ev_pl, hipEventDisableTiming));
   if (!c->ev_tab) HIPCHK(c, hipEventCreateWithFlags(&c->ev_tab, hipEventDisableTiming));
   if (!c->pl_copy) HIPCHK(c, hipStreamCreateWithFlags(&c->pl_copy, hipStreamNonBlocking));
+  struct HookGuard { mind_ctx *c; ~HookGuard() { c->enc_pre = nullptr; c->enc_post = nullptr; } } hook_guard{c};
   if ((rc = p.pl_root())) return rc;
   memset(out, 0, sizeof(*out));
   p.TR.t0 = std::chrono::steady_clock::now();
@@ -708,6 +773,11 @@
   if (e == hipErrorNotReady) return 1;
   if (e != hipSuccess) return fail(c, MIND_EHIP, "mind_ctx_busy: %s", hipGetErrorString(e));
   return 0;
+}
+
+extern "C" int mind_debug_wait_word(const unsigned *word, unsigned want, double timeout_s, double (*clock)(void *), void *user, int spins_per_look) {
+  if (!word || !(timeout_s >= 0.0) || spins_per_look <= 0) return MIND_EINVAL;
+  return pl_wait_word(word, want, timeout_s, clock ? clock : pl_steady_now, user, (unsigned)spins_per_look) ? 1 : 0;
 }
 
 constexpr int PL_BOOK_HEADER = 16;
diff --git a/mind_amd/csrc/encdec_kernels.hip b/mind_amd/csrc/encdec_kernels.hip
--- a/mind_amd/csrc/encdec_kernels.hip
+++ b/mind_amd/csrc/encdec_kernels.hip
@@ -302,6 +302,66 @@
     }
 #pragma unroll
     for (int r = 0; r < R; ++r) part[(kp * R + r) * NOUT + o] = acc[r];
+  }
+  __syncthreads();
+  for (int i = threadIdx.x; i < R * NOUT; i += nthr) {
+    const int r = i / NOUT, oo = i % NOUT;
+    float v = b ? b[oo] : 0.f;
+    for (int q = 0; q < KP; ++q) v += part[(q * R + r) * NOUT + oo];
+    out[r * ldo + oo] = v;
+  }
+}
+
+constexpr int dense_scalar_kp(int R, int NOUT, int K, int nthr, int part_floats) {
+  int KP = NOUT < nthr ? nthr / NOUT : 1;
+  while (KP > 1 && (KP * R * NOUT > part_floats || (K / 4) < KP)) KP >>= 1;
+  int p2 = 1;
+  while (p2 * 2 <= KP) p2 *= 2;
+  return p2;
+}
+
+template <int R, int RPT>
+__device__ __forceinline__ void dense_ksplit(const float *in, int ldi, int K, const float *__restrict__ WT, const float *__restrict__ b, int NOUT,
+                                             float *out, int ldo, float *part, int KP) {
+  const int nthr = blockDim.x;
+  constexpr int NG = (R + RPT - 1) / RPT;
+  const int Kc = ((K / 4 + KP - 1) / KP) * 4;
+  for (int item = threadIdx.x; item < NG * KP * NOUT; item += nthr) {
+    const int o = item % NOUT, kp = (item / NOUT) % KP, r0 = (item / (NOUT * KP)) * RPT;
+    float acc[RPT];
+#pragma unroll
+    for (int j = 0; j < RPT; ++j) acc[j] = 0.f;
+    const int k0 = kp * Kc, k1 = min(K, k0 + Kc);
+    int k = k0;
+    for (; k + DB <= k1; k += DB) {
+      float w[DB];
+#pragma unroll
+      for (int q = 0; q < DB; ++q) w[q] = WT[(size_t)(k + q) * NOUT + o];
+#pragma unroll
+      for (int j = 0; j < RPT; ++j) {
+        if (r0 + j >= R) continue;
+#pragma unroll
+        for (int q4 = 0; q4 < DB / 4; ++q4) {
+          const f32x4 x = *(const f32x4 *)(in + (r0 + j) * ldi + k + 4 * q4);
+          acc[j] = fmaf(w[4 * q4 + 0], x[0], acc[j]);
+          acc[j] = fmaf(w[4 * q4 + 1], x[1], acc[j]);
+          acc[j] = fmaf(w[4 * q4 + 2], x[2], acc[j]);
+          acc[j] = fmaf(w[4 * q4 + 3], x[3], acc[j]);
+        }
+      }
+    }
+    for (; k < k1; k += 4) {
+#pragma unroll
+      for (int j = 0; j < RPT; ++j) {
+        if (r0 + j >= R) continue;
+        const f32x4 x = *(const f32x4 *)(in + (r0 + j) * ldi + k);
+#pragma unroll
+        for (int q = 0; q < 4; ++q) acc[j] = fmaf(WT[(size_t)(k + q) * NOUT + o], x[q], acc[j]);
+      }
+    }
+#pragma unroll
+    for (int j = 0; j < RPT; ++j)
+      if (r0 + j < R) part[(kp * R + r0 + j) * NOUT + o] = acc[j];
   }
   __syncthreads();
   for (int i = threadIdx.x; i < R * NOUT; i += nthr) {
@@ -852,7 +912,7 @@
 
 #define RA 4
 #define DEC_ACTOR_LDS_FLOATS (512 + 1536 + 3072 + 3072 + 3072 + 960 + 6144)
-template <int PART>
+template <int PART, int RAT = RA>
 __global__ __launch_bounds__(DT) void k_dec_actor(const float *__restrict__ x ,
                                                   const int *__restrict__ actor_row ,
                                                   const int *__restrict__ actor_scene , int n_actors,
@@ -868,37 +928,39 @@
   float (*prm)[40] = (float (*)[40])(dsm + 11264);
   float *part = dsm + 12224;
   const int PF = 6144;
+  static_assert(RAT == RA || (PART == 2 && (RAT == 1 || RAT == 2)), "only the head runs with fewer agents per workgroup");
+  constexpr int HEAD_KP = dense_scalar_kp(RA * 6, 128, 128, DT, 6144);
   const int tid = threadIdx.x;
-  const int a0 = blockIdx.x * RA;
+  const int a0 = blockIdx.x * RAT;
   if (PART != 2) {
-    for (int i = tid; i < RA * 128; i += blockDim.x) {
+    for (int i = tid; i < RAT * 128; i += blockDim.x) {
       const int r = i / 128, a = a0 + r;
       xin[r][i % 128] = a < n_actors ? x[(size_t)actor_row[a] * 128 + i % 128] : 0.f;
     }
     __syncthreads();
-    dense<RA>(&xin[0][0], 128, 128, W.a0W, W.a0b, 384, &h1[0][0], 384, part, PF);
-    __syncthreads();
-    ln_rows(&h1[0][0], 384, RA, 384, W.a0g, W.a0be, true);
-    __syncthreads();
-    dense<RA>(&h1[0][0], 384, 384, W.a3W, W.a3b, 768, &h2[0][0], 768, part, PF);
-    __syncthreads();
-    ln_rows(&h2[0][0], 768, RA, 768, W.a3g, W.a3be, true);
+    dense<RAT>(&xin[0][0], 128, 128, W.a0W, W.a0b, 384, &h1[0][0], 384, part, PF);
+    __syncthreads();
+    ln_rows(&h1[0][0], 384, RAT, 384, W.a0g, W.a0be, true);
+    __syncthreads();
+    dense<RAT>(&h1[0][0], 384, 384, W.a3W, W.a3b, 768, &h2[0][0], 768, part, PF);
+    __syncthreads();
+    ln_rows(&h2[0][0], 768, RAT, 768, W.a3g, W.a3be, true);
     __syncthreads();
     if (PART == 1) {
-      for (int i = tid; i < RA * 768; i += blockDim.x) {
+      for (int i = tid; i < RAT * 768; i += blockDim.x) {
         const int r = i / 768, a = a0 + r;
         if (a < n_actors) h2g[(size_t)a * 768 + i % 768] = h2[r][i % 768];
       }
       return;
     }
   } else {
-    for (int i = tid; i < RA * 768; i += blockDim.x) {
+    for (int i = tid; i < RAT * 768; i += blockDim.x) {
       const int r = i / 768, a = a0 + r;
       h2[r][i % 768] = a < n_actors ? h2g[(size_t)a * 768 + i % 768] : 0.f;
     }
     __syncthreads();
   }
-  for (int i = tid; i < RA * 768; i += blockDim.x) {
+  for (int i = tid; i < RAT * 768; i += blockDim.x) {
     const int r = i / 768, k = (i % 768) / 128, c = i % 128;
     const int a = a0 + r;
     float v = 0.f;
@@ -910,22 +972,24 @@
     E[r * 6 + k][c] = v;
   }
   __syncthreads();
-  dense<RA * 6>(&E[0][0], 128, 128, W.r0W, W.r0b, 128, &t1[0][0], 128, part, PF);
-  __syncthreads();
-  ln_rows(&t1[0][0], 128, RA * 6, 128, W.r0g, W.r0be, true);
-  __syncthreads();
-  dense<RA * 6>(&t1[0][0], 128, 128, W.r3W, W.r3b, 128, &E[0][0], 128, part, PF);
-  __syncthreads();
-  ln_rows(&E[0][0], 128, RA * 6, 128, W.r3g, W.r3be, true);
-  __syncthreads();
-  for (int i = tid; i < RA * 6 * 40; i += blockDim.x) {
+  if (RAT == RA) dense<RA * 6>(&E[0][0], 128, 128, W.r0W, W.r0b, 128, &t1[0][0], 128, part, PF);
+  else dense_ksplit<RAT * 6, RAT + 1>(&E[0][0], 128, 128, W.r0W, W.r0b, 128, &t1[0][0], 128, part, HEAD_KP);
+  __syncthreads();
+  ln_rows(&t1[0][0], 128, RAT * 6, 128, W.r0g, W.r0be, true);
+  __syncthreads();
+  if (RAT == RA) dense<RA * 6>(&t1[0][0], 128, 128, W.r3W, W.r3b, 128, &E[0][0], 128, part, PF);
+  else dense_ksplit<RAT * 6, RAT + 1>(&t1[0][0], 128, 128, W.r3W, W.r3b, 128, &E[0][0], 128, part, HEAD_KP);
+  __syncthreads();
+  ln_rows(&E[0][0], 128, RAT * 6, 128, W.r3g, W.r3be, true);
+  __syncthreads();
+  for (int i = tid; i < RAT * 6 * 40; i += blockDim.x) {
     const int r = i / 40, o = i % 40;
     float acc = W.r6b[o];
     for (int k = 0; k < 128; ++k) acc = fmaf(W.r6W[k * 40 + o], E[r][k], acc);
     prm[r][o] = acc;
   }
   __syncthreads();
-  for (int i = tid; i < RA * 6 * 60; i += blockDim.x) {
+  for (int i = tid; i < RAT * 6 * 60; i += blockDim.x) {
     const int r = i / 60, t = i % 60;
     const int a = a0 + r / 6, k = r % 6;
     if (a >= n_actors) continue;
diff --git a/mind_amd/csrc/mind_hip.hip b/mind_amd/csrc/mind_hip.hip
--- a/mind_amd/csrc/mind_hip.hip
+++ b/mind_amd/csrc/mind_hip.hip
@@ -80,6 +80,11 @@
   int upload_kernel_max = 1 << 20;
   bool dec_mirror = true;
   bool glue_fused = true;
+  bool dec_poll = true;
+  unsigned dec_gen = 0;
+  DevBuf pl_cnt;
+  bool root_head = true, round_head = true;
+  std::function<int(hipStream_t)> enc_pre, enc_post;
   bool early_eval = true;
   int tab_host_max = 4096;
   bool tab_small = true;
@@ -289,6 +294,9 @@
   if (const char *we = getenv("MIND_EARLY_EVAL")) c->early_eval = atoi(we) != 0;
   if (const char *we = getenv("MIND_GLUE_FUSED")) c->glue_fused = atoi(we) != 0;
   if (const char *we = getenv("MIND_DEC_MIRROR")) c->dec_mirror = atoi(we) != 0;
+  if (const char *we = getenv("MIND_DEC_POLL")) c->dec_poll = atoi(we) != 0;
+  if (const char *we = getenv("MIND_ROOT_HEAD")) c->root_head = atoi(we) != 0;
+  if (const char *we = getenv("MIND_ROUND_HEAD")) c->round_head = atoi(we) != 0;
   if (const char *we = getenv("MIND_UPLOAD_KERNEL_MAX")) c->upload_kernel_max = std::max(0, atoi(we));
   const char *const il_env[][2] = {{"MIND_ILQR_CHUNK", "ilqr_chunk"}, {"MIND_ILQR_WGS", "ilqr_wgs"}, {"MIND_ILQR_SPEC_DERIV", "ilqr_spec_deriv"},
                                    {"MIND_ILQR_HOST_OUT_MAX", "ilqr_host_out_max"}, {"MIND_ILQR_SLOTS", "ilqr_slots"}};
@@ -302,6 +310,9 @@
   (void)hipFuncSetAttribute((const void *)k_dec_actor<0>, hipFuncAttributeMaxDynamicSharedMemorySize, (int)mind_dec_actor_lds_bytes());
   (void)hipFuncSetAttribute((const void *)k_dec_actor<1>, hipFuncAttributeMaxDynamicSharedMemorySize, (int)mind_dec_actor_lds_bytes());
   (void)hipFuncSetAttribute((const void *)k_dec_actor<2>, hipFuncAttributeMaxDynamicSharedMemorySize, (int)mind_dec_actor_lds_bytes());
+  (void)hipFuncSetAttribute((const void *)k_dec_actor<2, 1>, hipFuncAttributeMaxDynamicSharedMemorySize, (int)mind_dec_actor_lds_bytes());
+  (void)hipFuncSetAttribute((const void *)k_dec_actor<2, 2>, hipFuncAttributeMaxDynamicSharedMemorySize, (int)mind_dec_actor_lds_bytes());
+  if (const char *te = getenv("MIND_DEC_HEAD_RA")) (void)pred_tuning_set(c->pt, "dec_head_ra", atoi(te));
   *out = c;
   return MIND_OK;
 }
@@ -323,7 +334,7 @@
     if (b->p) (void)hipFree(b->p);
   if (c->dec_abort) (void)hipHostFree(c->dec_abort);
   for (DevBuf *b : {&c->pl_root, &c->pl_in[0], &c->pl_in[1], &c->pl_lf, &c->pl_lrep, &c->pl_pred, &c->pl_small, &c->pl_tab[0], &c->pl_tab[1], &c->pl_win[0],
-                    &c->pl_win[1], &c->pl_flat, &c->x_send, &c->x_recv, &c->x_seg})
+                    &c->pl_win[1], &c->pl_flat, &c->x_send, &c->x_recv, &c->x_seg, &c->pl_cnt})
     if (b->p) (void)hipFree(b->p);
   for (DevBuf &b : c->pl_world)
     if (b.p) (void)hipFree(b.p);
@@ -377,6 +388,9 @@
   else if (n == "early_eval") c->early_eval = value != 0;
   else if (n == "glue_fused") c->glue_fused = value != 0;
   else if (n == "dec_mirror") c->dec_mirror = value != 0;
+  else if (n == "dec_poll") c->dec_poll = value != 0;
+  else if (n == "root_head") c->root_head = value != 0;
+  else if (n == "round_head") c->round_head = value != 0;
   else if (n == "upload_kernel_max") c->upload_kernel_max = value < 0 ? 0 : value;
   else return fail(c, MIND_EINVAL, "mind_set_tuning: unknown knob '%s'", name);
   return MIND_OK;
@@ -820,11 +834,11 @@
     const int lc = lane_check ? 1 : 0;
     if (fused) {
       hipLaunchKernelGGL(k_aime_select_branch, dim3(B * AIME_K), dim3(64), 0, st, t_sc, cls, t_prob, topo, ego_end, lc, dist_thres, pf_, world, sel, sel_prob,
-                         hit, (float *)nullptr, (float *)nullptr, (unsigned *)nullptr, sm);
+                         hit, (float *)nullptr, (float *)nullptr, (unsigned *)nullptr, sm, AimeDone{nullptr, nullptr, 0u});
     } else {
       hipLaunchKernelGGL(k_aime_select, dim3(B), dim3(64), 0, st, t_sc, cls, t_prob, topo, ego_end, lc, dist_thres, sel, sel_prob, pf_, sm);
       hipLaunchKernelGGL(k_aime_branch, dim3(B * AIME_K), dim3(64), 0, st, t_sc, (const float *)sel, world, hit, (const float *)sel_prob, (float *)nullptr,
-                         (float *)nullptr, (unsigned *)nullptr, sm);
+                         (float *)nullptr, (unsigned *)nullptr, sm, AimeDone{nullptr, nullptr, 0u});
     }
     e = hipGetLastError();
     if (e == hipSuccess) e = hipStreamSynchronize(st);
diff --git a/mind_amd/csrc/pred_choice.h b/mind_amd/csrc/pred_choice.h
--- a/mind_amd/csrc/pred_choice.h
+++ b/mind_amd/csrc/pred_choice.h
@@ -17,6 +17,7 @@
   int tok_small_max = 2048;
   int dec_mfma_min = 1 << 30;
   bool dec_overlap = true;
+  int dec_head_ra = 0;
   bool dec_mw = false;
   bool dec_cls_side = false;
   bool tgt_side = true;
@@ -35,6 +36,7 @@
   else if (is("xcd_order")) t.xcd_order = value != 0;
   else if (is("pair_tile")) t.pair_tile = value != 0;
   else if (is("dec_overlap")) t.dec_overlap = value != 0;
+  else if (is("dec_head_ra")) t.dec_head_ra = (value == 1 || value == 2 || value == RA) ? value : 0;
   else if (is("tok_mfma")) t.tok_mfma = value != 0;
   else if (is("tok_small_max")) t.tok_small_max = value;
   else if (is("tok_merge")) t.tok_merge = value != 0;
@@ -80,6 +82,7 @@
   bool l5_jobs5 = false;
   int xcd_lanes = 1, xcd_lanes5 = 1;
   int dec_actor = PRED_DEC_ONE;
+  int dec_head_ra = RA;
   bool fp32_dec = true, split_dec = false, want_mw = false, cls_side = false;
   int mw_blocks = 0;
   bool tgt_wait_first = false;
@@ -144,6 +147,7 @@
   ch.fp32_dec = pair_prec == 0 || !t.enc_mfma || A < t.dec_mfma_min;
   ch.split_dec = ch.fp32_dec && have_side && t.dec_overlap;
   ch.dec_actor = ch.split_dec ? PRED_DEC_SPLIT : ch.fp32_dec ? PRED_DEC_ONE : PRED_DEC_MFMA;
+  if (ch.split_dec) ch.dec_head_ra = t.dec_head_ra ? t.dec_head_ra : A <= n_cu ? 1 : (A + 1) / 2 <= n_cu ? 2 : RA;
   ch.mw_blocks = ((n_scenes + 7) / 8) * 8 * DEC_MW_G;
   ch.want_mw = t.dec_mw && ch.mw_blocks <= n_cu;
   ch.cls_side = ch.split_dec && t.dec_cls_side;
diff --git a/mind_amd/csrc/predict.hip b/mind_amd/csrc/predict.hip
--- a/mind_amd/csrc/predict.hip
+++ b/mind_amd/csrc/predict.hip
@@ -116,7 +116,7 @@
       PRED_CHOICE_HEADER, (long long)ch.tok_runs.size(), ch.np, ch.actor_form, ch.actor_arg, ch.actor_grid, ch.actor_chunk, ch.actor_chunks,
       ch.actor_launches, ch.qsplit, ch.qk_stride, ch.tiled, ch.edge_bf16, pred_edge_pair_bytes(t, pair_prec), ch.tok_chunk, ch.tok_lw,
       ch.last_tok_chunks, ch.pair_family, ch.pair_np, ch.l5_jobs5, ch.xcd_lanes, ch.xcd_lanes5, ch.dec_actor, mfma_dec ? ch.np : 0,
-      ch.fp32_dec, ch.split_dec, ch.want_mw, ch.mw_blocks, ch.cls_side && !ch.want_mw, ch.tgt_wait_first, 0, 0};
+      ch.fp32_dec, ch.split_dec, ch.want_mw, ch.mw_blocks, ch.cls_side && !ch.want_mw, ch.tgt_wait_first, ch.split_dec ? ch.dec_head_ra : 0, 0};
   std::vector<long long> rec(head, head + PRED_CHOICE_HEADER);
   for (const PredTokRun &r : ch.tok_runs) rec.insert(rec.end(), {r.t0, r.n, r.kind, r.layerwise, r.small, r.merged});
   for (size_t i = 0; i < rec.size() && (int)i < cap; ++i) out[i] = rec[i];
@@ -269,6 +269,11 @@
   int rc;
   if ((rc = pred_actor_net(p))) return rc;
   if (act_timed) HIPCHK(c, hipEventRecord(c->ev_act1, st));
+  if (c->enc_pre) {
+    const std::function<int(hipStream_t)> pre = std::move(c->enc_pre);
+    c->enc_pre = nullptr;
+    if ((rc = pre(ss))) return rc;
+  }
   p.lane_feat = in->lane_feat;
   if (!p.lane_feat) {
     float *lf = p.out->lane_feat ? p.out->lane_feat : (float *)c->lane_feat.p;
@@ -287,6 +292,11 @@
   hipLaunchKernelGGL(k_lane_net, dim3((Bn + PL - 1) / PL), dim3(DT), 0, ss, in->tgt_nodes, Bn, (float *)c->tgt_feat.p, c->W.lane);
   hipLaunchKernelGGL(k_dec_tgt, dim3(Bn), dim3(DT), mind_dec_scene_lds_bytes(), ss, (const float *)c->tgt_feat.p, in->tgt_rpe, (float *)c->tgt_emb.p,
                      c->W.dec);
+  if (c->enc_post) {
+    const std::function<int(hipStream_t)> post = std::move(c->enc_post);
+    c->enc_post = nullptr;
+    if ((rc = post(ss))) return rc;
+  }
   if (c->side) HIPCHK(c, hipEventRecord(c->ev_tgt, c->side));
   if (p.ch.tgt_wait_first) HIPCHK(c, hipStreamWaitEvent(st, c->ev_tgt, 0));
   return MIND_OK;
@@ -471,8 +481,13 @@
   switch (ch.dec_actor) {
   case PRED_DEC_SPLIT:
     HIPCHK(c, hipStreamWaitEvent(st, c->ev_side, 0));
-    hipLaunchKernelGGL(k_dec_actor<2>, agrid, dim3(DT), mind_dec_actor_lds_bytes(), st, x, d_actor_row, d_actor_scene, A, cmode, tgt_emb, out->reg,
-                       out->vel, c->W.dec, (float *)c->dec_h2.p);
+#define DEC_HEAD(RAV)                                                                                                                       \
+  hipLaunchKernelGGL((k_dec_actor<2, RAV>), dim3((A + RAV - 1) / RAV), dim3(DT), mind_dec_actor_lds_bytes(), st, x, d_actor_row, d_actor_scene, A, \
+                     cmode, tgt_emb, out->reg, out->vel, c->W.dec, (float *)c->dec_h2.p)
+    if (ch.dec_head_ra == 1) DEC_HEAD(1);
+    else if (ch.dec_head_ra == 2) DEC_HEAD(2);
+    else DEC_HEAD(RA);
+#undef DEC_HEAD
     break;
   case PRED_DEC_ONE:
     hipLaunchKernelGGL(k_dec_actor<0>, agrid, dim3(DT), mind_dec_actor_lds_bytes(), st, x, d_actor_row, d_actor_scene, A, cmode, tgt_emb, out->reg,
```

Result: faster. 1821, median of 6 (+1.8%).
